# tsereda/fast-cwdm

Hardware: AMD Instinct MI355X
Metric: denoising-steps/sec on 8-ch 128^3 volumes (1000-step DDPM, i2i cWDM) (higher is better)
Workload: dtype bf16; 1 GPU; config2: BraTS 3->1 conditional synthesis, 1xMI355X per replica, 128^3 subbands, 1000-step DDPM (direct linear schedule); model=UNetModel run.sh (mc 64, mult 1,2,2,4,4, 2 res blocks, 81.5M params), global_batch=1, seq_len=2097152, parallelism=replicas1

## Files before the change

### fast-cwdm_amd/csrc/common.hpp

```cpp
#pragma once
#include <hip/hip_runtime.h>
#include <stdint.h>
#include <cstdlib>
#include <string>

#include "../../include/cwdm.h"

namespace cwdm {

void set_error(const std::string& msg);
int fail(int code, const std::string& msg);

#define CWDM_HIP(expr)                                                        \
  do {                                                                        \
    hipError_t e_ = (expr);                                                   \
    if (e_ != hipSuccess)                                                     \
      return ::cwdm::fail(CWDM_E_HIP, std::string(#expr) + ": " +            \
                                          hipGetErrorString(e_));             \
  } while (0)

#define CWDM_REQUIRE(cond, code, msg)                                         \
  do {                                                                        \
    if (!(cond)) return ::cwdm::fail(code, msg);                              \
  } while (0)
// ... 42 lines not shown
  static constexpr int kDtype = CWDM_BF16;
  __device__ __forceinline__ static float to_f(bf16_t v) { return bf2f(v); }
  __device__ __forceinline__ static bf16_t from_f(float v) { return f2bf(v); }
};
template <> struct Elem<f16_t> {
  static constexpr int kDtype = CWDM_F16;
  __device__ __forceinline__ static float to_f(f16_t v) { return (float)v; }
  __device__ __forceinline__ static f16_t from_f(float v) { return (f16_t)v; }
};

template <typename T> __device__ __forceinline__ float lo2f(unsigned u);
template <typename T> __device__ __forceinline__ float hi2f(unsigned u);
template <> __device__ __forceinline__ float lo2f<bf16_t>(unsigned u) { return __uint_as_float(u << 16); }
template <> __device__ __forceinline__ float hi2f<bf16_t>(unsigned u) { return __uint_as_float(u & 0xffff0000u); }
template <> __device__ __forceinline__ float lo2f<f16_t>(unsigned u) {
  return (float)__builtin_bit_cast(f16_t, (unsigned short)(u & 0xffffu));
}
template <> __device__ __forceinline__ float hi2f<f16_t>(unsigned u) {
  return (float)__builtin_bit_cast(f16_t, (unsigned short)(u >> 16));
}
template <typename T> __device__ __forceinline__ unsigned pack2(float a, float b);
template <> __device__ __forceinline__ unsigned pack2<bf16_t>(float a, float b) {
  typedef __bf16 bf16x2_t __attribute__((ext_vector_type(2)));
  const f32x2_t v = {a, b};
  return __builtin_bit_cast(unsigned, __builtin_convertvector(v, bf16x2_t));
}
template <> __device__ __forceinline__ unsigned pack2<f16_t>(float a, float b) {
  const f32x2_t v = {a, b};
  return __builtin_bit_cast(unsigned, __builtin_convertvector(v, f16x2_t));
}

inline int dtype_size(int dtype) { return dtype == CWDM_F32 ? 4 : 2; }
inline bool dtype_half(int dtype) { return dtype == CWDM_BF16 || dtype == CWDM_F16; }
inline bool dtype_compute(int dtype) { return dtype == CWDM_F32 || dtype == CWDM_BF16 || dtype == CWDM_F16; }

template <typename F>
inline int dispatch_dtype(int dtype, F&& f) {
  if (dtype == CWDM_BF16) return f(bf16_t{});
  if (dtype == CWDM_F16) return f(f16_t{});
  return f(float{});
}

inline int ck_of(int dtype) { return 32 / dtype_size(dtype); }

inline int64_t ceil_div(int64_t a, int64_t b) { return (a + b - 1) / b; }

inline int env_int(const char* name, int dflt) {
  const char* e = std::getenv(name);
  return e ? std::atoi(e) : dflt;
}
inline long long env_ll(const char* name, long long dflt) {
  const char* e = std::getenv(name);
  return e ? std::atoll(e) : dflt;
}
inline double env_double(const char* name, double dflt) {
  const char* e = std::getenv(name);
  return e ? std::atof(e) : dflt;
}
inline bool env_not0(const char* name) {
  const char* e = std::getenv(name);
  return !(e && e[0] == '0');
}
inline bool env_is1(const char* name) {
  const char* e = std::getenv(name);
  return e && e[0] == '1';
}
inline bool env_set(const char* name) { return std::getenv(name) != nullptr; }

struct FastDiv {
  unsigned d, m, s;
};
inline FastDiv make_fastdiv(unsigned d) {
  unsigned s = 0;
  while ((1ull << s) < d) ++s;
  return {d, (unsigned)(((1ull << 32) * ((1ull << s) - d)) / d + 1), s};
}
__device__ __forceinline__ unsigned fdiv(unsigned n, const FastDiv& f) { return (__umulhi(n, f.m) + n) >> f.s; }


struct PackJob {
  const float* w;
  void* out;
  long long total;
  int cout, cin, ntaps, NT, transpose, cin_real, s2_ci0, pad;
  long long blk0;
};
static_assert(sizeof(PackJob) == 64, "PackJob layout");

struct GbwdFuse {
  const void* x0; const void* x1; int c0;
  const float* ss; const float* mr; int groups;
  float* part; long long part_bytes;
  bool used; int nblk;
};
extern thread_local GbwdFuse* g_gbwd;

struct GapplyFuse {
  const void* x0; const void* x1;
  const void* du;
  const float* ss;
  const float* coef;
  bool used;
};
extern thread_local GapplyFuse* g_gapply;

struct GnFinFuse {
  const float* s0; long long p0; int c0;
  const float* s1; long long p1; int c1;
  const float* gamma; const float* beta;
  int groups; long long voxels; float eps;
  float* ss;
  float* mr;
  long long B;
  bool used;
};
extern thread_local GnFinFuse* g_gnfin;
}
```

### fast-cwdm_amd/csrc/conv3d.hip

```cpp
#include <algorithm>
#include <cstdlib>
#include <cstring>
#include <vector>

#include "conv3d_kernels.hpp"
#include "internal.hpp"

namespace cwdm {
CWDM_WIDE_INSTANCES(extern template, bf16_t)
CWDM_SMALL_INSTANCES(extern template, bf16_t)
CWDM_WIDE_INSTANCES(extern template, f16_t)
CWDM_SMALL_INSTANCES(extern template, f16_t)
CWDM_WIDE_INSTANCES(extern template, float)
CWDM_SMALL_INSTANCES(extern template, float)

__device__ __forceinline__ int s2_k(int t, int p) { return t == 1 ? 1 + p : ((t == 0 && p == 1) ? 0 : -1); }
__device__ __forceinline__ float s2_weight(const float* w, int ci0, int co, int ci_e, int t) {
  const int ph = ci_e / ci0, ci = ci_e % ci0;
  const int kz = s2_k(t / 9, ph >> 2), ky = s2_k((t / 3) % 3, (ph >> 1) & 1), kx = s2_k(t % 3, ph & 1);
  if (kz < 0 || ky < 0 || kx < 0) return 0.f;
  return w[((long long)co * ci0 + ci) * 27 + (kz * 3 + ky) * 3 + kx];
}

template <typename T>
__device__ __forceinline__ void pack_elem(const float* __restrict__ w, int cout, int cin, int ntaps, int NT,
                                          T* __restrict__ out, int transpose, int cin_real, int s2_ci0, long long i) {
  constexpr int CK = ConvTr<T>::CK, EPQ = ConvTr<T>::EPQ;
  const int nch = cin / CK;
  const int e = i % EPQ;
  long long r = i / EPQ;
  const int qp = r % 2;
  r /= 2;
  const int n = r % NT;
  r /= NT;
  const int tap = r % ntaps;
  r /= ntaps;
  const int chunk = r % nch;
  const int ct = r / nch;
  const int q = qp ^ ((n >> 3) & 1);
  const int co = ct * NT + n, ci = chunk * CK + q * EPQ + e;
  float v = 0.f;
  if (co < cout && ci < cin_real) {
    if (s2_ci0) v = transpose ? s2_weight(w, s2_ci0, ci, co, ntaps - 1 - tap) : s2_weight(w, s2_ci0, co, ci, tap);
    else if (transpose) v = w[((long long)ci * cout + co) * ntaps + (ntaps - 1 - tap)];
    else v = w[((long long)co * cin + ci) * ntaps + tap];
  }
  out[i] = Elem<T>::from_f(v);
}

template <typename T>
__global__ void __launch_bounds__(256) pack_kernel(const float* __restrict__ w, int cout, int cin, int ntaps, int NT,
                                                   int nct, T* __restrict__ out, int transpose, int cin_real,
                                                   int s2_ci0) {
  constexpr int CK = ConvTr<T>::CK;
  const long long total = (long long)nct * (cin / CK) * ntaps * NT * CK;
  const long long i = (long long)blockIdx.x * blockDim.x + threadIdx.x;
  if (i < total) pack_elem<T>(w, cout, cin, ntaps, NT, out, transpose, cin_real, s2_ci0, i);
}

template <typename T>
__global__ void __launch_bounds__(256) pack_batch_kernel(const PackJob* __restrict__ jobs, int njobs) {
  const long long bid = blockIdx.x;
  int lo = 0, hi = njobs - 1;
  while (lo < hi) {
    const int mid = (lo + hi + 1) >> 1;
    if (jobs[mid].blk0 <= bid) lo = mid;
    else hi = mid - 1;
  }
  const PackJob j = jobs[lo];
  const long long base = (bid - j.blk0) * 1024;
#pragma unroll
  for (int k = 0; k < 4; ++k) {
    const long long i = base + k * 256 + threadIdx.x;
    if (i < j.total)
      pack_elem<T>(j.w, j.cout, j.cin, j.ntaps, j.NT, reinterpret_cast<T*>(j.out), j.transpose, j.cin_real,
                   j.s2_ci0, i);
  }
}

template <typename T>
__global__ void __launch_bounds__(256) pack_tile_kernel(const PackJob* __restrict__ jobs, int njobs) {
  constexpr int CK = ConvTr<T>::CK, EPQ = ConvTr<T>::EPQ;
  __shared__ __attribute__((aligned(16))) float sm[32 * CK * 27];
  const long long bid = blockIdx.x;
  int lo = 0, hi = njobs - 1;
  while (lo < hi) {
    const int mid = (lo + hi + 1) >> 1;
    if (jobs[mid].blk0 <= bid) lo = mid;
    else hi = mid - 1;
  }
  const PackJob j = jobs[lo];
  const int nch = j.cin / CK, nsubs = j.NT / 32, nt = j.ntaps;
  long long r = bid - j.blk0;
  const int chunk = (int)(r % nch);
  r /= nch;
  const int nsub = (int)(r % nsubs);
  const int ct = (int)(r / nsubs);
  const int co0 = ct * j.NT + nsub * 32, ci0 = chunk * CK;
  const int tid = threadIdx.x;
  const int rows = j.transpose ? CK : 32, L = j.transpose ? 32 * nt : CK * nt;
  const int nk = j.transpose ? min(32, j.cout - co0) * nt : L;
  auto src_of = [&](int row) -> const float* {
    return j.transpose ? j.w + ((long long)(ci0 + row) * j.cout + co0) * nt
                       : j.w + ((long long)(co0 + row) * j.cin + ci0) * nt;
  };
  auto row_ok = [&](int row) { return j.transpose ? ci0 + row < j.cin_real : co0 + row < j.cout; };
  const bool v4 = ((size_t)j.w & 15) == 0 && L % 4 == 0 && nk % 4 == 0 &&
                  (j.transpose ? (long long)j.cout * nt % 4 == 0 : (long long)j.cin * nt % 4 == 0);
  if (v4) {
    const int L4 = L / 4, n4 = rows * L4;
    for (int i0 = tid; i0 < n4; i0 += 4 * 256) {
      float4 v[4];
#pragma unroll
      for (int u = 0; u < 4; ++u) {
        const int i = i0 + u * 256;
        v[u] = make_float4(0.f, 0.f, 0.f, 0.f);
        if (i < n4) {
          const int row = i / L4, k4 = i - row * L4;
          if (row_ok(row) && 4 * k4 < nk) v[u] = reinterpret_cast<const float4*>(src_of(row))[k4];
        }
      }
#pragma unroll
      for (int u = 0; u < 4; ++u) {
        const int i = i0 + u * 256;
        if (i < n4) reinterpret_cast<float4*>(sm)[i] = v[u];
      }
    }
  } else {
    for (int row = 0; row < rows; ++row) {
      const float* src = src_of(row);
      const bool ok = row_ok(row);
      for (int k = tid; k < L; k += 256) sm[row * L + k] = (ok && k < nk) ? src[k] : 0.f;
    }
  }
  __syncthreads();
  T* out = reinterpret_cast<T*>(j.out);
  for (int v = tid; v < nt * 64; v += 256) {
    const int qp = v & 1, nl = (v >> 1) & 31, tap = v >> 6;
    const int q = qp ^ ((nl >> 3) & 1);
    T tmp[EPQ] __attribute__((aligned(16)));
#pragma unroll
    for (int e = 0; e < EPQ; ++e) {
      const int cil = q * EPQ + e;
      const float x = j.transpose ? sm[(cil * 32 + nl) * nt + (nt - 1 - tap)] : sm[(nl * CK + cil) * nt + tap];
      tmp[e] = Elem<T>::from_f(x);
    }
    const long long off = (((((long long)ct * nch + chunk) * nt + tap) * j.NT + nsub * 32 + nl) * 2 + qp) * EPQ;
    *reinterpret_cast<uint4*>(out + off) = *reinterpret_cast<const uint4*>(tmp);
  }
}

__global__ void __launch_bounds__(256) pack_split_kernel(const float* __restrict__ w, int cout, int cin, int NT,
                                                         bf16_t* __restrict__ out, long long total) {
  const long long i = (long long)blockIdx.x * blockDim.x + threadIdx.x;
  if (i >= total) return;
  const int nvc = 3 * (cin / 16);
  const int e = (int)(i % 8);
  long long r = i / 8;
  const int qp = (int)(r % 2);
// ... 19 lines not shown
template <typename T, int NF>
int dispatch_brick(const ConvParams& p, const Brick& br, hipStream_t s) {
  if (br.bx == 32 && br.bz == 4) return launch_wide<T, NF>(p, s);
  if (br.bx == 32) return launch_conv<T, 32, 4, 2, NF>(p, s);
  if (br.bx == 16) return launch_conv<T, 16, 4, 4, NF>(p, s);
  return launch_conv<T, 8, 8, 4, NF>(p, s);
}

inline int pick_ksplit(long long nblk, int total_chunks) {
  static const long long target = env_ll("CWDM_KSPLIT_TARGET", 768);
  if (nblk >= 512 || nblk >= target || total_chunks <= 1) return 1;
  int S = (int)((target + nblk - 1) / nblk);
  if (S > total_chunks) S = total_chunks;
  const int per = (total_chunks + S - 1) / S;
  return (total_chunks + per - 1) / per;
}

}

using namespace cwdm;

extern "C" int64_t cwdm_conv3d_packed_bytes(int cout, int cin, int ksize, int dtype) {
  if (cout <= 0 || cin <= 0 || (ksize != 1 && ksize != 3)) return -1;
  const int ck = ck_of(dtype);
  if (cin % ck) return -1;
  const int NT = 32 * pick_nf(cout);
  const int nct = (int)ceil_div(cout, NT);
  const int ntaps = ksize * ksize * ksize;
  if (!dtype_compute(dtype)) return -1;
  const int esz = dtype_size(dtype);
  return (int64_t)nct * (cin / ck) * ntaps * NT * ck * esz;
}

static int pack_impl(const float* w, int cout, int cin, int ksize, int dtype, void* packed, int transpose,
                     cwdm_stream_t stream, int s2_ci0 = 0) {
  CWDM_REQUIRE(w && packed, CWDM_E_INVALID, "cwdm_conv3d_pack: null pointer");
  CWDM_REQUIRE(ksize == 1 || ksize == 3, CWDM_E_UNSUPPORTED, "cwdm_conv3d_pack: kernel size must be 1 or 3");
  CWDM_REQUIRE(dtype_compute(dtype), CWDM_E_INVALID, "cwdm_conv3d_pack: bad dtype");
  const int ck = ck_of(dtype);
  const int cin_real = cin;
  if (transpose) cin = (int)ceil_div(cin, ck) * ck;
  CWDM_REQUIRE(cin % ck == 0, CWDM_E_UNSUPPORTED,
               "cwdm_conv3d_pack: input channels must be a multiple of " + std::to_string(ck));
  const int NT = 32 * pick_nf(cout);
  const int nct = (int)ceil_div(cout, NT);
  const int ntaps = ksize * ksize * ksize;
  const long long total = (long long)nct * (cin / ck) * ntaps * NT * ck;
  if (g_pack_batch) {
    g_pack_batch->push_back(PackJob{w, packed, total, cout, cin, ntaps, NT, transpose, cin_real, s2_ci0, 0, 0});
    return CWDM_OK;
  }
  dim3 grid((unsigned)ceil_div(total, 256));
  return dispatch_dtype(dtype, [&](auto tag) -> int {
    using T = decltype(tag);
    hipLaunchKernelGGL(pack_kernel<T>, grid, dim3(256), 0, (hipStream_t)stream, w, cout, cin, ntaps, NT, nct,
                       reinterpret_cast<T*>(packed), transpose, cin_real, s2_ci0);
    CWDM_LAUNCHED();
    return CWDM_OK;
  });
}

extern "C" int cwdm_conv3d_pack(const float* w, int cout, int cin, int ksize, int dtype, void* packed,
                                cwdm_stream_t stream) {
  return pack_impl(w, cout, cin, ksize, dtype, packed, 0, stream);
}

extern "C" int64_t cwdm_conv3d_packed_split_bytes(int cout, int cin) {
  if (cout <= 0 || cout % 64 || cin <= 0 || cin % 16) return -1;
  return cwdm_conv3d_packed_bytes(cout, 3 * cin, 3, CWDM_BF16);
}

extern "C" int cwdm_conv3d_pack_split(const float* w, int cout, int cin, void* packed, cwdm_stream_t stream) {
  CWDM_REQUIRE(w && packed, CWDM_E_INVALID, "cwdm_conv3d_pack_split: null pointer");
  CWDM_REQUIRE(cout > 0 && cout % 64 == 0 && cin > 0 && cin % 16 == 0, CWDM_E_UNSUPPORTED,
               "cwdm_conv3d_pack_split: cout % 64 == 0, cin % 16 == 0");
  const int NT = 64;
  const long long total = (long long)(cout / NT) * (3 * cin / 16) * 27 * NT * 16;
  hipLaunchKernelGGL(pack_split_kernel, dim3((unsigned)ceil_div(total, 256)), dim3(256), 0, (hipStream_t)stream, w,
                     cout, cin, NT, reinterpret_cast<bf16_t*>(packed), total);
  CWDM_LAUNCHED();
  return CWDM_OK;
}

extern "C" int cwdm_conv3d_pack_s2(const float* w, int cout, int cin, int dtype, void* packed, int transpose,
                                   cwdm_stream_t stream) {
  return transpose ? pack_impl(w, 8 * cin, cout, 3, dtype, packed, 1, stream, cin)
                   : pack_impl(w, cout, 8 * cin, 3, dtype, packed, 0, stream, cin);
}

extern "C" int cwdm_conv3d_pack_dgrad(const float* w, int cout, int cin, int ksize, int dtype, void* packed,
                                      cwdm_stream_t stream) {
  return pack_impl(w, cin, cout, ksize, dtype, packed, 1, stream);
}

namespace cwdm {
thread_local std::vector<PackJob>* g_pack_batch = nullptr;

int pack_batch_run(std::vector<PackJob>& jobs, int dtype, PackJob* table, std::vector<PackJob>& cache,
                   hipStream_t s) {
  if (jobs.empty()) return CWDM_OK;
  static const bool tiled_on = env_not0("CWDM_PACK_TILED");
  auto tiled = [&](const PackJob& j) { return tiled_on && j.s2_ci0 == 0 && j.ntaps <= 27 && j.NT % 32 == 0; };
  std::stable_partition(jobs.begin(), jobs.end(), tiled);
  size_t nt = 0;
  while (nt < jobs.size() && tiled(jobs[nt])) ++nt;
  const int ck = ck_of(dtype);
  long long tb = 0, blk = 0;
  for (size_t i = 0; i < jobs.size(); ++i) {
    auto& j = jobs[i];
    if (i < nt) {
      j.blk0 = tb;
      tb += ceil_div(j.cout, j.NT) * (j.NT / 32) * (long long)(j.cin / ck);
    } else {
      j.blk0 = blk;
      blk += ceil_div(j.total, 1024);
    }
  }
  CWDM_REQUIRE(blk < (1LL << 31) && tb < (1LL << 31), CWDM_E_UNSUPPORTED, "pack batch: too many blocks");
  if (cache.size() != jobs.size() || std::memcmp(cache.data(), jobs.data(), jobs.size() * sizeof(PackJob))) {
    CWDM_HIP(hipMemcpyAsync(table, jobs.data(), jobs.size() * sizeof(PackJob), hipMemcpyHostToDevice, s));
    CWDM_HIP(hipStreamSynchronize(s));
    cache = jobs;
  }
  return dispatch_dtype(dtype, [&](auto tag) -> int {
    using T = decltype(tag);
    if (nt > 0) {
      hipLaunchKernelGGL(pack_tile_kernel<T>, dim3((unsigned)tb), dim3(256), 0, s, table, (int)nt);
      CWDM_LAUNCHED();
    }
    if (nt < jobs.size()) {
      hipLaunchKernelGGL(pack_batch_kernel<T>, dim3((unsigned)blk), dim3(256), 0, s, table + nt,
                         (int)(jobs.size() - nt));
      CWDM_LAUNCHED();
    }
    return CWDM_OK;
  });
}
}

namespace {
struct Plan1 { Brick br; int nf, nct, S; long long nblk; int64_t ws; };
Plan1 plan_conv(const cwdm_conv3d_desc* d) {
  Plan1 q;
  q.br = pick_brick(d->D, d->H, d->W);
  q.nf = pick_nf(d->cout);
  q.nct = (int)ceil_div(d->cout, 32 * q.nf);
  q.nblk = (long long)d->B * ceil_div(d->W, q.br.bx) * ceil_div(d->H, q.br.by) * ceil_div(d->D, q.br.bz) * q.nct;
  const int ck = ck_of(d->dtype);
  const int total = (d->a_c0 + d->a_c1) / ck + (d->b_w ? (d->b_c0 + d->b_c1) / ck : 0);
  q.S = pick_ksplit(q.nblk, total);
  q.ws = q.S > 1 ? (int64_t)q.S * d->B * d->D * d->H * d->W * d->cout * 4 : 0;
  return q;
}
}

extern "C" int64_t cwdm_conv3d_workspace_bytes(const cwdm_conv3d_desc* d) {
  if (!d || d->B <= 0 || d->D <= 0 || d->H <= 0 || d->W <= 0 || d->cout <= 0) return -1;
  const int64_t legacy = plan_conv(d).ws;
  return (v4_eligible(d) || (d->a_w_split && v5_eligible(d, false))) ? std::max(legacy, v4_workspace_bytes(d)) : legacy;
}

extern "C" int64_t cwdm_conv3d_parts(int dtype, int64_t D, int64_t H, int64_t W, int cout) {
  (void)dtype; (void)cout;
  Brick br = pick_brick(D, H, W);
  return ceil_div(D, br.bz) * ceil_div(H, br.by) * ceil_div(W, br.bx);
}

extern "C" int cwdm_conv3d_forward(const cwdm_conv3d_desc* d, cwdm_stream_t stream) {
  CWDM_REQUIRE(d && d->out && (d->a_w || d->b_w), CWDM_E_INVALID, "cwdm_conv3d_forward: null pointer");
  CWDM_REQUIRE(!d->a_w || (d->a0 && d->a_c0 > 0), CWDM_E_INVALID, "cwdm_conv3d_forward: segment A input missing");
  CWDM_REQUIRE(dtype_compute(d->dtype), CWDM_E_INVALID, "cwdm_conv3d_forward: bad dtype");
  CWDM_REQUIRE(d->B > 0 && d->D > 0 && d->H > 0 && d->W > 0 && d->cout > 0, CWDM_E_SHAPE,
               "cwdm_conv3d_forward: empty shape");
  const int ck = ck_of(d->dtype);
  CWDM_REQUIRE(!d->a_w || (d->a_c0 % ck == 0 && d->a_c1 % ck == 0 && (d->a_c1 == 0 || d->a1)), CWDM_E_UNSUPPORTED,
               "cwdm_conv3d_forward: segment A channels must be multiples of " + std::to_string(ck));
  if (d->b_w)
    CWDM_REQUIRE(d->b0 && d->b_c0 > 0 && d->b_c0 % ck == 0 && d->b_c1 % ck == 0 && (d->b_c1 == 0 || d->b1),
                 CWDM_E_UNSUPPORTED, "cwdm_conv3d_forward: segment B channels must be multiples of " + std::to_string(ck));
  CWDM_REQUIRE(d->a_mode >= 0 && d->a_mode <= 2 && d->res_mode >= -1 && d->res_mode <= 2, CWDM_E_INVALID,
               "cwdm_conv3d_forward: bad resample mode");
  if (d->a_mode == 1 || d->res_mode == 1)
    CWDM_REQUIRE(d->D % 2 == 0 && d->H % 2 == 0 && d->W % 2 == 0, CWDM_E_SHAPE,
                 "cwdm_conv3d_forward: upsample needs an even output grid");
  CWDM_REQUIRE(d->res_mode < 0 || d->res, CWDM_E_INVALID, "cwdm_conv3d_forward: residual pointer missing");
// ... 56 lines not shown
```

### fast-cwdm_amd/csrc/conv3d_v4.hip

```cpp
#include <algorithm>
#include <atomic>
#include <cstdlib>

#include "conv3d_v4.hpp"

namespace cwdm {

template __global__ void conv3d_v4_kernel<bf16_t, 0, true>(V4Params);
template __global__ void conv3d_v4_kernel<bf16_t, 0, true, true>(V4Params);
template __global__ void conv3d_v4_kernel<bf16_t, 0, true, false, true>(V4Params);
template __global__ void conv3d_v4_kernel<bf16_t, 0, true, true, true>(V4Params);
template __global__ void conv3d_v4_kernel<bf16_t, 1, true, true>(V4Params);
template __global__ void conv3d_v4_kernel<bf16_t, 1, true>(V4Params);
template __global__ void conv3d_v4_kernel<bf16_t, 0, false>(V4Params);
template __global__ void conv3d_v4_kernel<bf16_t, 1, false>(V4Params);
template __global__ void conv3d_v4_kernel<f16_t, 0, true>(V4Params);
template __global__ void conv3d_v4_kernel<f16_t, 0, true, true>(V4Params);
template __global__ void conv3d_v4_kernel<f16_t, 0, true, false, true>(V4Params);
template __global__ void conv3d_v4_kernel<f16_t, 0, true, true, true>(V4Params);
template __global__ void conv3d_v4_kernel<f16_t, 1, true, true>(V4Params);
template __global__ void conv3d_v4_kernel<f16_t, 1, true>(V4Params);
template __global__ void conv3d_v4_kernel<f16_t, 0, false>(V4Params);
template __global__ void conv3d_v4_kernel<f16_t, 1, false>(V4Params);
template __global__ void conv3d_v4_kernel<float, 0, false>(V4Params);
// ... 225 lines not shown
namespace {
bool gn_fin_fusable(const GnFinFuse& f, int dtype, int c0, int c1) {
  const int C = c0 + c1;
  if (!dtype_half(dtype) || C % 16 || c0 % 16 || f.c0 != c0 || f.c1 != c1 || f.groups <= 0 || C % f.groups) return false;
  const int cpg = C / f.groups;
  static const long long maxv = env_ll("CWDM_GNFIN_MAXV", 32768);
  return cpg <= 16 && 16 % cpg == 0 && f.p0 <= 256 && (c1 == 0 || f.p1 <= 256) && f.voxels <= maxv;
}

int gn_fin_apply(const GnFinFuse& f, const void* x0, int c0, const void* x1, int c1, int64_t B, int64_t V, int dtype,
                 void* out, hipStream_t s) {
  GnFinApplyArgs a{};
  a.x0 = x0; a.c0 = c0; a.x1 = x1; a.c1 = c1;
  a.s0 = f.s0; a.p0 = f.p0; a.s1 = f.s1; a.p1 = f.p1;
  a.gamma = f.gamma; a.beta = f.beta; a.groups = f.groups;
  a.n = (double)((c0 + c1) / f.groups) * (double)f.voxels; a.eps = f.eps;
  a.ss = f.ss; a.mr = f.mr; a.out = out;
  CWDM_REQUIRE(V < (1LL << 31) && V * (c0 + c1) < (1LL << 31), CWDM_E_UNSUPPORTED, "gn_fin_apply: grid too large");
  a.V = (int)V;
  const int nchunk = (c0 + c1) / 16;
  long long nvb = std::max<long long>(1, 512 / (nchunk * B));
  a.vblk = (int)std::max<long long>(128, ceil_div(V, nvb));
  nvb = ceil_div(V, (long long)a.vblk);
  CWDM_REQUIRE(B < 65536 && nvb < 65536, CWDM_E_UNSUPPORTED, "gn_fin_apply: grid too large");
  const dim3 grid((unsigned)nchunk, (unsigned)nvb, (unsigned)B);
  if (dtype == CWDM_F16) hipLaunchKernelGGL(gn_fin_apply_kernel<f16_t>, grid, dim3(256), 0, s, a);
  else hipLaunchKernelGGL(gn_fin_apply_kernel<bf16_t>, grid, dim3(256), 0, s, a);
  CWDM_LAUNCHED();
  return CWDM_OK;
}
}

bool gbwd_grid_ok(const cwdm_conv3d_desc* d) {
  static const int gb_maxw = env_int("CWDM_GBWD_MAXW", 32);
  return g_gbwd && !g_gbwd->used && dtype_half(d->dtype) && d->W <= gb_maxw && d->a_mode == 0 && d->res_mode < 0 &&
         !d->stats;
}

int gn_apply(const void* x0, int c0, const void* x1, int c1, const float* gn, int64_t B, int64_t vpb, int dtype,
             void* out, hipStream_t s, int cm = 0) {
  constexpr int VPT = 4;
  const int G8 = (c0 + c1) / 8;
  CWDM_REQUIRE(B * vpb * G8 < (1LL << 31) - 256 * VPT, CWDM_E_UNSUPPORTED,
               "gn_apply: more than 2^31 channel groups in one launch");
  const int64_t nvox = B * vpb, nq = ceil_div(nvox, VPT);
  const dim3 grid((unsigned)ceil_div(nq * G8, 256));
  const FastDiv dvpb = make_fastdiv((unsigned)vpb), dg8 = make_fastdiv((unsigned)G8);
  return dispatch_dtype(dtype, [&](auto tag) -> int {
    using T = decltype(tag);
    hipLaunchKernelGGL((gn_apply_kernel<T, VPT>), grid, dim3(256), 0, s, reinterpret_cast<const T*>(x0), c0,
                       reinterpret_cast<const T*>(x1), c1, gn, dvpb, dg8, (unsigned)nvox, (unsigned)nq,
                       reinterpret_cast<T*>(out), cm);
    CWDM_LAUNCHED();
    return CWDM_OK;
  });
}

int v4_launch(const cwdm_conv3d_desc* d, const void* a0, int c0, const void* a1, int c1, int a0_cm,
              const void* res, int rmode, void* partial, hipStream_t s) {
  const int esz = dtype_size(d->dtype);
  const int ck = 32 / esz;
  const int64_t SV = src_voxels(d);
  V4Params p{};
  p.B = (int)d->B; p.D = (int)d->D; p.H = (int)d->H; p.W = (int)d->W;
  p.tx = (p.W + 31) / 32; p.ty = p.H / 4; p.tz = p.D / 4;
  p.cout = d->cout; p.nct = d->cout / 64;
  p.nch0 = c0 / ck; p.nch = (c0 + c1) / ck;
  p.a0 = a0; p.ac0 = c0; p.a1 = a1; p.ac1 = c1;
  p.a0_bstride = SV * c0 * esz; p.a1_bstride = SV * c1 * esz;
  p.a0_bytes = (unsigned)(SV * c0 * esz); p.a1_bytes = (unsigned)(SV * c1 * esz);
  p.amode = d->a_mode;
  p.a0_cm = a0_cm;
  p.a0_cvox = (int)SV;
  p.aw = reinterpret_cast<const unsigned char*>(d->a_w);
  p.bias = d->bias; p.bias_bs = d->bias_bstride;
  p.res = res; p.rmode = rmode;
  p.out = d->out;
  p.out_f32 = (d->out_dtype == CWDM_F32 && d->dtype != CWDM_F32) ? 1 : 0;
  p.stats = d->stats;
  p.out1 = d->out1; p.out_c0 = d->out_c0;
  p.accumulate = d->accumulate;
  p.stamps = g_stamps.load(std::memory_order_relaxed);
  if (sg_eligible(d)) return sg_launch(p, d, partial, s);
  if (v5_eligible(d, false))
    return v5_launch(d, a0, c0, a1, c1, a0_cm, nullptr, res, rmode, s);
  const int S = v4_ksplit(d);
  p.ksplit = S;
  p.kper = (p.nch + S - 1) / S;
  if (S > 1) {
    CWDM_REQUIRE(partial, CWDM_E_INVALID, "conv3d: K-split scratch missing");
    p.ks_stride = (long long)p.B * p.D * p.H * p.W * p.cout;
    p.bias = nullptr; p.res = nullptr; p.rmode = -1; p.stats = nullptr;
    p.out = partial; p.out_f32 = 1; p.out1 = nullptr; p.out_c0 = 0; p.accumulate = 0;
  }
  static const bool ct32_on = env_not0("CWDM_V4_CT32");
  const bool ct32 = ct32_on && dtype_half(d->dtype) && S == 1 && !p.out_f32 && !p.accumulate && !p.out1 &&
                    (long long)p.B * p.tx * p.ty * p.tz * p.nct < 256 &&
                    (long long)p.D * p.H * p.W * p.cout * 2 < 0xFFFFE000LL;
  if (ct32) p.nct = d->cout / 32;
  const long long nblk = (long long)p.B * p.tx * p.ty * p.tz * p.nct * S;
  p.nblk = (int)nblk;
  static const int ncu = [] {
    int dev = 0, n = 0;
    if (hipGetDevice(&dev) != hipSuccess || hipDeviceGetAttribute(&n, hipDeviceAttributeMultiprocessorCount, dev) != hipSuccess)
      return 256;
    return n > 0 ? n : 256;
  }();
  static const long long gmul = env_ll("CWDM_V4_GRID_MULT", 4);
  const dim3 grid((unsigned)std::min<long long>(nblk, gmul * ncu));
  static const int stagger_env = env_int("CWDM_CONV_STAGGER", 0);
  p.stagger_cycles = nblk > 2LL * ncu ? (stagger_env >= 0 ? stagger_env : (p.nch * 17000 + 12000) / 2) : 0;
  const bool fast = !p.out_f32 && !p.accumulate && !p.out1 &&
                    (long long)p.D * p.H * p.W * p.cout * 2 < 0xFFFFE000LL;
  prof_begin(s);
  auto launch16 = [&](auto tag) {
    using T = decltype(tag);
    if (p.gx0) {
      if (ct32) hipLaunchKernelGGL((conv3d_v4_kernel<T, 0, true, true, true>), grid, dim3(256), 0, s, p);
      else hipLaunchKernelGGL((conv3d_v4_kernel<T, 0, true, false, true>), grid, dim3(256), 0, s, p);
    } else if (ct32) {
      if (p.amode == 1) hipLaunchKernelGGL((conv3d_v4_kernel<T, 1, true, true>), grid, dim3(256), 0, s, p);
      else hipLaunchKernelGGL((conv3d_v4_kernel<T, 0, true, true>), grid, dim3(256), 0, s, p);
    } else if (fast) {
      if (p.amode == 1) hipLaunchKernelGGL((conv3d_v4_kernel<T, 1, true>), grid, dim3(256), 0, s, p);
      else hipLaunchKernelGGL((conv3d_v4_kernel<T, 0, true>), grid, dim3(256), 0, s, p);
    } else {
      if (p.amode == 1) hipLaunchKernelGGL((conv3d_v4_kernel<T, 1, false>), grid, dim3(256), 0, s, p);
      else hipLaunchKernelGGL((conv3d_v4_kernel<T, 0, false>), grid, dim3(256), 0, s, p);
    }
  };
  if (gbwd_grid_ok(d) && (ct32 || fast) && S == 1 && rmode < 0 && !p.stats && p.amode == 0) {
    GbwdFuse& g = *g_gbwd;
    const int nc = ct32 ? 32 : 64;
    const int C = d->cout;
    const long long need = (long long)p.B * p.tx * p.ty * p.tz * C * 8;
    if (g.groups > 0 && C % g.groups == 0 && C / g.groups >= 2 && g.c0 % nc == 0 && g.c0 <= C &&
        (g.c0 == C || g.x1) && need <= g.part_bytes) {
      p.gx0 = g.x0; p.gx1 = g.x1; p.gc0 = g.c0;
      p.gss = g.ss; p.gmr = g.mr; p.ggroups = g.groups;
      p.gdiv = make_fastdiv((unsigned)(C / g.groups));
      p.stats = g.part;
      g.used = true;
      g.nblk = p.tx * p.ty * p.tz;
    }
  }
  if (d->dtype == CWDM_BF16) {
    launch16(bf16_t{});
  } else if (d->dtype == CWDM_F16) {
    launch16(f16_t{});
  } else {
    if (p.amode == 1) hipLaunchKernelGGL((conv3d_v4_kernel<float, 1, false>), grid, dim3(256), 0, s, p);
    else hipLaunchKernelGGL((conv3d_v4_kernel<float, 0, false>), grid, dim3(256), 0, s, p);
  }
  prof_end(s, 2.0 * p.B * p.D * p.H * p.W * (double)p.cout * 27.0 * (c0 + c1));
  CWDM_LAUNCHED();
  if (S > 1) {
    const long long n4 = p.ks_stride / 4;
    float* part = reinterpret_cast<float*>(partial);
    hipLaunchKernelGGL(splitk_sum_kernel<0>, dim3((unsigned)ceil_div(n4, 256)), dim3(256), 0, s, part, S, n4);
    CWDM_LAUNCHED();
    ConvParams q{};
    q.B = p.B; q.D = p.D; q.H = p.H; q.W = p.W;
    q.tx = p.tx; q.ty = p.ty; q.tz = p.tz;
    q.cout = p.cout; q.nct = p.nct;
    q.bias = d->bias; q.bias_bs = d->bias_bstride;
    q.res = res; q.rmode = rmode;
// ... 278 lines not shown
```

### fast-cwdm_amd/csrc/conv3d_v4.hpp

```cpp
#pragma once
#include <type_traits>

#include "conv3d_kernels.hpp"
#include "internal.hpp"

namespace cwdm {

struct V4Params {
  int B, D, H, W;
  int tx, ty, tz;
  int nct, cout;
  int nch, nch0;
  const void* a0; int ac0; const void* a1; int ac1;
  unsigned a0_bytes, a1_bytes;
  long long a0_bstride, a1_bstride;
  int amode;
  int a0_cm;
  int a0_cvox;
  const unsigned char* aw;
  const float* bias; long long bias_bs;
  const void* res; int rmode;
  void* out; int out_f32;
  float* stats;
  void* out1; int out_c0;
  int accumulate;
  int stagger_cycles;
  int nblk;
  int ksplit, kper;
  long long ks_stride;
  unsigned long long* stamps;
  const void* gx0; const void* gx1; int gc0;
  const float* gss; const float* gmr; int ggroups;
  FastDiv gdiv;
  const float* agn;
  int diag;
  const void* ax0; const void* ax1; int axc0, axc1; int aa_lead;
  int aa_units;
  int aa_prio;
  unsigned* aa_cnt;
  int aa_spin;
  int aa_extra;
  int stats_wg;
};


__device__ unsigned g_v4_cu_arrivals[8 * 256];

constexpr int kV5AaWords = 4096;
struct V5Aa { const void* x0; int c0; const void* x1; int c1; const float* gn; int lead, units; unsigned* cnt; };

int sg_launch(const V4Params& v, const cwdm_conv3d_desc* d, void* partial, hipStream_t s);
int v5_launch(const cwdm_conv3d_desc* d, const void* a0, int c0, const void* a1, int c1, int a0_cm,
              const float* agn, const void* res, int rmode, hipStream_t s, const V5Aa* aa = nullptr);

struct V4Cfg {
  static constexpr int HX = 34, HY = 6, HZ = 6, HV = HX * HY * HZ;
  static constexpr int HVP = 1280;
  static constexpr int PIECES = 2 * HVP / 64;
  static constexpr int HALO_B = 2 * HVP * 16;
  static constexpr int SMEM = 2 * HALO_B;
  static constexpr int pad(int k) { return (k >> 1) * HALO_B + (k & 1) * HVP * 16 + HV * 16; }
  static constexpr int gss_off(int s) { return pad(1 + 2 * s) + 256; }
  static constexpr int gmr_off(int s) { return pad(2) + 256 + 256 * s; }
};

template <typename T>
__device__ __forceinline__ void v4_mfma(f32x16& acc, const u32x4& a, const u32x4& b) {
  mfma_acc(acc, a, b, (T*)nullptr);
}

__device__ __forceinline__ void v4_gload(u32x4& dst, const unsigned char* src) {
  asm volatile("global_load_dwordx4 %0, %1, off" : "=v"(dst) : "v"(src) : "memory");
}
#ifdef CWDM_CONV_STAMPS
#define V4_STAMP(k)                                                                                   \
  do {                                                                                                \
    if (p.stamps && tid == 0) p.stamps[(long long)blockIdx.x * 24 + (k)] = __builtin_amdgcn_s_memtime(); \
  } while (0)
#else
#define V4_STAMP(k) do { } while (0)
#endif
#ifndef V4_HALO_GI
#define V4_HALO_GI 1
#endif
#define V4_WAIT_W(n, w) \
  asm volatile("s_waitcnt vmcnt(" #n ")" : "+v"((w)[0]), "+v"((w)[1]), "+v"((w)[2]) :: "memory")

__device__ __forceinline__ unsigned pack_bf16x2(float a, float b) {
  typedef __bf16 bf16x2_t __attribute__((ext_vector_type(2)));
  typedef float f32x2_t __attribute__((ext_vector_type(2)));
  const f32x2_t v = {a, b};
  return __builtin_bit_cast(unsigned, __builtin_convertvector(v, bf16x2_t));
}

__device__ __forceinline__ float row16_sum(float v) {
  v += __builtin_bit_cast(float, __builtin_amdgcn_mov_dpp(__builtin_bit_cast(int, v), 0xB1, 0xF, 0xF, true));
  v += __builtin_bit_cast(float, __builtin_amdgcn_mov_dpp(__builtin_bit_cast(int, v), 0x4E, 0xF, 0xF, true));
  v += __builtin_bit_cast(float, __builtin_amdgcn_mov_dpp(__builtin_bit_cast(int, v), 0x141, 0xF, 0xF, true));
  v += __builtin_bit_cast(float, __builtin_amdgcn_mov_dpp(__builtin_bit_cast(int, v), 0x140, 0xF, 0xF, true));
  return v;
}

template <int K>
__device__ __forceinline__ void v4_read_step(u32x4 (&av)[6], const unsigned char* hb) {
  constexpr int G = K / 2, PL = K % 2, DZ = G / 3 - 1, DX = G % 3 - 1;
#pragma unroll
  for (int L = 0; L < 6; ++L)
    av[L] = *reinterpret_cast<const u32x4*>(hb + (((PL + 1 + DZ) * V4Cfg::HY + L) * V4Cfg::HX + (DX + 1)) * 16);
}

template <typename T, bool FAST, bool CT32 = false, bool GB = false>
__device__ __forceinline__ void v4_epilogue(const V4Params& p, f32x16 (&acc)[2][4], int b, int sl, int ct, int x0,
                                            int y0, int z0, int ks, int tid, int wv, unsigned char* smem,
                                            int gslot = 0) {
  constexpr int NPL = CT32 ? 1 : 2;
  using T16 = std::conditional_t<sizeof(T) == 2, T, bf16_t>;
  const int lane = tid & 63, lr = lane & 31, hh = lane >> 5;
  const int zb = CT32 ? wv : 2 * (wv >> 1);
  const int c0w = CT32 ? ct * 32 : ct * 64 + (wv & 1) * 32;
  const int cbase = c0w + 4 * hh;
  float ssum[16], ssq[16];
#pragma unroll
  for (int i = 0; i < 16; ++i) { ssum[i] = 0.f; ssq[i] = 0.f; }
  const int ox = x0 + lr;
  const bool xin = ox < p.W;
  const float xm = xin ? 1.f : 0.f;
  const long long HW = (long long)p.H * p.W;
  const long long vox0 = (((long long)b * p.D + z0 + zb) * p.H + y0) * p.W + ox;
  if constexpr (FAST) {
    const int cl = c0w + 8 * hh;
    const long long V = (long long)p.D * HW;
    const __amdgpu_buffer_rsrc_t ro = __builtin_amdgcn_make_buffer_rsrc(
        reinterpret_cast<T16*>(p.out) + (long long)b * V * p.cout, (short)0, (int)(V * p.cout * 2), 0x00020000);
    const unsigned vb0 = (unsigned)((((z0 + zb) * p.H) + y0) * p.W + ox);
    const unsigned rowb = (unsigned)p.W * (unsigned)p.cout * 2u, planeb = (unsigned)HW * (unsigned)p.cout * 2u;
    const unsigned obase = vb0 * (unsigned)p.cout * 2u + (unsigned)cl * 2u;
// ... 155 lines not shown
          if (p.out1) {
            if (co >= p.out_c0) { obase = p.out1; ostride = p.cout - p.out_c0; oc = co - p.out_c0; }
            else ostride = p.out_c0;
          }
          if (p.out_f32 || sizeof(T) == 4) {
            float* o = reinterpret_cast<float*>(obase) + ks * p.ks_stride + vox * ostride + oc;
            if (p.accumulate) {
              const float4 oq = *reinterpret_cast<const float4*>(o);
              v[0] += oq.x; v[1] += oq.y; v[2] += oq.z; v[3] += oq.w;
            }
            *reinterpret_cast<float4*>(o) = make_float4(v[0], v[1], v[2], v[3]);
          } else {
            T16* o = reinterpret_cast<T16*>(obase) + vox * ostride + oc;
            if (p.accumulate) {
              const uint2 oq = *reinterpret_cast<const uint2*>(o);
              v[0] += lo2f<T16>(oq.x); v[1] += hi2f<T16>(oq.x);
              v[2] += lo2f<T16>(oq.y); v[3] += hi2f<T16>(oq.y);
            }
            uint2 sq;
            sq.x = pack2<T16>(v[0], v[1]);
            sq.y = pack2<T16>(v[2], v[3]);
            *reinterpret_cast<uint2*>(o) = sq;
          }
#pragma unroll
          for (int k = 0; k < 4; ++k) {
            ssum[4 * j + k] += v[k];
            ssq[4 * j + k] += v[k] * v[k];
          }
        }
      }
    }
  }
  if (p.stats) {
#pragma unroll
    for (int i = 0; i < 16; ++i) {
      ssum[i] = row16_sum(ssum[i]);
      ssq[i] = row16_sum(ssq[i]);
      ssum[i] += __builtin_bit_cast(float, __builtin_amdgcn_ds_swizzle(__builtin_bit_cast(int, ssum[i]), 0x401F));
      ssq[i] += __builtin_bit_cast(float, __builtin_amdgcn_ds_swizzle(__builtin_bit_cast(int, ssq[i]), 0x401F));
    }
    float* R = reinterpret_cast<float*>(smem + V4Cfg::pad(wv));
    if (lr == 0) {
#pragma unroll
      for (int i = 0; i < 16; ++i) {
        R[hh * 32 + i] = ssum[i];
        R[hh * 32 + 16 + i] = ssq[i];
      }
    }
    asm volatile("s_waitcnt lgkmcnt(0)" ::: "memory");
    __builtin_amdgcn_s_barrier();
    if (CT32 ? tid < 32 : tid < 64) {
      const int ff = tid >> 5, c32 = tid & 31;
      const int h2 = GB ? (c32 >> 3) & 1 : (c32 >> 2) & 1;
      const int i = GB ? 8 * (c32 >> 4) + (c32 & 7) : 4 * (c32 >> 3) + (c32 & 3);
      const int tiles = p.tx * p.ty * p.tz;
      float su, sq;
      if constexpr (CT32) {
        su = 0.f; sq = 0.f;
#pragma unroll
        for (int w = 0; w < 4; ++w) {
          const float* Rw = reinterpret_cast<const float*>(smem + V4Cfg::pad(w)) + h2 * 32;
          su += Rw[i];
          sq += Rw[16 + i];
        }
      } else {
        const float* R0 = reinterpret_cast<const float*>(smem + V4Cfg::pad(ff)) + h2 * 32;
        const float* R1 = reinterpret_cast<const float*>(smem + V4Cfg::pad(ff + 2)) + h2 * 32;
        su = R0[i] + R1[i];
        sq = R0[16 + i] + R1[16 + i];
      }
      const int c = (CT32 ? ct * 32 : ct * 64) + tid;
      if constexpr (GB) {
        const float* gm = reinterpret_cast<const float*>(smem + V4Cfg::gmr_off(gslot));
        const unsigned gi = fdiv((unsigned)c, p.gdiv) - fdiv((unsigned)(c - tid), p.gdiv);
        sq = gm[2 * gi + 1] * (sq - gm[2 * gi] * su);
      }
      const long long pidx = ((long long)b * tiles + sl) * p.cout + c;
      p.stats[pidx * 2 + 0] = su;
      p.stats[pidx * 2 + 1] = sq;
    }
  }
}

struct V4Tile { int b, sl, ct, x0, y0, z0, ks, c0, c1; };
__device__ __forceinline__ V4Tile v4_tile_of(const V4Params& p, int it) {
  const int tiles = p.tx * p.ty * p.tz;
  const int nbase = p.nblk / p.ksplit;
  const int t = blockIdx.x + it * gridDim.x;
  const int xcd = t & 7, q8 = p.nblk >> 3, r8 = p.nblk & 7;
  int wg = (xcd < r8 ? xcd * (q8 + 1) : r8 * (q8 + 1) + (xcd - r8) * q8) + (t >> 3);
  V4Tile r;
  r.ks = wg / nbase;
  wg -= r.ks * nbase;
  r.c0 = r.ks * p.kper;
  r.c1 = min(p.nch, r.c0 + p.kper);
  r.ct = wg % p.nct;
  const int st = wg / p.nct;
  r.b = st / tiles;
  r.sl = st - r.b * tiles;
  r.x0 = (r.sl % p.tx) * 32; r.y0 = ((r.sl / p.tx) % p.ty) * 4; r.z0 = (r.sl / (p.tx * p.ty)) * 4;
  r.ct = __builtin_amdgcn_readfirstlane(r.ct); r.b = __builtin_amdgcn_readfirstlane(r.b);
  r.sl = __builtin_amdgcn_readfirstlane(r.sl); r.x0 = __builtin_amdgcn_readfirstlane(r.x0);
  r.y0 = __builtin_amdgcn_readfirstlane(r.y0); r.z0 = __builtin_amdgcn_readfirstlane(r.z0);
  r.ks = __builtin_amdgcn_readfirstlane(r.ks); r.c0 = __builtin_amdgcn_readfirstlane(r.c0);
  r.c1 = __builtin_amdgcn_readfirstlane(r.c1);
  return r;
}

template <typename T, int MODE, int PB = V4Cfg::HVP * 16, bool ALL = false>
__device__ __forceinline__ void v4_issue_halo(const V4Params& p, const V4Tile& tt, int c, unsigned char* hb, int wv,
                                              int lane) {
  using C = V4Cfg;
  constexpr int CK = ConvTr<T>::CK;
  constexpr int ESZ = sizeof(T);
  const int SH = MODE == 1 ? p.H >> 1 : p.H, SW = MODE == 1 ? p.W >> 1 : p.W;
  int svox[5];
#pragma unroll
  for (int j = 0; j < 5; ++j) {
    const int hv = (wv + 4 * j) * 64 + lane;
    int sv = -2;
    if (hv < C::HV) {
      sv = -1;
      const int hx = hv % C::HX, hy = (hv / C::HX) % C::HY, hz = hv / (C::HX * C::HY);
      int ox = tt.x0 + hx - 1, oy = tt.y0 + hy - 1, oz = tt.z0 + hz - 1;
      if (ox >= 0 && oy >= 0 && oz >= 0 && ox < p.W && oy < p.H && oz < p.D) {
        if (MODE == 1) { ox >>= 1; oy >>= 1; oz >>= 1; }
        sv = (oz * SH + oy) * SW + ox;
      }
    }
    svox[j] = sv;
  }
  const bool s0 = c < p.nch0;
  const unsigned char* base = s0 ? reinterpret_cast<const unsigned char*>(p.a0) + (long long)tt.b * p.a0_bstride
                                 : reinterpret_cast<const unsigned char*>(p.a1) + (long long)tt.b * p.a1_bstride;
  const __amdgpu_buffer_rsrc_t rs =
      __builtin_amdgcn_make_buffer_rsrc((void*)base, (short)0, (int)(s0 ? p.a0_bytes : p.a1_bytes), 0x00020000);
  const int cs = s0 ? p.ac0 : p.ac1;
  const int cb = (s0 ? c : c - p.nch0) * CK;
  const bool cm = s0 && p.a0_cm;
  const unsigned rowb = cm ? 32u : (unsigned)cs * ESZ;
  const unsigned cofs = cm ? (unsigned)c * (unsigned)p.a0_cvox * 32u : (unsigned)(cb * ESZ);
#pragma unroll
  for (int j = 0; j < 10; ++j) {
    const int pc = wv + 4 * j;
    const int sv = svox[j % 5];
    const unsigned voff = sv >= 0 ? (unsigned)sv * rowb + cofs + (unsigned)((j / 5) * 16) : 0xFFFFFFF0u;
    if (ALL || sv != -2)
      __builtin_amdgcn_raw_ptr_buffer_load_lds(
          rs, (__attribute__((address_space(3))) void*)(hb + (PB == 20 * 1024 ? pc * 1024 : (pc / 20) * PB + (pc % 20) * 1024)),
          16, voff, 0, 0, 0);
  }
}

template <typename T, int MODE, bool FAST, bool CT32 = false, bool GB = false>
__global__ void __launch_bounds__(256, 2) conv3d_v4_kernel(V4Params p) {
  static_assert(!FAST || sizeof(T) == 2, "the fast epilogue is 16-bit (bf16 / fp16) only");
  using C = V4Cfg;
  __shared__ __attribute__((aligned(1024))) unsigned char smem[C::SMEM];

  const int tid = threadIdx.x, lane = tid & 63, lr = lane & 31, hh = lane >> 5;
  const int wv = __builtin_amdgcn_readfirstlane(tid >> 6);
  const int f = wv & 1, vg = wv >> 1;
  constexpr int NPL = CT32 ? 1 : 2;
  const int zb = CT32 ? wv : 2 * vg;
  V4_STAMP(0);
#ifdef CWDM_CONV_STAMPS
  if (p.stamps && tid == 0) p.stamps[(long long)blockIdx.x * 24 + 20] = __builtin_amdgcn_s_memrealtime();
  if (p.stamps && tid == 0) {
    p.stamps[(long long)blockIdx.x * 24 + 22] = __builtin_amdgcn_s_getreg((4 << 0) | (0 << 6) | (31 << 11));
    p.stamps[(long long)blockIdx.x * 24 + 23] = __builtin_amdgcn_s_getreg((20 << 0) | (0 << 6) | (31 << 11));
  }
#endif

  if (p.stagger_cycles > 0) {
// ... 159 lines not shown
```

### fast-cwdm_amd/csrc/conv3d_v5.hip

```cpp
#include <atomic>
#include <cstdlib>

#include "conv3d_v4.hpp"

namespace cwdm {

struct V5Cfg {
  static constexpr int HALO_B = V4Cfg::HALO_B;
  static constexpr int STG1 = 3 * HALO_B;
  static constexpr int BIAS = STG1 + 32768;
  static constexpr int SCR = BIAS + 512;
  static constexpr int GSS = SCR + 2048;
  static constexpr int CNT = GSS + 1536;
  static constexpr int RUN = CNT + 256;
  static constexpr int SMEM = RUN + 1024;
};
static_assert(V5Cfg::SMEM <= 163840, "v5 LDS");

#ifdef CWDM_V5_DIAG
#define V5_DIAG(bit) ((p.diag & (bit)) != 0)
#else
#define V5_DIAG(bit) false
#endif
#define V5_PHYS(t, c) (V5_DIAG(64) ? (t).c0 + ((c) - (t).c0 + (t).sl) % ((t).c1 - (t).c0) : (c))

#ifdef CWDM_CONV_STAMPS
#define V5_STAMP(k, cond)                                                                        \
  do {                                                                                           \
    if (p.stamps && (cond)) p.stamps[(long long)blockIdx.x * 64 + (k)] = __builtin_amdgcn_s_memtime(); \
  } while (0)
#else
#define V5_STAMP(k, cond) do { } while (0)
#endif

constexpr int kV5AaCnt = kV5AaWords;
__device__ unsigned g_cwdm_dev_err;

__device__ __forceinline__ bool v5aa_wait(unsigned* c, unsigned need, int spin, int sleep2) {
  for (int n = 0; __hip_atomic_load(c, __ATOMIC_RELAXED, __HIP_MEMORY_SCOPE_AGENT) < need; ++n) {
    if (n >= spin) {
      __hip_atomic_fetch_or(&g_cwdm_dev_err, 1u, __ATOMIC_RELAXED, __HIP_MEMORY_SCOPE_AGENT);
      return false;
    }
    if (sleep2) __builtin_amdgcn_s_sleep(2);
    else __builtin_amdgcn_s_sleep(1);
  }
  asm volatile("" ::: "memory");
  return true;
}

__device__ __forceinline__ int v5aa_pos() {
  const int G = gridDim.x;
  const int b = blockIdx.x;
  return (G & 7) ? b : (b & 7) * (G >> 3) + (b >> 3);
}
__device__ __forceinline__ V4Tile v5aa_tile_of(const V4Params& p, int it) {
  const int wg = it * (int)gridDim.x + v5aa_pos();
  V4Tile r;
  r.ks = 0; r.c0 = 0; r.c1 = p.nch; r.b = 0;
  r.ct = wg % p.nct;
  r.sl = wg / p.nct;
  r.x0 = (r.sl % p.tx) * 32; r.y0 = ((r.sl / p.tx) % p.ty) * 4; r.z0 = (r.sl / (p.tx * p.ty)) * 4;
  r.ct = __builtin_amdgcn_readfirstlane(r.ct); r.sl = __builtin_amdgcn_readfirstlane(r.sl);
  r.x0 = __builtin_amdgcn_readfirstlane(r.x0); r.y0 = __builtin_amdgcn_readfirstlane(r.y0);
  r.z0 = __builtin_amdgcn_readfirstlane(r.z0);
  return r;
}
__host__ __device__ __forceinline__ unsigned v5aa_need(int j, int G, int nblk, int nct, int tx, int ty, int D, int H,
                                                       int W) {
  if (j < 0) return 0u;
  long long w = (long long)(j + 1) * G;
  if (w > nblk) w = nblk;
  const int st = (int)(w - 1) / nct;
  const int z1 = (st / (tx * ty)) * 4 + 5;
  return (unsigned)(z1 < D ? z1 : D) * (unsigned)H * (unsigned)W;
}

template <typename T, int MODE, bool GN, int AA = 0>
__global__ void __launch_bounds__(512) conv3d_v5_kernel(V4Params p) {
  using C = V4Cfg;
  using T16 = T;
  constexpr int NI = 10 + (GN ? 1 : 0);
  __shared__ __attribute__((aligned(1024))) unsigned char smem[V5Cfg::SMEM];

  const int tid = threadIdx.x, lane = tid & 63, lr = lane & 31, hh = lane >> 5;
  const int wv = __builtin_amdgcn_readfirstlane(tid >> 6);
  const int nblk = p.nblk;
  const int ntile = (nblk - (AA ? v5aa_pos() : (int)blockIdx.x) + (int)gridDim.x - 1) / (int)gridDim.x;
  if (ntile <= 0) return;
  auto tile_of = [&](int it) { return AA ? v5aa_tile_of(p, it) : v4_tile_of(p, it); };
  const int tiles = p.tx * p.ty * p.tz;

  const int G = (int)gridDim.x;
  const unsigned V = (unsigned)p.D * (unsigned)p.H * (unsigned)p.W;
  struct AaLane { const unsigned char* src; unsigned rowb, oq; int vo, vps; bool on; float a[8], b[8]; };
  auto aa_lane = [&](int slot, int nslot) {
    AaLane l{};
    if constexpr (AA > 0) {
      const int Q = (p.axc0 + p.axc1) >> 3, q0 = p.axc0 >> 3;
      l.vps = nslot / Q;
      l.on = slot < l.vps * Q;
      const int q = l.on ? slot % Q : 0;
      l.vo = l.on ? slot / Q : 0;
      l.src = q < q0 ? reinterpret_cast<const unsigned char*>(p.ax0) + q * 16
                     : reinterpret_cast<const unsigned char*>(p.ax1) + (q - q0) * 16;
      l.rowb = (unsigned)(q < q0 ? p.axc0 : p.axc1) * 2u;
      l.oq = (unsigned)(q >> 1) * V * 32u + (unsigned)(q & 1) * 16u;
#pragma unroll
      for (int e = 0; e < 8; ++e) silu_aff_coef(p.agn[(q * 8 + e) * 2], p.agn[(q * 8 + e) * 2 + 1], l.a[e], l.b[e]);
    } else {
      (void)slot; (void)nslot;
    }
    return l;
  };
  const __amdgpu_buffer_rsrc_t ract = __builtin_amdgcn_make_buffer_rsrc(
      const_cast<void*>(p.a0), (short)0, (int)(AA ? V * (unsigned)(p.axc0 + p.axc1) * 2u : 0u), 0x00020000);
  auto aa_load = [&](const AaLane& l, unsigned v, bool ok) -> u32x4 {
    return *reinterpret_cast<const __attribute__((address_space(1))) u32x4*>(
        (const __attribute__((address_space(1))) unsigned char*)(l.src) + (size_t)(ok ? v : 0u) * l.rowb);
  };
  auto aa_store = [&](const AaLane& l, const u32x4& x, unsigned v, bool ok) {
    float xv[8], y[8];
    unpack<T>(x, xv);
#pragma unroll
    for (int e = 0; e < 8; ++e) y[e] = silu_aff(xv[e], l.a[e], l.b[e]);
    __builtin_amdgcn_raw_buffer_store_b128(pack<T>(y), ract, ok ? l.oq + v * 32u : 0xFFFFFFF0u, 0, 16);
  };
  auto aa_piece = [&](unsigned r0, unsigned r1, unsigned& lo, unsigned& hi) {
    const int pos = v5aa_pos();
    lo = r0 + (unsigned)((unsigned long long)(r1 - r0) * (unsigned)pos / (unsigned)G);
    hi = r0 + (unsigned)((unsigned long long)(r1 - r0) * (unsigned)(pos + 1) / (unsigned)G);
  };
  auto aa_need = [&](int j) { return v5aa_need(j, G, nblk, p.nct, p.tx, p.ty, p.D, p.H, p.W); };
  const int aa_nit = (nblk + G - 1) / G;
  if constexpr (AA > 0) {
    V5_STAMP(55, tid == 0);
    const AaLane l = aa_lane(tid, 512);
    unsigned lo, hi;
    aa_piece(0u, aa_need(p.aa_lead - 1), lo, hi);
    const int nst = l.vps > 0 ? (int)((hi - lo + (unsigned)l.vps - 1) / (unsigned)l.vps) : 0;
    for (int s0 = 0; s0 < nst; s0 += 4) {
      u32x4 x[4];
#pragma unroll
      for (int k = 0; k < 4; ++k) {
        const unsigned v = lo + (unsigned)((s0 + k) * l.vps + l.vo);
        x[k] = aa_load(l, v, l.on && v < hi);
      }
#pragma unroll
      for (int k = 0; k < 4; ++k) {
        const unsigned v = lo + (unsigned)((s0 + k) * l.vps + l.vo);
        aa_store(l, x[k], v, l.on && v < hi);
      }
    }
    asm volatile("s_waitcnt vmcnt(0)" ::: "memory");
    __syncthreads();
    if (tid == 0) {
      __hip_atomic_fetch_add(&p.aa_cnt[0], 1u, __ATOMIC_RELAXED, __HIP_MEMORY_SCOPE_AGENT);
      v5aa_wait(&p.aa_cnt[0], (unsigned)(G + p.aa_extra), p.aa_spin, 1);
    }
    __syncthreads();
  }

  V5_STAMP(0, tid == 0);
#ifdef CWDM_CONV_STAMPS
  if (p.stamps && tid == 0) {
    p.stamps[(long long)blockIdx.x * 64 + 50] = __builtin_amdgcn_s_memrealtime();
    p.stamps[(long long)blockIdx.x * 64 + 53] = __builtin_amdgcn_s_getreg((4 << 0) | (0 << 6) | (31 << 11));
    p.stamps[(long long)blockIdx.x * 64 + 54] = __builtin_amdgcn_s_getreg((20 << 0) | (0 << 6) | (31 << 11));
  }
#endif
  if (wv < 4) {
    __builtin_amdgcn_s_setprio(2);
    const int f = wv & 1, vg = wv >> 1, zb = 2 * vg;
    const unsigned char* wlane = p.aw + f * 1024 + lr * 32 + ((hh ^ ((lr >> 3) & 1)) << 4);
    auto load_w = [&](u32x4 (&w)[3], int ct, int c, int g) {
      if (V5_DIAG(4)) return;
      const unsigned char* src = wlane + ((long long)ct * p.nch + c) * 27 * 2048 + ((g / 3) * 9 + (g % 3)) * 2048;
      v4_gload(w[0], src);
      v4_gload(w[1], src + 3 * 2048);
      v4_gload(w[2], src + 6 * 2048);
    };
    const int hlane = hh * (C::HVP * 16) + (zb * (C::HX * C::HY) + lr) * 16;
    f32x16 acc[2][4];
    u32x4 wr[3][3];
    V4Tile cur = tile_of(0);
    load_w(wr[0], cur.ct, V5_PHYS(cur, cur.c0), 0);
    load_w(wr[1], cur.ct, V5_PHYS(cur, cur.c0), 1);
    __builtin_amdgcn_s_barrier();
    V5_STAMP(1, tid == 0);
    int gch = 0;
    for (int it = 0; it < ntile; ++it) {
      const bool more = it + 1 < ntile;
      const V4Tile nxt = more ? tile_of(it + 1) : cur;
      {
        float bia[16];
        const float* bl = reinterpret_cast<const float*>(smem + V5Cfg::BIAS + (it & 1) * 256) + f * 32 + 4 * hh;
#pragma unroll
        for (int i = 0; i < 16; ++i) bia[i] = p.bias ? bl[8 * (i >> 2) + (i & 3)] : 0.f;
#pragma unroll
        for (int a = 0; a < 2; ++a)
#pragma unroll
          for (int m = 0; m < 4; ++m)
#pragma unroll
            for (int i = 0; i < 16; ++i) acc[a][m][i] = bia[i];
      }
      auto chunk = [&](auto lastc, int c) {
        constexpr bool LAST = decltype(lastc)::value;
        const unsigned char* hb = smem + (gch % 3) * C::HALO_B + hlane;
        u32x4 av[2][6];
        if (!V5_DIAG(2)) v4_read_step<0>(av[0], hb);
#define V5_STEP(K)                                                                                           \
        {                                                                                                    \
          constexpr int GI = (K) / 2, PL = (K) % 2, KN = (K) + 1, BC = (K) & 1;                              \
           \
           \
           \
             \
          if (PL == 0) {                                                                                     \
            if (GI + 2 < 9) load_w(wr[(GI + 2) % 3], cur.ct, V5_PHYS(cur, c), GI + 2);                       \
            else if (!LAST) load_w(wr[(GI + 2) % 3], cur.ct, V5_PHYS(cur, c + 1), GI - 7);                   \
            else load_w(wr[(GI + 2) % 3], nxt.ct, V5_PHYS(nxt, nxt.c0), GI - 7);                             \
          }                                                                                                  \
          if (KN < 18 && !V5_DIAG(2)) v4_read_step<KN % 18>(av[BC ^ 1], hb);                                 \
          if (PL == 0) V4_WAIT_W(6, wr[GI % 3]);                                                             \
          __builtin_amdgcn_sched_barrier(0);                                                                 \
          _Pragma("unroll") for (int dy = 0; dy < 3; ++dy)                                                   \
          _Pragma("unroll") for (int m = 0; m < 4; ++m)                                                      \
            v4_mfma<T>(acc[PL][m], wr[GI % 3][dy], av[BC][m + dy]);                                          \
          __builtin_amdgcn_sched_barrier(0);                                                                 \
        }
        V5_STEP(0) V5_STEP(1) V5_STEP(2) V5_STEP(3) V5_STEP(4) V5_STEP(5)
        V5_STEP(6) V5_STEP(7) V5_STEP(8) V5_STEP(9) V5_STEP(10) V5_STEP(11)
        V5_STEP(12) V5_STEP(13) V5_STEP(14) V5_STEP(15) V5_STEP(16) V5_STEP(17)
#undef V5_STEP
        V5_STAMP(2 + gch, tid == 0 && gch < 16);
        __builtin_amdgcn_s_barrier();
        V5_STAMP(18 + gch, tid == 0 && gch < 16);
        ++gch;
      };
      for (int c = cur.c0; c + 1 < cur.c1; ++c) chunk(std::false_type{}, c);
      chunk(std::true_type{}, cur.c1 - 1);
      unsigned char* st = smem + (vg == 0 ? ((gch + 2) % 3) * C::HALO_B : V5Cfg::STG1);
#pragma unroll
      for (int pl = 0; pl < 2; ++pl)
#pragma unroll
        for (int m = 0; m < 4; ++m)
#pragma unroll
          for (int jj = 0; jj < 2; ++jj) {
            float v[8];
#pragma unroll
            for (int k = 0; k < 8; ++k) v[k] = acc[pl][m][8 * jj + k];
            const unsigned p0 = pack2<T16>(v[0], v[1]), p1 = pack2<T16>(v[2], v[3]);
            const unsigned p2 = pack2<T16>(v[4], v[5]), p3 = pack2<T16>(v[6], v[7]);
            const auto t0 = __builtin_amdgcn_permlane32_swap(p0, p2, false, false);
            const auto t1 = __builtin_amdgcn_permlane32_swap(p1, p3, false, false);
            u32x4 w;
            w[0] = t0[0]; w[1] = t1[0]; w[2] = t0[1]; w[3] = t1[1];
            const int row = pl * 128 + m * 32 + lr;
            const int q = 4 * f + 2 * jj + hh;
            *reinterpret_cast<u32x4*>(st + row * 128 + ((q ^ (lr & 7)) << 4)) = w;
          }
      asm volatile("s_waitcnt lgkmcnt(0)" ::: "memory");
      __builtin_amdgcn_s_barrier();
      cur = nxt;
    }
    asm volatile("s_waitcnt vmcnt(0)" : "+v"(wr[0][0]), "+v"(wr[0][1]), "+v"(wr[0][2]), "+v"(wr[1][0]), "+v"(wr[1][1]),
                 "+v"(wr[1][2])::"memory");
#ifdef CWDM_CONV_STAMPS
    if (p.stamps && tid == 0) p.stamps[(long long)blockIdx.x * 64 + 51] = __builtin_amdgcn_s_memrealtime();
#endif
    return;
  }

  const int h = wv - 4;
  const int r8 = lane >> 3, q = lane & 7;
  unsigned* cnt = reinterpret_cast<unsigned*>(smem + V5Cfg::CNT);
  int pit = 0;
  V4Tile pt = tile_of(0);
  int pc = pt.c0;
  auto issue_next = [&](int buf) -> bool {
    if (pit >= ntile) return false;
    if (!V5_DIAG(1)) v4_issue_halo<T, MODE>(p, pt, V5_PHYS(pt, pc), smem + buf * C::HALO_B, h, lane);
    if constexpr (GN) {
      if (lane < 32)
        __builtin_amdgcn_global_load_lds(
            (const __attribute__((address_space(1))) void*)(p.agn + ((long long)pt.b * (p.ac0 + p.ac1) +
                                                                      V5_PHYS(pt, pc) * 16) * 2 + lane),
            (__attribute__((address_space(3))) void*)(smem + V5Cfg::GSS + (buf * 4 + h) * 128), 4, 0, 0);
    }
    if (pc + 1 < pt.c1) ++pc;
    else if (++pit < ntile) { pt = tile_of(pit); pc = pt.c0; }
    return true;
  };
  auto transform = [&](int x0, int y0, int z0, int buf) {
    if constexpr (GN) {
      if (V5_DIAG(16)) return;
      unsigned char* hb = smem + buf * C::HALO_B;
      const float* gs = reinterpret_cast<const float*>(smem + V5Cfg::GSS + (buf * 4 + h) * 128);
      u32x4 x[2][5];
#pragma unroll
      for (int j = 0; j < 5; ++j)
#pragma unroll
        for (int qd = 0; qd < 2; ++qd)
          x[qd][j] = *reinterpret_cast<const u32x4*>(hb + qd * (C::HVP * 16) + ((h + 4 * j) * 64 + lane) * 16);
      float mk[5];
#pragma unroll
      for (int j = 0; j < 5; ++j) {
        const int hv = (h + 4 * j) * 64 + lane;
        const int hx = hv % C::HX, hy = (hv / C::HX) % C::HY, hz = hv / (C::HX * C::HY);
        const int ox = x0 + hx - 1, oy = y0 + hy - 1, oz = z0 + hz - 1;
        mk[j] = (hv < C::HV && ox >= 0 && oy >= 0 && oz >= 0 && ox < p.W && oy < p.H && oz < p.D) ? 1.f : 0.f;
      }
      const bool inner = x0 >= 1 && y0 >= 1 && z0 >= 1 && x0 + C::HX - 1 <= p.W && y0 + C::HY - 1 <= p.H &&
                         z0 + C::HZ - 1 <= p.D;
#pragma unroll
      for (int qd = 0; qd < 2; ++qd) {
        float sa[8], sb[8];
#pragma unroll
        for (int e = 0; e < 8; ++e) silu_aff_coef(gs[2 * (8 * qd + e)], gs[2 * (8 * qd + e) + 1], sa[e], sb[e]);
#pragma unroll
        for (int j = 0; j < 5; ++j) {
          float xv[8], y[8];
          unpack<T>(x[qd][j], xv);
#pragma unroll
          for (int e = 0; e < 8; ++e) y[e] = V5_DIAG(8) ? xv[e] : silu_aff(xv[e], sa[e], sb[e]);
          if (!inner) {
#pragma unroll
            for (int e = 0; e < 8; ++e) y[e] *= mk[j];
          }
          *reinterpret_cast<u32x4*>(hb + qd * (C::HVP * 16) + ((h + 4 * j) * 64 + lane) * 16) = pack<T>(y);
        }
      }
    } else {
      (void)x0; (void)y0; (void)z0; (void)buf;
    }
  };
  const long long HW = (long long)p.H * p.W, VV = (long long)p.D * HW;
  const unsigned rowb = (unsigned)p.W * (unsigned)p.cout * 2u, planeb = (unsigned)HW * (unsigned)p.cout * 2u;
  float s1[8], s2[8];
  bool wg_final = false;
  u32x4 dq[8];
  unsigned doff[8];
  u32x4 rq[8];
  auto drain_load = [&](const V4Tile& tt, int part) {
    if (p.rmode < 0) return;
    const int ox = tt.x0 + 8 * h + r8;
    const bool xin = ox < p.W;
    const long long rV = p.rmode == 1 ? VV / 8 : VV;
    const __amdgpu_buffer_rsrc_t rr = __builtin_amdgcn_make_buffer_rsrc(
        (void*)(reinterpret_cast<const T16*>(p.res) + (long long)tt.b * rV * p.cout), (short)0,
        (int)(rV * p.cout * 2), 0x00020000);
#pragma unroll
    for (int k = 0; k < 8; ++k) {
      const int i = 8 * part + k;
      const int oy = tt.y0 + (i & 3), oz = tt.z0 + (i >> 2);
      unsigned rv = p.rmode == 1 ? (unsigned)(((oz >> 1) * (p.H >> 1) + (oy >> 1)) * (p.W >> 1) + (ox >> 1))
                                 : (unsigned)((oz * p.H + oy) * p.W + ox);
      rq[k] = __builtin_amdgcn_raw_buffer_load_b128(
          rr, xin ? rv * (unsigned)p.cout * 2u + (unsigned)(tt.ct * 64 + 8 * q) * 2u : 0xFFFFFFF0u, 0, 0);
    }
  };
  auto drain = [&](const V4Tile& tt, int part, int sb, int k0, int k1) {
    if (V5_DIAG(32)) return;
    const int ox = tt.x0 + 8 * h + r8;
    const bool xin = ox < p.W;
    const float xm = xin ? 1.f : 0.f;
    u32x4 sv[8];
    const unsigned char* base = smem + (part ? V5Cfg::STG1 : sb * C::HALO_B);
#pragma unroll
    for (int k = 0; k < 8; ++k) {
      if (k < k0 || k >= k1) continue;
      const int row = 8 * (h + 4 * k) + r8;
      sv[k] = *reinterpret_cast<const u32x4*>(base + row * 128 + ((q ^ r8) << 4));
    }
    if (part == 0) {
#pragma unroll
      for (int e = 0; e < 8; ++e) { s1[e] = 0.f; s2[e] = 0.f; }
    }
    const unsigned obase =
        ((unsigned)((tt.z0 * p.H + tt.y0) * p.W) + (unsigned)ox) * (unsigned)p.cout * 2u + (unsigned)(tt.ct * 64 + 8 * q) * 2u;
#pragma unroll
    for (int k = 0; k < 8; ++k) {
      if (k < k0 || k >= k1) continue;
      const int i = 8 * part + k;
      float v[8];
      unpack<T>(sv[k], v);
      if (p.rmode >= 0) {
        float r[8];
        unpack<T>(rq[k], r);
#pragma unroll
        for (int e = 0; e < 8; ++e) v[e] += r[e];
      }
#pragma unroll
      for (int e = 0; e < 8; ++e) {
        const float vv = v[e] * xm;
        s1[e] += vv;
        s2[e] += vv * vv;
      }
      const unsigned oo = obase + (unsigned)(i >> 2) * planeb + (unsigned)(i & 3) * rowb;
      dq[k] = pack<T>(v);
      doff[k] = xin ? oo : 0xFFFFFFF0u;
    }
    if (part == 1 && k1 == 8 && p.stats) {
#pragma unroll
      for (int e = 0; e < 16; ++e) {
        float& sx = e < 8 ? s1[e] : s2[e - 8];
        sx += __builtin_bit_cast(float, __builtin_amdgcn_mov_dpp(__builtin_bit_cast(int, sx), 0x128, 0xF, 0xF, true));
        sx += __builtin_bit_cast(float, __builtin_amdgcn_ds_swizzle(__builtin_bit_cast(int, sx), 0x401F));
        const unsigned u = __builtin_bit_cast(unsigned, sx);
        const auto sw = __builtin_amdgcn_permlane32_swap(u, u, false, false);
        sx += __builtin_bit_cast(float, lane < 32 ? (unsigned)sw[1] : (unsigned)sw[0]);
      }
      float* sc = reinterpret_cast<float*>(smem + V5Cfg::SCR) + (h * 64 + 8 * q) * 2;
      if (lane < 8) {
#pragma unroll
        for (int e = 0; e < 8; e += 2)
          *reinterpret_cast<float4*>(sc + 2 * e) = make_float4(s1[e], s2[e], s1[e + 1], s2[e + 1]);
      }
      asm volatile("s_waitcnt lgkmcnt(0)" ::: "memory");
      unsigned old = 0;
      if (lane == 0) old = __hip_atomic_fetch_add(cnt, 1u, __ATOMIC_ACQ_REL, __HIP_MEMORY_SCOPE_WORKGROUP);
      old = __builtin_amdgcn_readfirstlane(old);
      if ((old & 3u) == 3u) {
        const float* s0 = reinterpret_cast<const float*>(smem + V5Cfg::SCR) + lane * 2;
        float su = 0.f, sq = 0.f;
#pragma unroll
        for (int k = 0; k < 4; ++k) { su += s0[k * 128]; sq += s0[k * 128 + 1]; }
        if (p.stats_wg) {
          float2* run = reinterpret_cast<float2*>(smem + V5Cfg::RUN);
          float2 r = run[tt.ct * 64 + lane];
          r.x += su; r.y += sq;
          run[tt.ct * 64 + lane] = r;
          if (wg_final) {
            for (int ct = 0; ct < p.nct; ++ct)
              *reinterpret_cast<float2*>(p.stats + ((long long)blockIdx.x * p.cout + ct * 64 + lane) * 2) =
                  run[ct * 64 + lane];
          }
        } else {
          const long long pidx = ((long long)tt.b * tiles + tt.sl) * p.cout + tt.ct * 64 + lane;
          *reinterpret_cast<float2*>(p.stats + pidx * 2) = make_float2(su, sq);
        }
      }
    }
  };
  auto drain_put = [&](const V4Tile& tt, int k0, int k1) {
    if (V5_DIAG(32)) return;
    const __amdgpu_buffer_rsrc_t ro = __builtin_amdgcn_make_buffer_rsrc(
        reinterpret_cast<T16*>(p.out) + (long long)tt.b * VV * p.cout, (short)0, (int)(VV * p.cout * 2), 0x00020000);
#pragma unroll
    for (int k = 0; k < 8; ++k) {
      if (k < k0 || k >= k1) continue;
      __builtin_amdgcn_raw_buffer_store_b128(dq[k], ro, doff[k], 0, 0);
    }
  };
  auto issue_bias = [&](const V4Tile& tt, int slot) {
    if (p.bias && h == 0)
      __builtin_amdgcn_global_load_lds(
          (const __attribute__((address_space(1))) void*)(p.bias + (long long)tt.b * p.bias_bs + tt.ct * 64 + lane),
          (__attribute__((address_space(3))) void*)(smem + V5Cfg::BIAS + slot * 256), 4, 0, 0);
  };

  if constexpr (AA > 0) {
    constexpr int NA = 10;
    const AaLane al = aa_lane(h * 64 + lane, 256);
    const int L = p.aa_lead;
    int pit = 0;
    V4Tile pt = tile_of(0);
    int pc = pt.c0;
    bool chk = false;
    auto issue_aa = [&](int buf) {
      v4_issue_halo<T, MODE, C::HVP * 16, true>(p, pt, pc, smem + buf * C::HALO_B, h, lane);
      if (pc + 1 < pt.c1) {
        ++pc;
      } else if (pit + 1 < ntile) {
        ++pit; pt = tile_of(pit); pc = pt.c0;
        chk = pit >= L && pit < aa_nit;
      }
    };
    V4Tile cur = tile_of(0);
    if (h == 0 && lane == 0) *cnt = 0u;
    if (p.stats_wg && h == 0) {
      reinterpret_cast<float4*>(smem + V5Cfg::RUN)[lane] = make_float4(0.f, 0.f, 0.f, 0.f);
    }
    issue_aa(0);
    issue_bias(cur, 0);
    issue_aa(1);
    asm volatile("s_waitcnt vmcnt(%0)" ::"n"(NA) : "memory");
    asm volatile("s_waitcnt lgkmcnt(0)" ::: "memory");
    __builtin_amdgcn_s_barrier();
    int gch = 0;
    int pend = 0, pr = 0;
    const int nch = cur.c1 - cur.c0;
    const int nslice = (nch - 1) < 3 ? (nch - 1) : 3;
    const int srows = (8 + nslice - 1) / nslice;
    const int cs = nch >= 3 ? 1 : 0;
    V4Tile dt = cur;
    for (int it = 0; it < ntile; ++it) {
      const bool more = it + 1 < ntile;
      const V4Tile nxt = more ? tile_of(it + 1) : cur;
      unsigned plo = 0u, phi = 0u;
      if (it + L < aa_nit) aa_piece(aa_need(it + L - 1), aa_need(it + L), plo, phi);
      for (int c = cur.c0; c < cur.c1; ++c) {
        const bool first = c == cur.c0, lastc = c + 1 == cur.c1;
        const int cc = c - cur.c0;
        if (chk && pc == pt.c0) {
#ifdef CWDM_CONV_STAMPS
          const unsigned long long t0 = __builtin_amdgcn_s_memtime();
#endif
          v5aa_wait(&p.aa_cnt[pit], (unsigned)(G + p.aa_extra), p.aa_spin, 0);
          chk = false;
#ifdef CWDM_CONV_STAMPS
          if (p.stamps && tid == 256) p.stamps[(long long)blockIdx.x * 64 + 56] += __builtin_amdgcn_s_memtime() - t0;
#endif
        }
        if (cc == 1 && it > 0 && it - 1 + L < aa_nit && tid == 256)
          __hip_atomic_fetch_add(&p.aa_cnt[it - 1 + L], 1u, __ATOMIC_RELAXED, __HIP_MEMORY_SCOPE_AGENT);
        int d0 = 0, k0 = 0, k1 = 0;
        if (pend == 2) {
          drain(dt, 0, (gch + 2) % 3, 0, 8);
          d0 = 1; k0 = 0; k1 = 8;
          pend = 1; pr = 0;
        } else if (pend == 1) {
          k0 = pr; k1 = pr + srows < 8 ? pr + srows : 8;
          drain(dt, 1, 0, k0, k1);
          pr = k1;
          if (pr == 8) pend = 0;
        }
        if (k1 > k0) asm volatile("s_waitcnt lgkmcnt(0)" ::: "memory");
        const int n0 = cc >= cs ? (cc - cs) * p.aa_units : -1;
        u32x4 ax[AA];
        unsigned av[AA];
        bool aok[AA];
#pragma unroll
        for (int a = 0; a < AA; ++a) {
          av[a] = plo + (unsigned)((n0 + a) * al.vps + al.vo);
          aok[a] = n0 >= 0 && a < p.aa_units && al.on && av[a] < phi;
          v4_gload(ax[a], al.src + (size_t)(aok[a] ? av[a] : 0u) * al.rowb);
        }
        issue_aa((gch + 2) % 3);
        if constexpr (AA == 1) {
          asm volatile("s_waitcnt vmcnt(%1)" : "+v"(ax[0]) : "n"(NA) : "memory");
        } else if constexpr (AA == 2) {
          asm volatile("s_waitcnt vmcnt(%2)" : "+v"(ax[0]), "+v"(ax[1]) : "n"(NA) : "memory");
        } else if constexpr (AA == 4) {
          asm volatile("s_waitcnt vmcnt(%4)" : "+v"(ax[0]), "+v"(ax[1]), "+v"(ax[2]), "+v"(ax[3]) : "n"(NA) : "memory");
        } else {
          asm volatile("s_waitcnt vmcnt(%8)"
                       : "+v"(ax[0]), "+v"(ax[1]), "+v"(ax[2]), "+v"(ax[3]), "+v"(ax[4]), "+v"(ax[5]), "+v"(ax[6]),
                         "+v"(ax[7])
                       : "n"(NA)
                       : "memory");
        }
        if (p.aa_prio) __builtin_amdgcn_s_setprio(1);
#pragma unroll
// ... 361 lines not shown
      const float* gs = reinterpret_cast<const float*>(smem + S::GSS + (bi * 4 + h) * 128);
#pragma unroll
      for (int e = 0; e < 8; ++e) silu_aff_coef(gs[2 * e], gs[2 * e + 1], sc[e], sh[e]);
#pragma unroll
      for (int j = 0; j < 5; ++j) {
        const int hv = (h + 4 * j) * 64 + lane;
        const int hx = hv % C::HX, hy = (hv / C::HX) % C::HY, hz = hv / (C::HX * C::HY);
        const int ox = x0 + hx - 1, oy = y0 + hy - 1, oz = z0 + hz - 1;
        mk[j] = (hv < C::HV && ox >= 0 && oy >= 0 && oz >= 0 && ox < p.W && oy < p.H && oz < p.D) ? 1.f : 0.f;
      }
    } else {
      (void)x0; (void)y0; (void)z0;
    }
#pragma unroll
    for (int j = 0; j < 5; ++j) {
      const int hv = (h + 4 * j) * 64 + lane;
      if (j == 4 && hv >= C::HV) continue;
      float v[8];
#pragma unroll
      for (int e = 0; e < 4; ++e) { v[e] = __uint_as_float(x[0][j][e]); v[4 + e] = __uint_as_float(x[1][j][e]); }
      if constexpr (GN) {
#pragma unroll
        for (int e = 0; e < 8; ++e) v[e] = silu_aff(v[e], sc[e], sh[e]) * mk[j];
      }
      u32x4 hi, lo;
#pragma unroll
      for (int e = 0; e < 4; ++e) {
        hi[e] = pack2<bf16_t>(v[2 * e], v[2 * e + 1]);
        lo[e] = pack2<bf16_t>(v[2 * e] - lo2f<bf16_t>(hi[e]), v[2 * e + 1] - hi2f<bf16_t>(hi[e]));
      }
      *reinterpret_cast<u32x4*>(hb + hv * 16) = hi;
      *reinterpret_cast<u32x4*>(hb + S::PLANE + hv * 16) = lo;
    }
  };
  auto issue_bias = [&](const V4Tile& tt, int slot) {
    if (p.bias && h == 0)
      __builtin_amdgcn_global_load_lds(
          (const __attribute__((address_space(1))) void*)(p.bias + (long long)tt.b * p.bias_bs + tt.ct * 64 + lane),
          (__attribute__((address_space(3))) void*)(smem + S::BIAS + slot * 256), 4, 0, 0);
  };
  V4Tile cur = tile_of(0);
  if (h == 0 && lane < 2) cnt[lane] = 0u;
  if (p.stats_wg && h == 0) reinterpret_cast<float4*>(smem + S::RUN)[lane] = make_float4(0.f, 0.f, 0.f, 0.f);
  issue_pair(0);
  issue_bias(cur, 0);
  asm volatile("s_waitcnt vmcnt(0)" ::: "memory");
  split(cur.x0, cur.y0, cur.z0, 0);
  split(cur.x0, cur.y0, cur.z0, 1);
  asm volatile("s_waitcnt lgkmcnt(0)" ::: "memory");
  __builtin_amdgcn_s_barrier();
  int gp = 0;
  for (int it = 0; it < ntile; ++it) {
    const bool more = it + 1 < ntile;
    const V4Tile nxt = more ? tile_of(it + 1) : cur;
    for (int pp = cur.c0 / 2; pp < cur.c1 / 2; ++pp) {
      const bool first = pp == cur.c0 / 2, lastp = pp + 1 == cur.c1 / 2;
      const int st = (gp + 1) & 1;
      const bool iss = issue_pair(st);
      if (first && more) issue_bias(nxt, (it + 1) & 1);
      if (iss) {
        asm volatile("s_waitcnt vmcnt(0)" ::: "memory");
        const V4Tile& t1 = lastp ? nxt : cur;
        split(t1.x0, t1.y0, t1.z0, 2 * st);
        split(t1.x0, t1.y0, t1.z0, 2 * st + 1);
      }
      asm volatile("s_waitcnt vmcnt(0) lgkmcnt(0)" ::: "memory");
      __builtin_amdgcn_s_barrier();
      ++gp;
    }
    cur = nxt;
  }
}

namespace {
int v5_mode() {
  static const int m = env_int("CWDM_V5", 3);
  return m;
}
}

std::atomic<int> g_v5_grid{0};
std::atomic<int> g_v5_aa{env_int("CWDM_V5_AA", 1)};
std::atomic<int> g_v5_aa_launches{0};
std::atomic<int> g_v5_aa_extra{0};
std::atomic<int> g_v5_aa_spin{0};
thread_local int g_stats_wg = 0;
thread_local int64_t g_stats_rows = 0;

namespace {
int v5_ncu() {
  static const int ncu = [] {
    int dev = 0, n = 0;
    if (hipGetDevice(&dev) != hipSuccess || hipDeviceGetAttribute(&n, hipDeviceAttributeMultiprocessorCount, dev) != hipSuccess)
      return 256;
    return n > 0 ? n : 256;
  }();
  return ncu;
}
int v5_aa_grid(int64_t nblk) {
  static const int occ = [] {
    int n = 0;
    if (hipOccupancyMaxActiveBlocksPerMultiprocessor(&n, conv3d_v5_kernel<bf16_t, 0, false, 8>, 512, 0) != hipSuccess)
      return 1;
    return n > 0 ? n : 1;
  }();
  const int cap = g_v5_grid.load(std::memory_order_relaxed);
  const int64_t lim = (int64_t)v5_ncu() * occ;
  return (int)std::min<int64_t>(nblk, cap > 0 ? std::min<int64_t>(cap, lim) : v5_ncu());
}
}

bool v5_eligible(const cwdm_conv3d_desc* d, bool gn) {
  const int mode = v5_mode();
  const int path = g_conv_path.load(std::memory_order_relaxed);
  if (d->dtype == CWDM_F32) {
    if (!d->a_w_split || path == 1 || path == 3) return false;
    if (d->out_dtype != CWDM_F32 || d->accumulate || d->out1) return false;
    if (d->a_mode != 0 && d->a_mode != 1) return false;
    if (d->a_c0 % 16 || d->a_c1 % 16) return false;
    if (d->res_mode < -1 || d->res_mode > 1) return false;
    if (d->b_w && d->res_mode >= 0) return false;
    if (d->W < kWideMinW || d->H % 4 || d->D % 4 || d->cout % 64) return false;
    const int64_t lim = 0xFFFFE000LL;
    if (d->D * d->H * d->W * d->cout * 4 >= lim) return false;
    const int64_t sv = d->a_mode == 1 ? d->D * d->H * d->W / 8 : d->D * d->H * d->W;
    if (d->a_gn ? sv * (d->a_c0 + d->a_c1) * 4 >= lim : (sv * d->a_c0 * 4 >= lim || sv * d->a_c1 * 4 >= lim))
      return false;
    return !(gn && d->a_mode == 1);
  }
  if (mode <= 0 || (mode == 1 && !gn) || path == 1 || path == 3) return false;
  if (gn && (d->a_mode == 1 || mode == 3)) return false;
  if (!dtype_half(d->dtype) || sg_eligible(d)) return false;
  if (path != 2 && v4_ksplit(d) != 1) return false;
  if (d->out_dtype != d->dtype || d->accumulate || d->out1) return false;
  if (d->a_mode != 0 && d->a_mode != 1) return false;
  if (d->res_mode < -1 || d->res_mode > 1) return false;
  if (d->W < kWideMinW || d->H % 4 || d->D % 4 || d->cout % 64) return false;
  if (d->D * d->H * d->W * d->cout * 2 >= 0xFFFFE000LL) return false;
  if (d->a_c0 + d->a_c1 < 32) return false;
  if (gbwd_grid_ok(d)) return false;
  static const int ncu = [] {
    int dev = 0, n = 0;
    if (hipGetDevice(&dev) != hipSuccess || hipDeviceGetAttribute(&n, hipDeviceAttributeMultiprocessorCount, dev) != hipSuccess)
      return 256;
    return n > 0 ? n : 256;
  }();
  static const double min_tpc = env_double("CWDM_V5_MIN_TPC", 1.0);
  return path == 2 || (double)v4_items(d) >= min_tpc * ncu;
}

int v5_aa_units(const cwdm_conv3d_desc* d, int* lead) {
  const int mode = g_v5_aa.load(std::memory_order_relaxed);
  if (!mode || !d->a_gn || d->B != 1 || d->a_mode != 0 || !dtype_half(d->dtype)) return 0;
  const int C = d->a_c0 + d->a_c1;
  if (d->a_c0 % 8 || d->a_c1 % 8 || C % 16 || C > 2048) return 0;
  if (!v5_eligible(d, false)) return 0;
  static const int minch = env_int("CWDM_V5_AA_MINCH", 8);
  if (mode == 1 && (d->a_c0 + d->a_c1) / 16 < minch) return 0;
  const int64_t V = d->D * d->H * d->W;
  if (V * C * 2 >= 0x7FFFF000LL) return 0;
  const int tx = (int)((d->W + 31) / 32), ty = (int)(d->H / 4), tz = (int)(d->D / 4), nct = d->cout / 64;
  const int64_t nblk = (int64_t)tx * ty * tz * nct;
  const int G = v5_aa_grid(nblk);
  const int nit = (int)((nblk + G - 1) / G);
  if (nit > kV5AaCnt - 2) return 0;
  const int nch = C / 16;
  const int L = nch >= 8 ? 2 : 3;
  if (mode == 1 && nit < 16) return 0;
  const int Q = C / 8, vps = 256 / Q;
  if (vps < 1) return 0;
  const int cs = nch >= 3 ? 1 : 0;
  int64_t steps = 0;
  for (int r = L; r < nit; ++r) {
    const int64_t len = (int64_t)v5aa_need(r, G, (int)nblk, nct, tx, ty, (int)d->D, (int)d->H, (int)d->W) -
                        v5aa_need(r - 1, G, (int)nblk, nct, tx, ty, (int)d->D, (int)d->H, (int)d->W);
    steps = std::max<int64_t>(steps, ((len + G - 1) / G + vps - 1) / vps);
  }
  const int64_t per = std::max<int64_t>(1, (steps + (nch - cs) - 1) / (nch - cs));
  if (per > 8) return 0;
  if (lead) *lead = L;
  return (int)per;
}

int v5_launch(const cwdm_conv3d_desc* d, const void* a0, int c0, const void* a1, int c1, int a0_cm,
              const float* agn, const void* res, int rmode, hipStream_t s, const V5Aa* aa) {
  const int esz = dtype_size(d->dtype);
  const int ck = 32 / esz;
  const int64_t SV = d->a_mode == 1 ? d->D * d->H * d->W / 8 : d->D * d->H * d->W;
  CWDM_REQUIRE(!agn || !a0_cm, CWDM_E_INVALID, "conv3d_v5: GroupNorm applies to raw channels-last sources only");
  V4Params p{};
  p.B = (int)d->B; p.D = (int)d->D; p.H = (int)d->H; p.W = (int)d->W;
  p.tx = (p.W + 31) / 32; p.ty = p.H / 4; p.tz = p.D / 4;
  p.cout = d->cout; p.nct = d->cout / 64;
  p.nch0 = c0 / ck; p.nch = (c0 + c1) / ck;
  p.a0 = a0; p.ac0 = c0; p.a1 = a1; p.ac1 = c1;
  p.a0_bstride = SV * c0 * esz; p.a1_bstride = SV * c1 * esz;
  p.a0_bytes = (unsigned)(SV * c0 * esz); p.a1_bytes = (unsigned)(SV * c1 * esz);
  p.amode = d->a_mode;
  p.a0_cm = a0_cm;
  p.a0_cvox = (int)SV;
  p.aw = reinterpret_cast<const unsigned char*>(d->a_w);
  p.bias = d->bias; p.bias_bs = d->bias_bstride;
  p.res = res; p.rmode = rmode;
  p.out = d->out;
  p.stats = d->stats;
  p.ksplit = 1; p.kper = p.nch;
  p.agn = agn;
  if (aa) {
    CWDM_REQUIRE(a0_cm && !agn && d->B == 1 && d->a_mode == 0, CWDM_E_INVALID, "conv3d_v5: apply-ahead arguments");
    p.ax0 = aa->x0; p.axc0 = aa->c0; p.ax1 = aa->x1; p.axc1 = aa->c1;
    p.agn = aa->gn;
    p.aa_lead = aa->lead;
    p.aa_units = aa->units;
    static const int prio = env_int("CWDM_V5_AA_PRIO", 0);
    p.aa_prio = prio;
    CWDM_REQUIRE(aa->cnt, CWDM_E_INVALID, "conv3d_v5: apply-ahead counters missing");
    p.aa_cnt = aa->cnt;
    const int spin = g_v5_aa_spin.load(std::memory_order_relaxed);
    p.aa_spin = spin > 0 ? spin : (1 << 24);
    p.aa_extra = g_v5_aa_extra.load(std::memory_order_relaxed);
  }
#ifdef CWDM_V5_DIAG
  static const int diag = env_int("CWDM_V5_DIAGMASK", 0);
  p.diag = diag;
#endif
  p.stamps = g_stamps.load(std::memory_order_relaxed);
  const long long nblk = (long long)p.B * p.tx * p.ty * p.tz * p.nct;
  p.nblk = (int)nblk;
  static const int ncu = [] {
    int dev = 0, n = 0;
    if (hipGetDevice(&dev) != hipSuccess || hipDeviceGetAttribute(&n, hipDeviceAttributeMultiprocessorCount, dev) != hipSuccess)
      return 256;
    return n > 0 ? n : 256;
  }();
  const int cap = g_v5_grid.load(std::memory_order_relaxed);
  const dim3 grid(aa ? (unsigned)v5_aa_grid(nblk) : (unsigned)std::min<long long>(nblk, cap > 0 ? cap : ncu));
  if (g_stats_wg && d->stats && p.B == 1 && p.nct <= 2 &&
      (long long)grid.x <= (long long)p.tx * p.ty * p.tz) {
    p.stats_wg = 1;
    g_stats_rows = grid.x;
  }
  prof_begin(s);
  auto go = [&](auto tag) {
    using T = decltype(tag);
    if (agn) {
      if (p.amode == 1) hipLaunchKernelGGL((conv3d_v5_kernel<T, 1, true>), grid, dim3(512), 0, s, p);
      else hipLaunchKernelGGL((conv3d_v5_kernel<T, 0, true>), grid, dim3(512), 0, s, p);
    } else {
      if (p.amode == 1) hipLaunchKernelGGL((conv3d_v5_kernel<T, 1, false>), grid, dim3(512), 0, s, p);
      else hipLaunchKernelGGL((conv3d_v5_kernel<T, 0, false>), grid, dim3(512), 0, s, p);
    }
  };
  if (d->dtype == CWDM_F32) {
    p.aw = reinterpret_cast<const unsigned char*>(d->a_w_split);
    if (agn) {
      if (p.amode == 1) hipLaunchKernelGGL((conv3d_v5s_kernel<1, true>), grid, dim3(512), 0, s, p);
      else hipLaunchKernelGGL((conv3d_v5s_kernel<0, true>), grid, dim3(512), 0, s, p);
    } else {
      if (p.amode == 1) hipLaunchKernelGGL((conv3d_v5s_kernel<1, false>), grid, dim3(512), 0, s, p);
      else hipLaunchKernelGGL((conv3d_v5s_kernel<0, false>), grid, dim3(512), 0, s, p);
    }
  } else if (aa) {
    g_v5_aa_launches.fetch_add(1, std::memory_order_relaxed);
    auto go_aa = [&](auto tag) {
      using T = decltype(tag);
      if (aa->units <= 4) hipLaunchKernelGGL((conv3d_v5_kernel<T, 0, false, 4>), grid, dim3(512), 0, s, p);
      else hipLaunchKernelGGL((conv3d_v5_kernel<T, 0, false, 8>), grid, dim3(512), 0, s, p);
    };
    if (d->dtype == CWDM_BF16) go_aa(bf16_t{});
    else go_aa(f16_t{});
  } else if (d->dtype == CWDM_BF16) {
    go(bf16_t{});
  } else {
    go(f16_t{});
  }
  prof_end(s, 2.0 * p.B * p.D * p.H * p.W * (double)p.cout * 27.0 * (c0 + c1));
  CWDM_LAUNCHED();
  return CWDM_OK;
}

template __global__ void conv3d_v5_kernel<bf16_t, 0, true>(V4Params);
template __global__ void conv3d_v5_kernel<bf16_t, 1, true>(V4Params);
template __global__ void conv3d_v5_kernel<bf16_t, 0, false>(V4Params);
template __global__ void conv3d_v5_kernel<bf16_t, 1, false>(V4Params);
template __global__ void conv3d_v5_kernel<f16_t, 0, true>(V4Params);
template __global__ void conv3d_v5_kernel<f16_t, 1, true>(V4Params);
template __global__ void conv3d_v5_kernel<f16_t, 0, false>(V4Params);
template __global__ void conv3d_v5_kernel<f16_t, 1, false>(V4Params);
template __global__ void conv3d_v5_kernel<bf16_t, 0, false, 4>(V4Params);
template __global__ void conv3d_v5_kernel<bf16_t, 0, false, 8>(V4Params);
template __global__ void conv3d_v5_kernel<f16_t, 0, false, 4>(V4Params);
template __global__ void conv3d_v5_kernel<f16_t, 0, false, 8>(V4Params);
template __global__ void conv3d_v5s_kernel<0, true>(V4Params);
template __global__ void conv3d_v5s_kernel<1, true>(V4Params);
template __global__ void conv3d_v5s_kernel<0, false>(V4Params);
template __global__ void conv3d_v5s_kernel<1, false>(V4Params);

}

extern "C" int cwdm_debug_v5_aa(int on) {
  if (on < 0) return cwdm::g_v5_aa_launches.load(std::memory_order_relaxed);
  return cwdm::g_v5_aa.exchange(on > 2 ? 2 : on);
}

extern "C" int cwdm_debug_v5_aa_timeout(int extra, int spin) {
  CWDM_REQUIRE(extra >= 0 && spin >= 0, CWDM_E_INVALID, "cwdm_debug_v5_aa_timeout: extra, spin >= 0");
  cwdm::g_v5_aa_extra.store(extra);
  cwdm::g_v5_aa_spin.store(spin);
  return CWDM_OK;
}

extern "C" int cwdm_device_status(int clear) {
  unsigned v = 0;
  CWDM_HIP(hipDeviceSynchronize());
  CWDM_HIP(hipMemcpyFromSymbol(&v, HIP_SYMBOL(cwdm::g_cwdm_dev_err), sizeof(v), 0, hipMemcpyDeviceToHost));
  if (clear && v) {
    const unsigned z = 0;
    CWDM_HIP(hipMemcpyToSymbol(HIP_SYMBOL(cwdm::g_cwdm_dev_err), &z, sizeof(z), 0, hipMemcpyHostToDevice));
  }
  return (int)v;
}

extern "C" int cwdm_debug_v5_grid(int n) {
  CWDM_REQUIRE(n >= 0, CWDM_E_INVALID, "cwdm_debug_v5_grid: n >= 0");
  return cwdm::g_v5_grid.exchange(n);
}
```

### fast-cwdm_amd/csrc/internal.hpp

```cpp
#pragma once
#include <atomic>
#include <vector>

#include "common.hpp"

namespace cwdm {

extern std::atomic<int> g_conv_path;
extern std::atomic<unsigned long long*> g_stamps;

int legacy_conv3d_forward(const cwdm_conv3d_desc* d, cwdm_stream_t stream);
extern thread_local std::vector<PackJob>* g_pack_batch;
int pack_batch_run(std::vector<PackJob>& jobs, int dtype, PackJob* table, std::vector<PackJob>& cache, hipStream_t s);

bool head_eligible(const cwdm_conv3d_desc* d);
int head_conv_forward(const cwdm_conv3d_desc* d, hipStream_t s);
bool head_sampler_eligible(const cwdm_conv3d_desc* d, const cwdm_sampler_args* a);
int head_sampler_forward(const cwdm_conv3d_desc* d, const cwdm_sampler_args* a, hipStream_t s);
int head_split3_prep(const float* x, const float* gn, int64_t B, int64_t V, int C, void* x3, hipStream_t s);
int head_split3_pack(const float* w, int cout, int cin, float* tmp, void* out, hipStream_t s, int k);
int split3_prep(const float* x0, int c0, const float* x1, int c1, const float* gn, int64_t B, int64_t V, int cm,
                void* x3, hipStream_t s);

bool pw_eligible(const cwdm_conv3d_desc* d);
int pw_forward(const cwdm_conv3d_desc* d, hipStream_t s);
bool pw_gapply_ok(const cwdm_conv3d_desc* d);
bool pw_split_eligible(const cwdm_conv3d_desc* d);
int pw_split_forward(const cwdm_conv3d_desc* d, hipStream_t s);

bool v4_eligible(const cwdm_conv3d_desc* d);
int64_t v4_items(const cwdm_conv3d_desc* d);
int v4_ksplit(const cwdm_conv3d_desc* d);
int64_t v4_workspace_bytes(const cwdm_conv3d_desc* d);
int conv3d_v4_forward(const cwdm_conv3d_desc* d, hipStream_t s);
int v4_launch(const cwdm_conv3d_desc* d, const void* a0, int c0, const void* a1, int c1, int a0_cm,
              const void* res, int rmode, void* partial, hipStream_t s);
bool gbwd_grid_ok(const cwdm_conv3d_desc* d);
bool apply_skip_ok(int dtype, int C, int cout, int64_t B, int64_t vpb);
int gn_apply_skip(const void* x0, int c0, const void* x1, int c1, const float* gn, int64_t B, int64_t vpb, int dtype,
                  const void* wskip, int cout, void* act, void* skip, hipStream_t s);
int gnfin_flush(const cwdm_conv3d_desc* d, hipStream_t s);
extern thread_local void* g_act_keep;
extern thread_local int g_act_kept;
struct ActKeepScope {
  void* ptr;
  explicit ActKeepScope(void* p) : ptr(p) { g_act_keep = p; g_act_kept = 0; }
  ~ActKeepScope() { g_act_keep = nullptr; }
  bool used() const { return g_act_kept != 0; }
};

bool v5_eligible(const cwdm_conv3d_desc* d, bool gn);
int v5_aa_units(const cwdm_conv3d_desc* d, int* lead);
extern thread_local int g_stats_wg;
extern thread_local int64_t g_stats_rows;

bool sg_eligible(const cwdm_conv3d_desc* d);
int sg_ksplit(const cwdm_conv3d_desc* d);
bool sg_skip_eligible(const cwdm_conv3d_desc* d);
int sg_skip_ksplit(const cwdm_conv3d_desc* d);
int sg_skip_launch(const cwdm_conv3d_desc* d, void* out, void* partial, hipStream_t s);
int64_t ksplit_slice_voxels(const cwdm_conv3d_desc* d);
int64_t sg_sync_bytes(int ksplit);
int64_t plan_sync_bytes();
unsigned* plan_aa_counters();
extern thread_local unsigned* g_sg_sync;
struct SgSyncScope {
  SgSyncScope(void* block) { g_sg_sync = reinterpret_cast<unsigned*>(block); }
  ~SgSyncScope() { g_sg_sync = nullptr; }
};
extern thread_local bool g_sg_fp32x;
struct SgFp32xScope {
  SgFp32xScope() { g_sg_fp32x = true; }
  ~SgFp32xScope() { g_sg_fp32x = false; }
};

int launch_time_embed(const float* t, int B, int mc, const float* w1, const float* b1, const float* w2,
                      const float* b2, float* temb, hipStream_t s);
int launch_emb_proj(const float* temb, int B, int E, const float* W, const float* bias, int R, float* out,
                    hipStream_t s);
int launch_emb_bwd(const float* dEb, int R, int n, int B, const float* temb, int E, const float* W, float* dw,
                   float* db, float* dcb, float* dsil, hipStream_t s, int acc);
int launch_temb_bwd(const float* t, int B, int mc, const float* w1, const float* b1, const float* w2,
                    const float* temb, const float* dsil, float* dw1, float* db1, float* dw2, float* db2,
                    hipStream_t s);
int gn_silu_bwd_impl(const void* x0, int c0, const void* x1, int c1, const void* du, int du_mode, const float* ss,
                     const float* mr, const float* gamma, int groups, int64_t B, int64_t d, int64_t h, int64_t w,
                     int dtype, void* dx0, int acc0, void* dx1, int acc1, float* dgamma, float* dbeta, void* ws,
                     int64_t ws_bytes, float* chs, int64_t chs_stride, cwdm_stream_t stream, int acc_affine,
                     const float* pre_part = nullptr, int pre_nblk = 0, const float** coef_out = nullptr);
int gb_part_reduce(const float* part, int nblk, int C, int64_t B, int slices, float* out, hipStream_t s);
int haar_nd_synth_add(int dtype, int64_t B, int64_t d, int64_t h, int64_t w, int C, const void* L, int64_t l_vs,
                      float lll, const void* H, int64_t h_vs, float high, void* fine, int acc, hipStream_t s);
int haar_nd_anal_add(int dtype, int64_t B, int64_t d, int64_t h, int64_t w, int C, const void* fine, void* L,
                     int64_t l_vs, float lll, int accL, void* H, int64_t h_vs, float high, int accH, hipStream_t s);
int sampler2_launch(const cwdm_sampler_args* a, hipStream_t s);

}
```

### fast-cwdm_amd/csrc/unet_plan.cpp

```cpp
#include <hip/hip_runtime.h>

#include <algorithm>
#include <cstring>
#include <mutex>
#include <string>
#include <cstdlib>
#include <vector>

#include "internal.hpp"

using namespace cwdm;

namespace {

constexpr int64_t kAlign = 256;
inline int64_t align_up(int64_t v) { return (v + kAlign - 1) / kAlign * kAlign; }

struct Param { std::string name; std::vector<int64_t> shape; int64_t numel() const { int64_t n = 1; for (auto s : shape) n *= s; return n; } };

struct Tensor {
  int level, channels;
  int stats_kind = 0;
};

struct GnStep {
  int src0, src1;
  int gamma_p, beta_p;
  int64_t gamma_off, beta_off;
  int channels;
  int level;
  int ss_id;
};

struct ConvStep {
  int a0, a1, amode, gn;
  int w_p, b_p;
  int64_t w_off;
  int cin_a;
  int sb0, sb1;
  int ws_p, wsb_p;
  int64_t wsk_off;
  int cin_b;
  int bias_kind;
  int64_t bias_off;
  int emb_w_p, emb_b_p;
  int res, rmode;
  int out;
  int cout;
  int level;
  bool stats;
  int skip_conv = -1;
  int64_t wsplit_off = -1;
  int64_t hsplit_off = -1;
  int64_t xsplit_off = -1;
  int64_t xsplit_sk_off = -1;
  int s2 = 0;
};

struct S2dStep {
  int src, out, level_out, channels;
};

struct PoolStep {
  int src, ss_id, out_h, out_x, level_out, channels;
};

struct HaarStep {
  int src, high_in, out, high_out;
  int inverse, all8;
  float lll_scale, high_scale;
  int emb_row;
  bool stats;
  int level;
};

struct Step { int kind; int idx; };

struct Block {
  int g1, pool, c1, g2, c2;
  int x0, x1;
  int updown;
  int p_begin, p_end;
  int emb_k;
  int hh = -1, hx = -1;
};

}

struct CopyJob {
  float* dst;
  const float* a;
  const float* b;
  long long n, blk0;
};

struct cwdm_unet {
  cwdm_unet_config cfg;
  cwdm::PackJob* pack_tab = nullptr;
  cwdm::PackJob* bwd_tab = nullptr;
  CopyJob* copy_tab = nullptr;
  size_t pack_cap = 0, bwd_cap = 0, copy_cap = 0;
  std::vector<cwdm::PackJob> pack_cache, bwd_cache;
  std::vector<CopyJob> copy_cache;
  int E = 0;
  std::vector<Param> params;
  std::vector<Tensor> tensors;
  std::vector<GnStep> gns;
  std::vector<ConvStep> convs;
  std::vector<PoolStep> pools;
  std::vector<S2dStep> s2ds;
  std::vector<HaarStep> haars;
  std::vector<Step> steps;
  struct Alias { std::string name; int owner, before; };
  std::vector<Alias> aliases;
  std::vector<int> trace;
  std::vector<int> trace_level;
  int input_tensor = -1;
  int R = 0;
  std::vector<int> emb_rows_w, emb_rows_b, emb_rows_cb;
  std::vector<int> emb_rows_off, emb_rows_n;
  int te_w1, te_b1, te_w2, te_b2;
  std::vector<Block> blocks;
  int head_g = -1, head_c = -1, head_p_begin = 0;
  std::vector<int64_t> goff;
  int64_t grad_numel = 0;
  std::vector<int64_t> dg_off, dgs_off;
  int64_t packed_bwd_bytes = 0;
  std::vector<char> ginit;
  int64_t off_te_w1, off_te_b1, off_te_w2, off_te_b2, off_emb_w, off_emb_b;
  int64_t packed_bytes = 0;
  int64_t split3_tmp = -1;
  bool profiling = false;
  std::vector<hipEvent_t> ev;
  std::vector<double> ev_flops;
  std::vector<cwdm::ProfHook> hooks;
  int ev_used = 0;
// ... 286 lines not shown
          h = resblock(p + ".0", h, -1, ch, 0);
          alias_from.clear();
          h = resblock(p + ".1", h, -1, ch, 6, sk);
          --level;
        }
        u->trace.push_back(h); u->trace_level.push_back(level);
        ++idx;
      }
    }
    for (int i = 0; i < c.num_res_blocks; ++i) {
      h = resblock("out_res." + std::to_string(i) + ".0", h, -1, ch, 0);
      u->trace.push_back(h); u->trace_level.push_back(level);
    }
  }
  for (int l = 0; l < nl && !c.use_freq; ++l) {
    const int mult = c.channel_mult[l];
    for (int r = 0; r < c.num_res_blocks; ++r) {
      h = resblock("input_blocks." + std::to_string(idx) + ".0", h, -1, mult * mc, 0);
      ch = mult * mc;
      stack.push_back(h);
      u->trace.push_back(h); u->trace_level.push_back(level);
      ++idx;
    }
    if (l != nl - 1) {
      const std::string p = "input_blocks." + std::to_string(idx) + ".0";
      h = c.resblock_updown ? resblock(p, h, -1, ch, 2) : resample_layer(p + ".op", h, 1);
      ++level;
      stack.push_back(h);
      u->trace.push_back(h); u->trace_level.push_back(level);
      ++idx;
    }
  }
  if (!c.use_freq) {
    h = resblock("middle_block.0", h, -1, ch, 0);
    u->trace.push_back(h); u->trace_level.push_back(level);
    h = resblock("middle_block.1", h, -1, ch, 0);
    u->trace.push_back(h); u->trace_level.push_back(level);
    idx = 0;
  }
  for (int l = nl - 1; l >= 0 && !c.use_freq; --l) {
    const int mult = c.channel_mult[l];
    for (int i = 0; i <= c.num_res_blocks; ++i) {
      int skip = stack.back();
      stack.pop_back();
      h = resblock("output_blocks." + std::to_string(idx) + ".0", h, skip, mc * mult, 0);
      ch = mc * mult;
      u->trace.push_back(h); u->trace_level.push_back(level);
      if (l && i == c.num_res_blocks) {
        const std::string p = "output_blocks." + std::to_string(idx) + ".1";
        h = c.resblock_updown ? resblock(p, h, -1, ch, 1) : resample_layer(p + ".conv", h, 0);
        --level;
        u->trace.push_back(h); u->trace_level.push_back(level);
      }
      ++idx;
    }
  }
  u->head_p_begin = (int)u->params.size();
  int g = gn_step("out.0", h, -1, 0);
  u->head_g = g;
  ConvStep co{};
  conv_params("out.2", c.out_channels, ch, 3, &co.w_p, &co.b_p);
  co.a0 = h; co.a1 = -1; co.amode = 0; co.gn = g; co.cin_a = ch;
  co.sb0 = co.sb1 = -1; co.ws_p = co.wsb_p = -1; co.cin_b = 0;
  co.bias_kind = 0; co.res = -1; co.rmode = -1; co.cout = c.out_channels; co.level = 0; co.stats = false;
  co.out = -1;
  u->convs.push_back(co);
  u->head_c = (int)u->convs.size() - 1;
  u->steps.push_back({1, (int)u->convs.size() - 1});
  u->trace.push_back(-1); u->trace_level.push_back(0);

  int64_t off = 0;
  auto take = [&](int64_t bytes) { int64_t o = off; off = align_up(off + bytes); return o; };
  u->off_te_w1 = take(u->params[u->te_w1].numel() * 4);
  u->off_te_b1 = take(u->params[u->te_b1].numel() * 4);
  u->off_te_w2 = take(u->params[u->te_w2].numel() * 4);
  u->off_te_b2 = take(u->params[u->te_b2].numel() * 4);
  u->off_emb_w = take((int64_t)u->R * E * 4);
  u->off_emb_b = take((int64_t)u->R * 4);
  int64_t split3_max = 0;
  for (auto& cs : u->convs) {
    cs.w_off = take(cwdm_conv3d_packed_bytes(cs.cout, cs.cin_a, 3, c.dtype));
    if (c.mfma_split && c.dtype == CWDM_F32 && !cs.s2 && cs.cout % 64 == 0 && cs.cin_a % 16 == 0)
      cs.wsplit_off = take(cwdm_conv3d_packed_split_bytes(cs.cout, cs.cin_a));
    if (c.mfma_split && c.dtype == CWDM_F32 && &cs == &u->convs[u->head_c] && cs.a1 < 0 && cs.amode == 0 &&
        cs.gn >= 0 && cs.cout <= 16 && cs.cin_a % 32 == 0 && 3 * cs.cin_a <= 256) {
      cs.hsplit_off = take(cwdm_conv3d_packed_bytes(cs.cout, 3 * cs.cin_a, 3, CWDM_BF16));
      split3_max = std::max(split3_max, (int64_t)3 * cs.cout * cs.cin_a * 27 * 4);
    }
    if (c.mfma_split && c.dtype == CWDM_F32 && !cs.s2 && cs.level >= 2 && cs.amode <= 1 &&
        cs.cout % 64 == 0 && cs.cin_a % 32 == 0) {
      cs.xsplit_off = take(cwdm_conv3d_packed_bytes(cs.cout, 3 * cs.cin_a, 3, CWDM_BF16));
      split3_max = std::max(split3_max, (int64_t)3 * cs.cout * cs.cin_a * 27 * 4);
      if (cs.ws_p >= 0 && cs.cin_b % 32 == 0) {
        cs.xsplit_sk_off = take(cwdm_conv3d_packed_bytes(cs.cout, 3 * cs.cin_b, 1, CWDM_BF16));
        split3_max = std::max(split3_max, (int64_t)3 * cs.cout * cs.cin_b * 4);
      }
    }
    if (cs.ws_p >= 0) cs.wsk_off = take(cwdm_conv3d_packed_bytes(cs.cout, cs.cin_b, 1, c.dtype));
    if (cs.bias_kind == 0) cs.bias_off = take((int64_t)cs.cout * 4);
  }
  for (auto& gs : u->gns) {
    gs.gamma_off = take((int64_t)gs.channels * 4);
    gs.beta_off = take((int64_t)gs.channels * 4);
  }
  if (split3_max > 0) u->split3_tmp = take(split3_max);
  u->packed_bytes = off;

  int64_t go = 0;
  for (const auto& pr : u->params) { u->goff.push_back(go); go += pr.numel(); }
  u->grad_numel = go;
  const int ck = ck_of(c.dtype);
  int64_t bo = 0;
  auto takeb = [&](int64_t bytes) { int64_t o = bo; bo = align_up(bo + bytes); return o; };
  for (size_t i = 0; i < u->convs.size(); ++i) {
    const auto& cs = u->convs[i];
    const int cpad = (int)((cs.cout + ck - 1) / ck * ck);
    u->dg_off.push_back(i == 0 ? -1 : takeb(cwdm_conv3d_packed_bytes(cs.cin_a, cpad, 3, c.dtype)));
    u->dgs_off.push_back(cs.ws_p >= 0 ? takeb(cwdm_conv3d_packed_bytes(cs.cin_b, cpad, 1, c.dtype)) : -1);
  }
  u->packed_bwd_bytes = bo;
}

struct Layout {
  int64_t temb, ebias, split, split_bytes, sync;
  int64_t skipbuf = 0;
  std::vector<char> skip_fused;
  std::vector<int64_t> t_off, s_off, s_parts;
  std::vector<int64_t> ss_off, mr_off;
  int64_t total;
  std::vector<int64_t> keep_off;
  int64_t train_total;
};

cwdm_conv3d_desc conv_shape(const cwdm_unet* u, const ConvStep& cs, int64_t B, int64_t D, int64_t H, int64_t W) {
  cwdm_conv3d_desc d{};
  d.dtype = u->cfg.dtype;
  d.B = B; d.D = D >> cs.level; d.H = H >> cs.level; d.W = W >> cs.level;
  d.cout = cs.cout;
  d.a_c0 = u->tensors[cs.a0].channels;
  d.a_c1 = cs.a1 >= 0 ? u->tensors[cs.a1].channels : 0;
  d.a_mode = cs.amode;
  d.a_w = reinterpret_cast<const void*>(1);
  if (cs.gn >= 0) d.a_gn = reinterpret_cast<const float*>(1);
  if (cs.ws_p >= 0) {
    d.b_c0 = u->tensors[cs.sb0].channels;
    d.b_c1 = cs.sb1 >= 0 ? u->tensors[cs.sb1].channels : 0;
    d.b_w = reinterpret_cast<const void*>(1);
  }
  d.res_mode = cs.rmode;
  d.out_dtype = cs.out < 0 ? CWDM_F32 : u->cfg.dtype;
  if (cs.wsplit_off >= 0) d.a_w_split = reinterpret_cast<const void*>(1);
  return d;
}

struct XsgPlan {
  bool ok = false;
  bool sk_sg = false;
  cwdm_conv3d_desc e{};
  cwdm_conv3d_desc ek{};
  int64_t x3_bytes = 0, skip_bytes = 0, total = 0;
};
XsgPlan xsg_plan(const cwdm_unet* u, const ConvStep& cs, const cwdm_conv3d_desc& d) {
  XsgPlan x;
  if (cs.xsplit_off < 0 || d.res_mode > 1 || (d.b_w && d.res_mode >= 0)) return x;
  const int64_t sv = cs.amode == 1 ? (d.D / 2) * (d.H / 2) * (d.W / 2) : d.D * d.H * d.W;
  const int C = d.a_c0 + d.a_c1;
// ... 194 lines not shown
}

extern "C" int cwdm_unet_num_aliases(const cwdm_unet* u) { return u ? (int)u->aliases.size() : -1; }

extern "C" int cwdm_unet_alias_info(const cwdm_unet* u, int i, char* name, int cap, int* owner, int* before) {
  CWDM_REQUIRE(u && i >= 0 && i < (int)u->aliases.size(), CWDM_E_INVALID, "cwdm_unet_alias_info: bad index");
  if (name && cap > 0) {
    std::strncpy(name, u->aliases[i].name.c_str(), cap - 1);
    name[cap - 1] = 0;
  }
  if (owner) *owner = u->aliases[i].owner;
  if (before) *before = u->aliases[i].before;
  return CWDM_OK;
}

extern "C" int64_t cwdm_unet_packed_bytes(const cwdm_unet* u) { return u ? u->packed_bytes : -1; }

template <typename J>
static int ensure_table(J*& tab, size_t& cap, size_t n) {
  if (n <= cap) return CWDM_OK;
  if (tab) CWDM_HIP(hipFree(tab));
  tab = nullptr;
  CWDM_HIP(hipMalloc(reinterpret_cast<void**>(&tab), n * sizeof(J)));
  cap = n;
  return CWDM_OK;
}

static int copy_batch_run(cwdm_unet* u, std::vector<CopyJob>& jobs, hipStream_t s) {
  if (jobs.empty()) return CWDM_OK;
  long long blk = 0;
  for (auto& j : jobs) {
    j.blk0 = blk;
    blk += (j.n + 1023) / 1024;
  }
  int rc;
  if ((rc = ensure_table(u->copy_tab, u->copy_cap, jobs.size()))) return rc;
  if (u->copy_cache.size() != jobs.size() ||
      std::memcmp(u->copy_cache.data(), jobs.data(), jobs.size() * sizeof(CopyJob))) {
    CWDM_HIP(hipMemcpyAsync(u->copy_tab, jobs.data(), jobs.size() * sizeof(CopyJob), hipMemcpyHostToDevice, s));
    CWDM_HIP(hipStreamSynchronize(s));
    u->copy_cache = jobs;
  }
  hipLaunchKernelGGL(cwdm::copy_batch_kernel, dim3((unsigned)blk), dim3(256), 0, s, u->copy_tab, (int)jobs.size());
  CWDM_LAUNCHED();
  return CWDM_OK;
}

struct PackBatchScope {
  explicit PackBatchScope(std::vector<cwdm::PackJob>* v) { cwdm::g_pack_batch = v; }
  ~PackBatchScope() { cwdm::g_pack_batch = nullptr; }
};

extern "C" int cwdm_unet_pack(const cwdm_unet* uc, const float* const* P, void* packed, cwdm_stream_t stream) {
  CWDM_REQUIRE(uc && P && packed, CWDM_E_INVALID, "cwdm_unet_pack: null pointer");
  cwdm_unet* u = const_cast<cwdm_unet*>(uc);
  hipStream_t s = (hipStream_t)stream;
  auto* base = reinterpret_cast<unsigned char*>(packed);
  std::vector<CopyJob> cj;
  auto cp = [&](int pi, int64_t off) {
    cj.push_back(CopyJob{reinterpret_cast<float*>(base + off), P[pi], nullptr, u->params[pi].numel(), 0});
  };
  cp(u->te_w1, u->off_te_w1);
  cp(u->te_b1, u->off_te_b1);
  cp(u->te_w2, u->off_te_w2);
  cp(u->te_b2, u->off_te_b2);
  float* ew = reinterpret_cast<float*>(base + u->off_emb_w);
  float* eb = reinterpret_cast<float*>(base + u->off_emb_b);
  for (size_t k = 0; k < u->emb_rows_w.size(); ++k) {
    const int64_t o = u->emb_rows_off[k], n = u->emb_rows_n[k];
    cj.push_back(CopyJob{ew + o * u->E, P[u->emb_rows_w[k]], nullptr, n * u->E, 0});
    cj.push_back(CopyJob{eb + o, P[u->emb_rows_b[k]], u->emb_rows_cb[k] < 0 ? nullptr : P[u->emb_rows_cb[k]], n, 0});
  }
  std::vector<cwdm::PackJob> jobs;
  int rc;
  {
    PackBatchScope scope(&jobs);
    for (const auto& cs : u->convs) {
      if (cs.s2) {
        if ((rc = cwdm_conv3d_pack_s2(P[cs.w_p], cs.cout, cs.cin_a / 8, u->cfg.dtype, base + cs.w_off, 0, stream)))
          return rc;
      } else if ((rc = cwdm_conv3d_pack(P[cs.w_p], cs.cout, cs.cin_a, 3, u->cfg.dtype, base + cs.w_off, stream))) {
        return rc;
      }
      if (cs.wsplit_off >= 0 &&
          (rc = cwdm_conv3d_pack_split(P[cs.w_p], cs.cout, cs.cin_a, base + cs.wsplit_off, stream)))
        return rc;
      if (cs.ws_p >= 0 &&
          (rc = cwdm_conv3d_pack(P[cs.ws_p], cs.cout, cs.cin_b, 1, u->cfg.dtype, base + cs.wsk_off, stream)))
        return rc;
      if (cs.bias_kind == 0)
        cj.push_back(CopyJob{reinterpret_cast<float*>(base + cs.bias_off), P[cs.b_p],
                             cs.wsb_p >= 0 ? P[cs.wsb_p] : nullptr, cs.cout, 0});
    }
  }
  for (const auto& cs : u->convs) {
    float* tmp = reinterpret_cast<float*>(base + u->split3_tmp);
    for (const int64_t o : {cs.hsplit_off, cs.xsplit_off})
      if (o >= 0 && (rc = cwdm::head_split3_pack(P[cs.w_p], cs.cout, cs.cin_a, tmp, base + o, s, 3))) return rc;
    if (cs.xsplit_sk_off >= 0 &&
        (rc = cwdm::head_split3_pack(P[cs.ws_p], cs.cout, cs.cin_b, tmp, base + cs.xsplit_sk_off, s, 1)))
      return rc;
  }
  for (const auto& g : u->gns) {
    cp(g.gamma_p, g.gamma_off);
    cp(g.beta_p, g.beta_off);
  }
  if ((rc = copy_batch_run(u, cj, s))) return rc;
  if ((rc = ensure_table(u->pack_tab, u->pack_cap, jobs.size()))) return rc;
  return cwdm::pack_batch_run(jobs, u->cfg.dtype, u->pack_tab, u->pack_cache, s);
}

extern "C" int64_t cwdm_unet_workspace_bytes(const cwdm_unet* u, int64_t B, int64_t D, int64_t H, int64_t W) {
  if (!u || B <= 0 || D <= 0 || H <= 0 || W <= 0) return -1;
  return layout(u, B, D, H, W).total;
}

extern "C" int64_t cwdm_unet_train_workspace_bytes(const cwdm_unet* u, int64_t B, int64_t D, int64_t H, int64_t W) {
  const int64_t n = cwdm_unet_workspace_bytes(u, B, D, H, W);
  if (n < 0) return n;
  return layout(u, B, D, H, W).train_total;
}

extern "C" double cwdm_unet_flops(const cwdm_unet* u, int64_t B, int64_t D, int64_t H, int64_t W) {
  if (!u) return -1;
  double f = 0;
  for (const auto& cs : u->convs) {
    const double v = (double)B * (D >> cs.level) * (H >> cs.level) * (W >> cs.level);
    f += 2.0 * v * cs.cout * (27.0 * (cs.s2 ? cs.cin_a / 8 : cs.cin_a) + cs.cin_b);
  }
  return f;
}

static int unet_forward_impl(cwdm_unet* u, const void* packed, const void* x, const float* t, float* out,
                             int64_t B, int64_t D, int64_t H, int64_t W, void* ws, int64_t ws_bytes,
                             cwdm_stream_t stream, const cwdm_sampler_args* samp, int* fused) {
  CWDM_REQUIRE(u && packed && x && t && out && ws, CWDM_E_INVALID, "cwdm_unet_forward: null pointer");
  CWDM_REQUIRE(B > 0 && D > 0 && H > 0 && W > 0, CWDM_E_SHAPE, "cwdm_unet_forward: empty grid");
  const int64_t div = int64_t(1) << (u->cfg.num_levels - (u->cfg.use_freq ? 0 : 1));
  CWDM_REQUIRE(D % div == 0 && H % div == 0 && W % div == 0, CWDM_E_SHAPE,
               "cwdm_unet_forward: every subband edge must be divisible by " + std::to_string(div));
  Layout L = layout(u, B, D, H, W);
  CWDM_REQUIRE(ws_bytes >= L.total, CWDM_E_WORKSPACE,
               "cwdm_unet_forward: workspace too small (need " + std::to_string(L.total) + " bytes)");
  const bool keep = L.train_total > L.total && ws_bytes >= L.train_total;
  hipStream_t s = (hipStream_t)stream;
  auto* pk = reinterpret_cast<const unsigned char*>(packed);
  auto* wb = reinterpret_cast<unsigned char*>(ws);
  CWDM_HIP(hipMemsetAsync(wb + L.sync, 0, cwdm::plan_sync_bytes(), s));
  SgSyncScope sync_scope(wb + L.sync);
  float* temb = reinterpret_cast<float*>(wb + L.temb);
  float* ebias = reinterpret_cast<float*>(wb + L.ebias);
  int rc;
  const float* f = nullptr;
  auto P = [&](int64_t off) { return reinterpret_cast<const float*>(pk + off); };
  if ((rc = launch_time_embed(t, (int)B, u->cfg.model_channels, P(u->off_te_w1), P(u->off_te_b1), P(u->off_te_w2),
                              P(u->off_te_b2), temb, s)))
    return rc;
  if ((rc = launch_emb_proj(temb, (int)B, u->E, P(u->off_emb_w), P(u->off_emb_b), u->R, ebias, s))) return rc;
  (void)f;
  auto tptr = [&](int id) -> const void* {
    if (id < 0) return nullptr;
    if (id == u->input_tensor) return x;
    return wb + L.t_off[id];
  };
  int conv_i = 0;
  struct ProfReset {
// ... 14 lines not shown
      for (int k = 0; k < 4; ++k) u->hooks[i].ev[k >> 1][k & 1] = u->ev[4 * i + k];
    u->ev_used = 0;
  }
  static const bool fin_on = env_not0("CWDM_GNFIN");
  static const int stats_wg = env_not0("CWDM_STATS_WG");
  std::vector<int64_t> srows(L.s_parts);
  struct StatsWgScope {
    StatsWgScope() { cwdm::g_stats_wg = stats_wg; cwdm::g_stats_rows = 0; }
    ~StatsWgScope() { cwdm::g_stats_wg = 0; cwdm::g_stats_rows = 0; }
  } stats_wg_scope;
  int fin_pend = -1;
  auto fin_args = [&](int gi, cwdm::GnFinFuse& f) {
    const auto& g = u->gns[gi];
    f.s0 = reinterpret_cast<const float*>(wb + L.s_off[g.src0]); f.p0 = srows[g.src0];
    f.c0 = u->tensors[g.src0].channels;
    f.s1 = g.src1 >= 0 ? reinterpret_cast<const float*>(wb + L.s_off[g.src1]) : nullptr;
    f.p1 = g.src1 >= 0 ? srows[g.src1] : 0; f.c1 = g.src1 >= 0 ? u->tensors[g.src1].channels : 0;
    f.gamma = P(g.gamma_off); f.beta = P(g.beta_off); f.groups = u->cfg.num_groups;
    f.voxels = (D >> g.level) * (H >> g.level) * (W >> g.level); f.eps = 1e-5f;
    f.ss = reinterpret_cast<float*>(wb + L.ss_off[g.ss_id]); f.mr = reinterpret_cast<float*>(wb + L.mr_off[g.ss_id]);
    f.B = B;
    f.used = false;
  };
  auto flush_fin = [&]() -> int {
    if (fin_pend < 0) return CWDM_OK;
    cwdm::GnFinFuse f{};
    fin_args(fin_pend, f);
    fin_pend = -1;
    return cwdm_gn_finalize(f.s0, f.p0, f.c0, f.s1, f.p1, f.c1, f.gamma, f.beta, f.groups, B, f.voxels, f.eps, f.ss,
                            f.mr, stream);
  };
  for (const auto& st : u->steps) {
    if (fin_pend >= 0 && !(st.kind == 1 && u->convs[st.idx].gn == u->gns[fin_pend].ss_id) && (rc = flush_fin()))
      return rc;
    if (st.kind == 2) {
      const auto& ps = u->pools[st.idx];
      const int lv = ps.level_out;
      if ((rc = cwdm_gn_silu_pool(tptr(ps.src), ps.channels, reinterpret_cast<const float*>(wb + L.ss_off[ps.ss_id]),
                                  B, D >> lv, H >> lv, W >> lv, u->cfg.dtype, wb + L.t_off[ps.out_h],
                                  wb + L.t_off[ps.out_x], stream)))
        return rc;
      continue;
    }
    if (st.kind == 3) {
      const auto& sd = u->s2ds[st.idx];
      const int lv = sd.level_out;
      if ((rc = cwdm_space_to_depth(tptr(sd.src), sd.channels, B, D >> lv, H >> lv, W >> lv, u->cfg.dtype,
                                    wb + L.t_off[sd.out], 1, 0, stream)))
        return rc;
      continue;
    }
    if (st.kind == 4) {
      const auto& hs = u->haars[st.idx];
      const int lv = hs.level;
      cwdm_haar_nd_desc a{};
      a.dtype = u->cfg.dtype;
      a.B = B; a.d = D >> lv; a.h = H >> lv; a.w = W >> lv;
      a.C = u->tensors[hs.src].channels;
      a.inverse = hs.inverse; a.all8 = hs.all8;
      a.src = tptr(hs.src); a.high_in = tptr(hs.high_in);
      a.lll_scale = hs.lll_scale; a.high_scale = hs.high_scale;
      a.out = wb + L.t_off[hs.out];
      a.high_out = hs.high_out >= 0 ? wb + L.t_off[hs.high_out] : nullptr;
      a.bias = hs.emb_row >= 0 ? ebias + hs.emb_row : nullptr;
      a.bias_bstride = u->R;
      a.stats = hs.stats ? reinterpret_cast<float*>(wb + L.s_off[hs.out]) : nullptr;
      if ((rc = cwdm_haar_nd(&a, stream))) return rc;
      continue;
    }
    if (st.kind == 0) {
      fin_pend = st.idx;
      if (!fin_on && (rc = flush_fin())) return rc;
      continue;
    }
    const auto& cs = u->convs[st.idx];
    cwdm_conv3d_desc d = conv_shape(u, cs, B, D, H, W);
    d.a0 = tptr(cs.a0);
    d.a1 = tptr(cs.a1);
    d.workspace = wb + L.split;
    d.ws_bytes = L.split_bytes;
    d.a_gn = cs.gn >= 0 ? reinterpret_cast<const float*>(wb + L.ss_off[cs.gn]) : nullptr;
    d.a_w = pk + cs.w_off;
    d.a_w_split = cs.wsplit_off >= 0 ? pk + cs.wsplit_off : nullptr;
    if (cs.ws_p >= 0) {
      d.b0 = tptr(cs.sb0); d.b_c0 = u->tensors[cs.sb0].channels;
      d.b1 = tptr(cs.sb1); d.b_c1 = cs.sb1 >= 0 ? u->tensors[cs.sb1].channels : 0;
      d.b_w = pk + cs.wsk_off;
    }
    if (cs.bias_kind == 0) { d.bias = P(cs.bias_off); d.bias_bstride = 0; }
    else { d.bias = ebias + cs.bias_off; d.bias_bstride = u->R; }
    d.res = tptr(cs.res); d.res_mode = cs.rmode;
    if (cs.out < 0) { d.out = out; d.out_dtype = CWDM_F32; }
    else { d.out = wb + L.t_off[cs.out]; d.out_dtype = u->cfg.dtype; }
    d.stats = (cs.stats && cs.out >= 0) ? reinterpret_cast<float*>(wb + L.s_off[cs.out]) : nullptr;
    if (u->profiling) cwdm::g_prof = &u->hooks[conv_i];
    auto skip_pass_at = [&](int ci) {
      if (!L.skip_fused[ci]) return false;
      if (keep) return true;
      const cwdm_conv3d_desc dc = conv_shape(u, u->convs[ci], B, D, H, W);
      return !cwdm::v5_eligible(&dc, true);
    };
    if (skip_pass_at(st.idx)) {
      const auto& c2 = u->convs[cs.skip_conv];
      const int64_t vpb = d.D * d.H * d.W;
      void* act = keep && L.keep_off[st.idx] >= 0 ? wb + L.keep_off[st.idx] : wb + L.split;
      if ((rc = flush_fin())) return rc;
      if ((rc = cwdm::gn_apply_skip(d.a0, d.a_c0, d.a1, d.a_c1, d.a_gn, B, vpb, u->cfg.dtype, pk + c2.wsk_off,
                                    c2.cout, act, wb + L.skipbuf, s)))
        return rc;
      void* part = wb + L.split + ((B * vpb * (d.a_c0 + d.a_c1) * es + 255) & ~(int64_t)255);
      if ((rc = cwdm::v4_launch(&d, act, d.a_c0 + d.a_c1, nullptr, 0, 1, d.res, d.res_mode, part, s))) return rc;
    } else {
      if (cs.ws_p >= 0 && st.idx > 0 && u->convs[st.idx - 1].skip_conv == st.idx && skip_pass_at(st.idx - 1)) {
        d.b0 = d.b1 = nullptr; d.b_c0 = d.b_c1 = 0; d.b_w = nullptr;
        d.res = wb + L.skipbuf; d.res_mode = 0;
      }
      const int64_t x3_bytes = B * d.D * d.H * d.W * 3 * d.a_c0 * 2;
      if (samp && cs.out < 0 && cwdm::head_sampler_eligible(&d, samp)) {
        if ((rc = flush_fin())) return rc;
        if ((rc = cwdm::head_sampler_forward(&d, samp, s))) return rc;
        if (fused) *fused = 1;
      } else if (cs.hsplit_off >= 0 && !keep && d.a_gn && x3_bytes <= L.split_bytes) {
        if ((rc = flush_fin())) return rc;
        void* x3 = wb + L.split;
        if ((rc = cwdm::head_split3_prep(reinterpret_cast<const float*>(d.a0), d.a_gn, B, d.D * d.H * d.W, d.a_c0, x3,
                                          s)))
          return rc;
        cwdm_conv3d_desc e = d;
        e.dtype = CWDM_BF16;
        e.a0 = x3; e.a_c0 = 3 * d.a_c0; e.a1 = nullptr; e.a_c1 = 0;
        e.a_gn = nullptr; e.a_w = pk + cs.hsplit_off; e.a_w_split = nullptr;
        e.workspace = nullptr; e.ws_bytes = 0;
        if ((rc = cwdm_conv3d_forward(&e, stream))) return rc;
      } else if (XsgPlan xp = keep ? XsgPlan{} : xsg_plan(u, cs, d); xp.ok && xp.total <= L.split_bytes) {
        if ((rc = flush_fin())) return rc;
        unsigned char* x3 = wb + L.split;
        const void* res = d.res;
        int rmode = d.res_mode;
        SgFp32xScope fx;
        void* part = x3 + xp.x3_bytes + xp.skip_bytes;
        if (d.b_w && xp.sk_sg) {
          if ((rc = cwdm::split3_prep(reinterpret_cast<const float*>(d.b0), d.b_c0, reinterpret_cast<const float*>(d.b1),
                                      d.b_c1, nullptr, B, d.D * d.H * d.W, 0, x3, s)))
            return rc;
          cwdm_conv3d_desc k = xp.ek;
          k.b0 = x3; k.b_w = pk + cs.xsplit_sk_off;
          if ((rc = cwdm::sg_skip_launch(&k, x3 + xp.x3_bytes, cwdm::sg_skip_ksplit(&k) > 1 ? part : nullptr, s)))
            return rc;
          res = x3 + xp.x3_bytes; rmode = 0;
        } else if (d.b_w) {
          cwdm_conv3d_desc k = d;
          k.a0 = k.a1 = nullptr; k.a_c0 = k.a_c1 = 0; k.a_gn = nullptr; k.a_w = nullptr; k.a_mode = 0;
          k.bias = nullptr; k.bias_bstride = 0; k.stats = nullptr; k.res = nullptr; k.res_mode = -1;
          k.out = x3 + xp.x3_bytes; k.out_dtype = CWDM_F32;
          k.workspace = nullptr; k.ws_bytes = 0;
          if ((rc = cwdm::pw_split_eligible(&k) ? cwdm::pw_split_forward(&k, s) : cwdm_conv3d_forward(&k, stream)))
            return rc;
          res = k.out; rmode = 0;
        }
        const int64_t sv = cs.amode == 1 ? (d.D / 2) * (d.H / 2) * (d.W / 2) : d.D * d.H * d.W;
        if ((rc = cwdm::split3_prep(reinterpret_cast<const float*>(d.a0), d.a_c0, reinterpret_cast<const float*>(d.a1),
                                    d.a_c1, d.a_gn, B, sv, 1, x3, s)))
          return rc;
        cwdm_conv3d_desc e = xp.e;
        e.a0 = x3; e.a1 = nullptr; e.a_w = pk + cs.xsplit_off;
        e.bias = d.bias; e.bias_bstride = d.bias_bstride;
// ... 634 lines not shown
```

### fast-cwdm_amd/cwdm_hip/_lib.py

```python
import ctypes
import os

_HERE = os.path.dirname(os.path.abspath(__file__))
LIB_PATH = os.environ.get("CWDM_LIB", os.path.join(_HERE, "..", "lib", "libcwdm.so"))

CWDM_F32 = 0
CWDM_BF16 = 1
CWDM_F64 = 2
CWDM_F16 = 3

E_INVALID, E_SHAPE, E_HIP, E_WORKSPACE, E_INDEX, E_UNSUPPORTED = -1, -2, -3, -4, -5, -6

i64 = ctypes.c_int64
vp = ctypes.c_void_p
I64x3 = i64 * 3
I64x4 = i64 * 4


class SamplerArgs(ctypes.Structure):
    _fields_ = [
        ("model_out", vp), ("mo_s", I64x3),
        ("x_t", vp), ("xt_s", I64x3),
        ("x_prev", vp), ("xp_s", I64x3),
        ("noise", vp), ("nz_s", I64x3),
        ("pred_xstart", vp), ("px_s", I64x3),
        ("mirror", vp), ("mirror_dtype", ctypes.c_int), ("mr_s", I64x3),
        ("coef", vp), ("t", vp),
        ("T", i64), ("B", i64), ("d", i64), ("h", i64), ("w", i64),
        ("clip_denoised", ctypes.c_int),
        ("mean_type", ctypes.c_int),
        ("update", ctypes.c_int),
        ("per_band", ctypes.c_int),
        ("levels", ctypes.c_int),
        ("noise_philox", ctypes.c_int),
        ("reserved0", ctypes.c_int),
        ("noise_seed", ctypes.c_uint64),
    ]


class ConvDesc(ctypes.Structure):
    _fields_ = [
        ("dtype", ctypes.c_int),
        ("B", i64), ("D", i64), ("H", i64), ("W", i64),
        ("cout", ctypes.c_int),
        ("a0", vp), ("a_c0", ctypes.c_int),
        ("a1", vp), ("a_c1", ctypes.c_int),
        ("a_mode", ctypes.c_int),
        ("a_gn", vp),
        ("a_w", vp),
        ("b0", vp), ("b_c0", ctypes.c_int),
        ("b1", vp), ("b_c1", ctypes.c_int),
        ("b_w", vp),
        ("bias", vp), ("bias_bstride", i64),
        ("res", vp), ("res_mode", ctypes.c_int),
        ("out", vp), ("out_dtype", ctypes.c_int),
        ("stats", vp),
        ("workspace", vp), ("ws_bytes", i64),
        ("out1", vp), ("out_c0", ctypes.c_int),
        ("accumulate", ctypes.c_int),
        ("a_w_split", vp),
    ]


class WgradDesc(ctypes.Structure):
    _fields_ = [
        ("dtype", ctypes.c_int),
        ("B", i64), ("D", i64), ("H", i64), ("W", i64),
        ("ksize", ctypes.c_int),
        ("u0", vp), ("u_c0", ctypes.c_int),
        ("u1", vp), ("u_c1", ctypes.c_int),
        ("u_mode", ctypes.c_int),
        ("u_gn", vp),
        ("dy", vp), ("dy_cs", ctypes.c_int), ("cout", ctypes.c_int),
        ("dw", vp),
        ("workspace", vp),
        ("u_cm", ctypes.c_int),
        ("ws_bytes", i64),
    ]


class UNetConfig(ctypes.Structure):
    _fields_ = [
        ("in_channels", ctypes.c_int), ("model_channels", ctypes.c_int),
        ("out_channels", ctypes.c_int), ("num_res_blocks", ctypes.c_int),
        ("num_levels", ctypes.c_int), ("channel_mult", ctypes.c_int * 8),
        ("num_groups", ctypes.c_int), ("dtype", ctypes.c_int),
        ("resblock_updown", ctypes.c_int), ("use_freq", ctypes.c_int),
        ("mfma_split", ctypes.c_int),
    ]


class HaarNdDesc(ctypes.Structure):
    _fields_ = [
        ("dtype", ctypes.c_int),
        ("B", i64), ("d", i64), ("h", i64), ("w", i64),
        ("C", ctypes.c_int),
        ("inverse", ctypes.c_int),
        ("src", vp), ("high_in", vp),
        ("lll_scale", ctypes.c_float), ("high_scale", ctypes.c_float),
        ("out", vp), ("all8", ctypes.c_int), ("high_out", vp),
        ("bias", vp), ("bias_bstride", i64),
        ("stats", vp),
    ]


_PROTOS = {
    "cwdm_version": (ctypes.c_int, []),
    "cwdm_last_error": (ctypes.c_char_p, []),
    "cwdm_build_id": (ctypes.c_char_p, []),
    "cwdm_haar_dwt3d": (ctypes.c_int, [vp, i64, i64, i64, i64, i64, vp, ctypes.c_int, ctypes.POINTER(i64),
                                       ctypes.c_int, vp]),
    "cwdm_haar_idwt3d": (ctypes.c_int, [vp, ctypes.c_int, ctypes.POINTER(i64), i64, i64, i64, i64, i64, vp,
                                        ctypes.c_int, ctypes.c_int, vp]),
    "cwdm_haar_idwt3d_planes": (ctypes.c_int, [ctypes.POINTER(vp), ctypes.c_int, ctypes.POINTER(i64), i64, i64, i64,
                                               i64, i64, vp, vp]),
    "cwdm_prepare_batch": (ctypes.c_int, [vp, vp, vp, vp, vp, i64, i64, i64, i64, vp, ctypes.c_int, vp, i64, vp, vp,
                                          vp]),
    "cwdm_prepare_batch2": (ctypes.c_int, [vp, vp, vp, vp, vp, i64, i64, i64, i64, vp, ctypes.c_int, vp, i64, vp, vp,
                                           vp]),
    "cwdm_sampler_step": (ctypes.c_int, [ctypes.POINTER(SamplerArgs), vp]),
    "cwdm_quantile_workspace_bytes": (i64, []),
    "cwdm_quantiles": (ctypes.c_int, [vp, ctypes.c_int, i64, ctypes.POINTER(i64), ctypes.c_int,
                                      ctypes.POINTER(ctypes.c_double), vp, vp, i64, vp]),
    "cwdm_volume_prepare": (ctypes.c_int, [vp, ctypes.c_int, i64, i64, i64, vp, i64, i64, vp, ctypes.c_int, vp]),
    "cwdm_sample_finish": (ctypes.c_int, [vp, i64, i64, i64, i64, vp, i64, vp, vp]),
    "cwdm_copy3": (ctypes.c_int, [vp, ctypes.c_int, ctypes.POINTER(i64), vp, ctypes.c_int, ctypes.POINTER(i64),
                                  i64, i64, i64, vp]),
    "cwdm_conv3d_packed_bytes": (i64, [ctypes.c_int, ctypes.c_int, ctypes.c_int, ctypes.c_int]),
    "cwdm_conv3d_pack": (ctypes.c_int, [vp, ctypes.c_int, ctypes.c_int, ctypes.c_int, ctypes.c_int, vp, vp]),
    "cwdm_conv3d_packed_split_bytes": (i64, [ctypes.c_int, ctypes.c_int]),
    "cwdm_conv3d_pack_split": (ctypes.c_int, [vp, ctypes.c_int, ctypes.c_int, vp, vp]),
    "cwdm_conv3d_pack_dgrad": (ctypes.c_int, [vp, ctypes.c_int, ctypes.c_int, ctypes.c_int, ctypes.c_int, vp, vp]),
    "cwdm_conv3d_parts": (i64, [ctypes.c_int, i64, i64, i64, ctypes.c_int]),
    "cwdm_space_to_depth": (ctypes.c_int, [vp, ctypes.c_int, i64, i64, i64, i64, ctypes.c_int, vp, ctypes.c_int,
                                           ctypes.c_int, vp]),
    "cwdm_conv3d_pack_s2": (ctypes.c_int, [vp, ctypes.c_int, ctypes.c_int, ctypes.c_int, vp, ctypes.c_int, vp]),
    "cwdm_conv3d_s2_fold_dw": (ctypes.c_int, [vp, ctypes.c_int, ctypes.c_int, vp, ctypes.c_int, vp]),
    "cwdm_conv3d_forward": (ctypes.c_int, [ctypes.POINTER(ConvDesc), vp]),
    "cwdm_conv3d_workspace_bytes": (i64, [ctypes.POINTER(ConvDesc)]),
    "cwdm_gn_finalize": (ctypes.c_int, [vp, i64, ctypes.c_int, vp, i64, ctypes.c_int, vp, vp, ctypes.c_int, i64, i64,
                                        ctypes.c_float, vp, vp, vp]),
    "cwdm_gn_silu_pool": (ctypes.c_int, [vp, ctypes.c_int, vp, i64, i64, i64, i64, ctypes.c_int, vp, vp, vp]),
    "cwdm_gn_apply": (ctypes.c_int, [vp, ctypes.c_int, vp, ctypes.c_int, vp, i64, i64, ctypes.c_int, vp, vp]),
    "cwdm_conv3d_set_path": (ctypes.c_int, [ctypes.c_int]),
    "cwdm_debug_v5_grid": (ctypes.c_int, [ctypes.c_int]),
    "cwdm_debug_v5_aa": (ctypes.c_int, [ctypes.c_int]),
    "cwdm_debug_v5_aa_timeout": (ctypes.c_int, [ctypes.c_int, ctypes.c_int]),
    "cwdm_device_status": (ctypes.c_int, [ctypes.c_int]),
    "cwdm_debug_gn_fin_apply": (ctypes.c_int, [vp, i64, ctypes.c_int, vp, i64, ctypes.c_int, vp, vp, ctypes.c_int,
                                               i64, i64, ctypes.c_float, vp, vp, ctypes.c_int, vp, vp, vp, vp]),
    "cwdm_debug_head2": (ctypes.c_int, [ctypes.c_int]),
    "cwdm_debug_pw_lt": (ctypes.c_int, [ctypes.c_int]),
    "cwdm_debug_conv_stamps": (ctypes.c_int, [vp]),
    "cwdm_conv3d_wgrad": (ctypes.c_int, [ctypes.POINTER(WgradDesc), vp]),
    "cwdm_conv3d_wgrad_workspace_bytes": (i64, [ctypes.c_int, ctypes.c_int, ctypes.c_int]),
    "cwdm_gn_silu_bwd_workspace_bytes": (i64, [ctypes.c_int, i64, i64, i64, i64]),
    "cwdm_gn_silu_bwd": (ctypes.c_int, [vp, ctypes.c_int, vp, ctypes.c_int, vp, ctypes.c_int, vp, vp, vp,
                                        ctypes.c_int, i64, i64, i64, i64, ctypes.c_int, vp, ctypes.c_int, vp,
                                        ctypes.c_int, vp, vp, vp, i64, vp]),
    "cwdm_resample_add": (ctypes.c_int, [vp, vp, ctypes.c_int, i64, i64, i64, i64, ctypes.c_int, ctypes.c_int,
                                         ctypes.c_int, vp]),
    "cwdm_channel_sum_workspace_bytes": (i64, [i64, i64, ctypes.c_int]),
    "cwdm_channel_sum": (ctypes.c_int, [vp, ctypes.c_int, i64, i64, ctypes.c_int, ctypes.c_int, vp, i64, vp, vp,
                                        vp, i64, vp]),
    "cwdm_adamw": (ctypes.c_int, [vp, vp, vp, vp, i64, ctypes.c_double, ctypes.c_double, ctypes.c_double,
                                  ctypes.c_double, ctypes.c_double, i64, vp]),
    "cwdm_adamw_device_step": (ctypes.c_int, [vp, vp, vp, vp, i64, ctypes.c_double, ctypes.c_double, ctypes.c_double,
                                               ctypes.c_double, ctypes.c_double, vp, vp, vp]),
    "cwdm_adamw_maxabs": (ctypes.c_int, [vp, vp, vp, vp, i64, ctypes.c_double, ctypes.c_double, ctypes.c_double,
                                         ctypes.c_double, ctypes.c_double, i64, vp, vp]),
    "cwdm_unet_create": (ctypes.c_int, [ctypes.POINTER(UNetConfig), ctypes.POINTER(vp)]),
    "cwdm_unet_destroy": (None, [vp]),
    "cwdm_unet_num_params": (ctypes.c_int, [vp]),
    "cwdm_unet_num_aliases": (ctypes.c_int, [vp]),
    "cwdm_unet_alias_info": (ctypes.c_int, [vp, ctypes.c_int, ctypes.c_char_p, ctypes.c_int,
                                            ctypes.POINTER(ctypes.c_int), ctypes.POINTER(ctypes.c_int)]),
    "cwdm_haar_nd_parts": (i64, [i64, i64, i64]),
    "cwdm_haar_nd": (ctypes.c_int, [ctypes.POINTER(HaarNdDesc), vp]),
    "cwdm_wavelet2_analysis": (ctypes.c_int, [vp, i64, i64, i64, i64, vp, ctypes.c_int, i64, i64, ctypes.c_int, vp]),
    "cwdm_wavelet2_synthesis": (ctypes.c_int, [vp, i64, i64, i64, i64, i64, i64, ctypes.c_int, vp, vp]),
    "cwdm_unet_param_info": (ctypes.c_int, [vp, ctypes.c_int, ctypes.c_char_p, ctypes.c_int, ctypes.POINTER(i64),
                                            ctypes.POINTER(ctypes.c_int)]),
    "cwdm_unet_packed_bytes": (i64, [vp]),
    "cwdm_unet_pack": (ctypes.c_int, [vp, ctypes.POINTER(vp), vp, vp]),
    "cwdm_unet_workspace_bytes": (i64, [vp, i64, i64, i64, i64]),
    "cwdm_unet_train_workspace_bytes": (i64, [vp, i64, i64, i64, i64]),
    "cwdm_unet_forward": (ctypes.c_int, [vp, vp, vp, vp, vp, i64, i64, i64, i64, vp, i64, vp]),
    "cwdm_unet_forward_step": (ctypes.c_int, [vp, vp, vp, vp, ctypes.POINTER(SamplerArgs), i64, i64, i64, i64,
                                              vp, i64, ctypes.POINTER(ctypes.c_int), vp]),
    "cwdm_unet_trace_count": (ctypes.c_int, [vp]),
    "cwdm_unet_trace_info": (ctypes.c_int, [vp, ctypes.c_int, i64, i64, i64, i64, ctypes.POINTER(i64),
                                            ctypes.POINTER(ctypes.c_int), ctypes.POINTER(ctypes.c_int)]),
    "cwdm_unet_flops": (ctypes.c_double, [vp, i64, i64, i64, i64]),
    "cwdm_unet_packed_bwd_bytes": (i64, [vp]),
    "cwdm_unet_pack_bwd": (ctypes.c_int, [vp, ctypes.POINTER(vp), vp, vp]),
    "cwdm_unet_grad_workspace_bytes": (i64, [vp, i64, i64, i64, i64]),
    "cwdm_unet_backward_segments": (ctypes.c_int, [vp]),
    "cwdm_unet_segment_range": (ctypes.c_int, [vp, ctypes.c_int, ctypes.POINTER(i64), ctypes.POINTER(i64)]),
    "cwdm_unet_backward": (ctypes.c_int, [vp, vp, vp, vp, vp, vp, vp, i64, i64, i64, i64, vp, i64, vp, i64,
                                          ctypes.c_int, ctypes.c_int, vp]),
    "cwdm_unet_backward_flops": (ctypes.c_double, [vp, i64, i64, i64, i64]),
    "cwdm_unet_set_profiling": (ctypes.c_int, [vp, ctypes.c_int]),
    "cwdm_unet_profile_read": (ctypes.c_int, [vp, ctypes.POINTER(ctypes.c_double), ctypes.POINTER(ctypes.c_double),
                                              ctypes.POINTER(ctypes.c_int)]),
}

EXPORTED = tuple(_PROTOS)

_lib = None


class CwdmError(RuntimeError):
    pass


def lib():
    global _lib
    if _lib is None:
        if not os.path.exists(LIB_PATH):
            raise OSError(f"libcwdm.so not found at {LIB_PATH}: run __graft_entry__.build() "
                          f"or `make -C fast-cwdm_amd/csrc` (no CPU fallback exists)")
        L = ctypes.CDLL(LIB_PATH)
        for name, (res, args) in _PROTOS.items():
            fn = getattr(L, name)
            fn.restype = res
            fn.argtypes = args
        check_build_id(L)
        _lib = L
    return _lib
# ... 41 lines not shown
```

### include/cwdm.h

```cpp
#ifndef CWDM_H_
#define CWDM_H_

#include <stddef.h>
#include <stdint.h>

#ifdef __cplusplus
extern "C" {
#endif

typedef struct ihipStream_t* cwdm_stream_t;

enum {
  CWDM_F32 = 0,
  CWDM_BF16 = 1,
  CWDM_F64 = 2,
  CWDM_F16 = 3
};

enum {
  CWDM_OK = 0,
  CWDM_E_INVALID = -1,
  CWDM_E_SHAPE = -2,
  CWDM_E_HIP = -3,
  CWDM_E_WORKSPACE = -4,
// ... 22 lines not shown
  int C;
  int inverse;
  const void* src;
  const void* high_in;
  float lll_scale, high_scale;
  void* out;
  int all8;
  void* high_out;
  const float* bias; int64_t bias_bstride;
  float* stats;
} cwdm_haar_nd_desc;
int64_t cwdm_haar_nd_parts(int64_t d, int64_t h, int64_t w);
int cwdm_haar_nd(const cwdm_haar_nd_desc* desc, cwdm_stream_t stream);

int cwdm_prepare_batch(const float* target, const float* c1, const float* c2, const float* c3,
                       const float* eps_img, int64_t B, int64_t D, int64_t H, int64_t W,
                       const float* coef, int per_band, const int64_t* t, int64_t T, float* x_in, float* x0,
                       cwdm_stream_t stream);

int cwdm_prepare_batch2(const float* target, const float* c1, const float* c2, const float* c3,
                        const float* eps_img, int64_t B, int64_t D, int64_t H, int64_t W,
                        const float* coef, int per_band, const int64_t* t, int64_t T, float* x_in, float* x0,
                        cwdm_stream_t stream);

typedef struct {
  const float* model_out; int64_t mo_s[3];
  const float* x_t;       int64_t xt_s[3];
  float* x_prev;          int64_t xp_s[3];
  const float* noise;     int64_t nz_s[3];
  float* pred_xstart;     int64_t px_s[3];
  void* mirror; int mirror_dtype; int64_t mr_s[3];
  const float* coef;
  const int64_t* t;
  int64_t T, B, d, h, w;
  int clip_denoised;
  int mean_type;
  int update;
  int per_band;
  int levels;
  int noise_philox;
  int reserved0;
  uint64_t noise_seed;
} cwdm_sampler_args;
int cwdm_sampler_step(const cwdm_sampler_args* args, cwdm_stream_t stream);

int cwdm_wavelet2_analysis(const float* x, int64_t B, int64_t D, int64_t H, int64_t W, void* out, int out_dtype,
                           int64_t out_bs, int64_t out_vs, int out_c0, cwdm_stream_t stream);
int cwdm_wavelet2_synthesis(const float* coef, int64_t B, int64_t d, int64_t h, int64_t w, int64_t c_bs,
                            int64_t c_vs, int c_c0, float* out, cwdm_stream_t stream);

int64_t cwdm_quantile_workspace_bytes(void);
int cwdm_quantiles(const void* x, int dtype, int64_t n, const int64_t* ranks , int nranks,
                   const double* gammas , double* out, void* workspace, int64_t ws_bytes,
                   cwdm_stream_t stream);
int cwdm_volume_prepare(const void* x, int dtype, int64_t X, int64_t Y, int64_t Z, const double* lohi,
                        int64_t crop, int64_t out_z, void* out, int out_dtype, cwdm_stream_t stream);
int cwdm_sample_finish(const float* sample, int64_t B, int64_t d, int64_t h, int64_t w, const float* mask,
                       int64_t keep_z, float* out, cwdm_stream_t stream);

int cwdm_copy3(const void* src, int src_dtype, const int64_t* src_s ,
               void* dst, int dst_dtype, const int64_t* dst_s ,
               int64_t B, int64_t C, int64_t V, cwdm_stream_t stream);

typedef struct {
  int dtype;
  int64_t B, D, H, W;
  int cout;
  const void* a0; int a_c0;
  const void* a1; int a_c1;
  int a_mode;
  const float* a_gn;
  const void* a_w;
  const void* b0; int b_c0;
  const void* b1; int b_c1;
  const void* b_w;
  const float* bias; int64_t bias_bstride;
  const void* res; int res_mode;
  void* out; int out_dtype;
  float* stats;
  void* workspace; int64_t ws_bytes;
  void* out1; int out_c0;
  int accumulate;
  const void* a_w_split;
} cwdm_conv3d_desc;
int64_t cwdm_conv3d_packed_bytes(int cout, int cin, int ksize, int dtype);
int64_t cwdm_conv3d_packed_split_bytes(int cout, int cin);
int cwdm_conv3d_pack_split(const float* w_oidhw, int cout, int cin, void* packed, cwdm_stream_t stream);
int cwdm_conv3d_pack(const float* w_oidhw, int cout, int cin, int ksize, int dtype,
                     void* packed, cwdm_stream_t stream);
int cwdm_conv3d_pack_dgrad(const float* w_oidhw, int cout, int cin, int ksize, int dtype,
                           void* packed, cwdm_stream_t stream);
int cwdm_space_to_depth(const void* x, int C, int64_t B, int64_t d, int64_t h, int64_t w, int dtype, void* out,
                        int to_depth, int accumulate, cwdm_stream_t stream);
int cwdm_conv3d_pack_s2(const float* w_oidhw, int cout, int cin, int dtype, void* packed, int transpose,
                        cwdm_stream_t stream);
int cwdm_conv3d_s2_fold_dw(const float* dwe, int cout, int cin, float* dw, int accumulate, cwdm_stream_t stream);
int64_t cwdm_conv3d_parts(int dtype, int64_t D, int64_t H, int64_t W, int cout);
int64_t cwdm_conv3d_workspace_bytes(const cwdm_conv3d_desc* desc);
int cwdm_conv3d_forward(const cwdm_conv3d_desc* desc, cwdm_stream_t stream);

int cwdm_gn_finalize(const float* stats0, int64_t parts0, int c0,
                     const float* stats1, int64_t parts1, int c1,
                     const float* gamma, const float* beta, int groups,
                     int64_t B, int64_t voxels, float eps,
                     float* scale_shift, float* mean_rstd ,
                     cwdm_stream_t stream);

int cwdm_gn_silu_pool(const void* x, int C, const float* gn, int64_t B, int64_t d, int64_t h, int64_t w,
                      int dtype, void* out_h, void* out_x, cwdm_stream_t stream);

int cwdm_conv3d_set_path(int path);

int cwdm_debug_v5_grid(int n);

int cwdm_debug_v5_aa(int on);

int cwdm_debug_v5_aa_timeout(int extra, int spin);

enum { CWDM_DEV_E_AA_TIMEOUT = 1 };
int cwdm_device_status(int clear);

int cwdm_debug_gn_fin_apply(const float* stats0, int64_t parts0, int c0, const float* stats1, int64_t parts1,
                            int c1, const float* gamma, const float* beta, int groups, int64_t B, int64_t voxels,
                            float eps, const void* x0, const void* x1, int dtype, float* scale_shift,
                            float* mean_rstd, void* out_cm, cwdm_stream_t stream);

int cwdm_debug_head2(int mode);

int cwdm_debug_pw_lt(int on);

int cwdm_debug_conv_stamps(void* buf);

int cwdm_gn_apply(const void* x0, int c0, const void* x1, int c1, const float* scale_shift, int64_t B,
                  int64_t voxels, int dtype, void* out, cwdm_stream_t stream);

typedef struct {
  int dtype;
  int64_t B, D, H, W;
  int ksize;
  const void* u0; int u_c0;
  const void* u1; int u_c1;
  int u_mode;
  const float* u_gn;
  const void* dy; int dy_cs; int cout;
  float* dw;
  void* workspace;
  int u_cm;
  int64_t ws_bytes;
} cwdm_wgrad_desc;
int64_t cwdm_conv3d_wgrad_workspace_bytes(int cout, int cin, int ksize);
int cwdm_conv3d_wgrad(const cwdm_wgrad_desc* desc, cwdm_stream_t stream);

int64_t cwdm_gn_silu_bwd_workspace_bytes(int C, int64_t B, int64_t d, int64_t h, int64_t w);
int cwdm_gn_silu_bwd(const void* x0, int c0, const void* x1, int c1, const void* du, int du_mode,
                     const float* scale_shift, const float* mean_rstd, const float* gamma, int groups,
                     int64_t B, int64_t d, int64_t h, int64_t w, int dtype,
                     void* dx0, int acc0, void* dx1, int acc1, float* dgamma, float* dbeta,
                     void* workspace, int64_t ws_bytes, cwdm_stream_t stream);

int cwdm_resample_add(void* dst, const void* src, int C, int64_t B, int64_t d, int64_t h, int64_t w,
                      int mode, int accumulate, int dtype, cwdm_stream_t stream);

int64_t cwdm_channel_sum_workspace_bytes(int64_t B, int64_t V, int C);
int cwdm_channel_sum(const void* src, int dtype, int64_t B, int64_t V, int C, int cs,
                     float* out_bc, int64_t bc_stride, float* out_c, float* out_c2,
                     void* workspace, int64_t ws_bytes, cwdm_stream_t stream);

int cwdm_adamw(float* p, const float* g, float* m, float* v, int64_t n, double lr, double beta1, double beta2,
               double eps, double weight_decay, int64_t step, cwdm_stream_t stream);

int cwdm_adamw_maxabs(float* p, const float* g, float* m, float* v, int64_t n, double lr, double beta1, double beta2,
                      double eps, double weight_decay, int64_t step, float* maxabs, cwdm_stream_t stream);

int cwdm_adamw_device_step(float* p, const float* g, float* m, float* v, int64_t n, double lr, double beta1,
                           double beta2, double eps, double weight_decay, double* step, const float* found_inf,
                           cwdm_stream_t stream);

typedef struct cwdm_unet cwdm_unet;
typedef struct {
  int in_channels, model_channels, out_channels, num_res_blocks;
  int num_levels;
  int channel_mult[8];
  int num_groups;
  int dtype;
  int resblock_updown;
  int use_freq;
  int mfma_split;
} cwdm_unet_config;

int cwdm_unet_create(const cwdm_unet_config* cfg, cwdm_unet** plan);
void cwdm_unet_destroy(cwdm_unet* plan);
int cwdm_unet_num_params(const cwdm_unet* plan);
int cwdm_unet_param_info(const cwdm_unet* plan, int i, char* name, int name_cap,
                         int64_t* shape , int* ndim);
int cwdm_unet_num_aliases(const cwdm_unet* plan);
int cwdm_unet_alias_info(const cwdm_unet* plan, int i, char* name, int name_cap, int* owner, int* before);
int64_t cwdm_unet_packed_bytes(const cwdm_unet* plan);
int cwdm_unet_pack(const cwdm_unet* plan, const float* const* params, void* packed,
// ... 32 lines not shown
```

Measured before the change: 65.75 denoising-steps/s.

## Fuse nearest upsample into conv via per-phase 2x2x2 folded weights

Adds a phase-decomposed path for 3x3x3 convolutions that read a nearest-upsampled (amode 1) input. The kernel reads the low-resolution halo directly and applies pre-summed 2x2x2 weights for each of the 8 output sub-voxel phases. This cuts MFMA work from 27 taps to 8 per output voxel and avoids reading an upsampled activation. It costs an extra packed phase-weight buffer per eligible conv, a new tile mapping and output addressing, and it drops the GN plus upsample kernel instance.

```diff
diff --git a/fast-cwdm_amd/csrc/common.hpp b/fast-cwdm_amd/csrc/common.hpp
--- a/fast-cwdm_amd/csrc/common.hpp
+++ b/fast-cwdm_amd/csrc/common.hpp
@@ -148,7 +148,8 @@
   const float* w;
   void* out;
   long long total;
-  int cout, cin, ntaps, NT, transpose, cin_real, s2_ci0, pad;
+  int cout, cin, ntaps, NT, transpose, cin_real, s2_ci0;
+  int phase;
   long long blk0;
 };
 static_assert(sizeof(PackJob) == 64, "PackJob layout");
diff --git a/fast-cwdm_amd/csrc/conv3d.hip b/fast-cwdm_amd/csrc/conv3d.hip
--- a/fast-cwdm_amd/csrc/conv3d.hip
+++ b/fast-cwdm_amd/csrc/conv3d.hip
@@ -49,6 +49,45 @@
 }
 
 template <typename T>
+__device__ __forceinline__ void pack_phase_elem(const float* __restrict__ w, int cout, int cin, T* __restrict__ out,
+                                                long long i) {
+  constexpr int CK = ConvTr<T>::CK, EPQ = ConvTr<T>::EPQ;
+  const int nch = cin / CK, nct = cout / 64;
+  const int e = i % EPQ;
+  long long r = i / EPQ;
+  const int qp = r % 2;
+  r /= 2;
+  const int n = r % 64;
+  r /= 64;
+  const int tap = r % 8;
+  r /= 8;
+  const int chunk = r % nch;
+  r /= nch;
+  const int ct = r % nct;
+  const int ph = (int)(r / nct);
+  const int q = qp ^ ((n >> 3) & 1);
+  const int co = ct * 64 + n, ci = chunk * CK + q * EPQ + e;
+  auto lo = [](int p, int t) { return t == 0 ? 0 : 1 + p; };
+  auto hi = [](int p, int t) { return t == 0 ? p : 2; };
+  const int pz = ph >> 2, py = (ph >> 1) & 1, px = ph & 1, tz = tap >> 2, ty = (tap >> 1) & 1, tx = tap & 1;
+  const float* wc = w + ((long long)co * cin + ci) * 27;
+  float v = 0.f;
+  for (int kz = lo(pz, tz); kz <= hi(pz, tz); ++kz)
+    for (int ky = lo(py, ty); ky <= hi(py, ty); ++ky)
+      for (int kx = lo(px, tx); kx <= hi(px, tx); ++kx) v += wc[(kz * 3 + ky) * 3 + kx];
+  out[i] = Elem<T>::from_f(v);
+}
+
+template <typename T>
+__global__ void __launch_bounds__(256) pack_phase_kernel(const float* __restrict__ w, int cout, int cin,
+                                                         T* __restrict__ out, long long total) {
+  const long long i = (long long)blockIdx.x * blockDim.x + threadIdx.x;
+  if constexpr (sizeof(T) == 2) {
+    if (i < total) pack_phase_elem<T>(w, cout, cin, out, i);
+  }
+}
+
+template <typename T>
 __global__ void __launch_bounds__(256) pack_kernel(const float* __restrict__ w, int cout, int cin, int ntaps, int NT,
                                                    int nct, T* __restrict__ out, int transpose, int cin_real,
                                                    int s2_ci0) {
@@ -72,9 +111,15 @@
 #pragma unroll
   for (int k = 0; k < 4; ++k) {
     const long long i = base + k * 256 + threadIdx.x;
-    if (i < j.total)
-      pack_elem<T>(j.w, j.cout, j.cin, j.ntaps, j.NT, reinterpret_cast<T*>(j.out), j.transpose, j.cin_real,
-                   j.s2_ci0, i);
+    if (i >= j.total) continue;
+    if constexpr (sizeof(T) == 2) {
+      if (j.phase) {
+        pack_phase_elem<T>(j.w, j.cout, j.cin, reinterpret_cast<T*>(j.out), i);
+        continue;
+      }
+    }
+    pack_elem<T>(j.w, j.cout, j.cin, j.ntaps, j.NT, reinterpret_cast<T*>(j.out), j.transpose, j.cin_real,
+                 j.s2_ci0, i);
   }
 }
 
@@ -260,6 +305,32 @@
   return CWDM_OK;
 }
 
+extern "C" int64_t cwdm_conv3d_packed_phase_bytes(int cout, int cin, int dtype) {
+  if (cout <= 0 || cout % 64 || cin <= 0 || cin % 16 || !dtype_half(dtype)) return -1;
+  return (int64_t)8 * (cout / 64) * (cin / 16) * 8 * 2048;
+}
+
+extern "C" int cwdm_conv3d_pack_phase(const float* w, int cout, int cin, int dtype, void* packed,
+                                      cwdm_stream_t stream) {
+  CWDM_REQUIRE(w && packed, CWDM_E_INVALID, "cwdm_conv3d_pack_phase: null pointer");
+  CWDM_REQUIRE(dtype_half(dtype) && cout > 0 && cout % 64 == 0 && cin > 0 && cin % 16 == 0, CWDM_E_UNSUPPORTED,
+               "cwdm_conv3d_pack_phase: bf16 / fp16, cout % 64 == 0, cin % 16 == 0");
+  const long long total = cwdm_conv3d_packed_phase_bytes(cout, cin, dtype) / 2;
+  if (g_pack_batch) {
+    g_pack_batch->push_back(PackJob{w, packed, total, cout, cin, 8, 64, 0, cin, 0, 1, 0});
+    return CWDM_OK;
+  }
+  const dim3 grid((unsigned)ceil_div(total, 256));
+  if (dtype == CWDM_BF16)
+    hipLaunchKernelGGL(pack_phase_kernel<bf16_t>, grid, dim3(256), 0, (hipStream_t)stream, w, cout, cin,
+                       reinterpret_cast<bf16_t*>(packed), total);
+  else
+    hipLaunchKernelGGL(pack_phase_kernel<f16_t>, grid, dim3(256), 0, (hipStream_t)stream, w, cout, cin,
+                       reinterpret_cast<f16_t*>(packed), total);
+  CWDM_LAUNCHED();
+  return CWDM_OK;
+}
+
 extern "C" int cwdm_conv3d_pack_s2(const float* w, int cout, int cin, int dtype, void* packed, int transpose,
                                    cwdm_stream_t stream) {
   return transpose ? pack_impl(w, 8 * cin, cout, 3, dtype, packed, 1, stream, cin)
@@ -278,7 +349,9 @@
                    hipStream_t s) {
   if (jobs.empty()) return CWDM_OK;
   static const bool tiled_on = env_not0("CWDM_PACK_TILED");
-  auto tiled = [&](const PackJob& j) { return tiled_on && j.s2_ci0 == 0 && j.ntaps <= 27 && j.NT % 32 == 0; };
+  auto tiled = [&](const PackJob& j) {
+    return tiled_on && j.s2_ci0 == 0 && !j.phase && j.ntaps <= 27 && j.NT % 32 == 0;
+  };
   std::stable_partition(jobs.begin(), jobs.end(), tiled);
   size_t nt = 0;
   while (nt < jobs.size() && tiled(jobs[nt])) ++nt;
diff --git a/fast-cwdm_amd/csrc/conv3d_v4.hip b/fast-cwdm_amd/csrc/conv3d_v4.hip
--- a/fast-cwdm_amd/csrc/conv3d_v4.hip
+++ b/fast-cwdm_amd/csrc/conv3d_v4.hip
@@ -331,6 +331,7 @@
   p.accumulate = d->accumulate;
   p.stamps = g_stamps.load(std::memory_order_relaxed);
   if (sg_eligible(d)) return sg_launch(p, d, partial, s);
+  if (v5_phase_ok(d, rmode)) return v5_launch(d, a0, c0, a1, c1, a0_cm, nullptr, nullptr, -1, s, nullptr, true);
   if (v5_eligible(d, false))
     return v5_launch(d, a0, c0, a1, c1, a0_cm, nullptr, res, rmode, s);
   const int S = v4_ksplit(d);
diff --git a/fast-cwdm_amd/csrc/conv3d_v4.hpp b/fast-cwdm_amd/csrc/conv3d_v4.hpp
--- a/fast-cwdm_amd/csrc/conv3d_v4.hpp
+++ b/fast-cwdm_amd/csrc/conv3d_v4.hpp
@@ -51,7 +51,8 @@
 
 int sg_launch(const V4Params& v, const cwdm_conv3d_desc* d, void* partial, hipStream_t s);
 int v5_launch(const cwdm_conv3d_desc* d, const void* a0, int c0, const void* a1, int c1, int a0_cm,
-              const float* agn, const void* res, int rmode, hipStream_t s, const V5Aa* aa = nullptr);
+              const float* agn, const void* res, int rmode, hipStream_t s, const V5Aa* aa = nullptr,
+              bool phase = false);
 
 struct V4Cfg {
   static constexpr int HX = 34, HY = 6, HZ = 6, HV = HX * HY * HZ;
@@ -373,7 +374,7 @@
   }
 }
 
-struct V4Tile { int b, sl, ct, x0, y0, z0, ks, c0, c1; };
+struct V4Tile { int b, sl, ct, x0, y0, z0, ks, c0, c1, ph; };
 __device__ __forceinline__ V4Tile v4_tile_of(const V4Params& p, int it) {
   const int tiles = p.tx * p.ty * p.tz;
   const int nbase = p.nblk / p.ksplit;
@@ -381,6 +382,7 @@
   const int xcd = t & 7, q8 = p.nblk >> 3, r8 = p.nblk & 7;
   int wg = (xcd < r8 ? xcd * (q8 + 1) : r8 * (q8 + 1) + (xcd - r8) * q8) + (t >> 3);
   V4Tile r;
+  r.ph = 0;
   r.ks = wg / nbase;
   wg -= r.ks * nbase;
   r.c0 = r.ks * p.kper;
diff --git a/fast-cwdm_amd/csrc/conv3d_v5.hip b/fast-cwdm_amd/csrc/conv3d_v5.hip
--- a/fast-cwdm_amd/csrc/conv3d_v5.hip
+++ b/fast-cwdm_amd/csrc/conv3d_v5.hip
@@ -57,7 +57,7 @@
 __device__ __forceinline__ V4Tile v5aa_tile_of(const V4Params& p, int it) {
   const int wg = it * (int)gridDim.x + v5aa_pos();
   V4Tile r;
-  r.ks = 0; r.c0 = 0; r.c1 = p.nch; r.b = 0;
+  r.ks = 0; r.c0 = 0; r.c1 = p.nch; r.b = 0; r.ph = 0;
   r.ct = wg % p.nct;
   r.sl = wg / p.nct;
   r.x0 = (r.sl % p.tx) * 32; r.y0 = ((r.sl / p.tx) % p.ty) * 4; r.z0 = (r.sl / (p.tx * p.ty)) * 4;
@@ -76,10 +76,42 @@
   return (unsigned)(z1 < D ? z1 : D) * (unsigned)H * (unsigned)W;
 }
 
+__device__ __forceinline__ V4Tile v5p_tile_of(const V4Params& p, int it) {
+  const int tiles = p.tx * p.ty * p.tz;
+  const int t = blockIdx.x + it * gridDim.x;
+  const int xcd = t & 7, q8 = p.nblk >> 3, r8 = p.nblk & 7;
+  const int wg = (xcd < r8 ? xcd * (q8 + 1) : r8 * (q8 + 1) + (xcd - r8) * q8) + (t >> 3);
+  V4Tile r;
+  r.ks = 0; r.c0 = 0; r.c1 = p.nch;
+  const int per = 8 * p.nct;
+  const int st = wg / per, in = wg - st * per;
+  r.ph = in / p.nct;
+  r.ct = in - r.ph * p.nct;
+  r.b = st / tiles;
+  r.sl = st - r.b * tiles;
+  r.x0 = (r.sl % p.tx) * 32; r.y0 = ((r.sl / p.tx) % p.ty) * 4; r.z0 = (r.sl / (p.tx * p.ty)) * 4;
+  r.ct = __builtin_amdgcn_readfirstlane(r.ct); r.b = __builtin_amdgcn_readfirstlane(r.b);
+  r.sl = __builtin_amdgcn_readfirstlane(r.sl); r.x0 = __builtin_amdgcn_readfirstlane(r.x0);
+  r.y0 = __builtin_amdgcn_readfirstlane(r.y0); r.z0 = __builtin_amdgcn_readfirstlane(r.z0);
+  r.ph = __builtin_amdgcn_readfirstlane(r.ph);
+  return r;
+}
+template <int K>
+__device__ __forceinline__ void v5p_read_step(u32x4 (&av)[6], const unsigned char* hb) {
+  constexpr int G = K / 2, PL = K % 2, TZ = G / 2, TX = G % 2;
+#pragma unroll
+  for (int L = 0; L < 5; ++L)
+    av[L] = *reinterpret_cast<const u32x4*>(hb + (((PL + TZ) * V4Cfg::HY + L) * V4Cfg::HX + TX) * 16);
+}
+#define V5P_WAIT_W(n, w) asm volatile("s_waitcnt vmcnt(" #n ")" : "+v"((w)[0]), "+v"((w)[1]) :: "memory")
+
 template <typename T, int MODE, bool GN, int AA = 0>
 __global__ void __launch_bounds__(512) conv3d_v5_kernel(V4Params p) {
   using C = V4Cfg;
   using T16 = T;
+  constexpr bool PH = MODE == 2;
+  constexpr int HM = MODE == 1 ? 1 : 0;
+  static_assert(!PH || (!GN && AA == 0), "the phase instance reads an activated or raw source");
   constexpr int NI = 10 + (GN ? 1 : 0);
   __shared__ __attribute__((aligned(1024))) unsigned char smem[V5Cfg::SMEM];
 
@@ -88,7 +120,10 @@
   const int nblk = p.nblk;
   const int ntile = (nblk - (AA ? v5aa_pos() : (int)blockIdx.x) + (int)gridDim.x - 1) / (int)gridDim.x;
   if (ntile <= 0) return;
-  auto tile_of = [&](int it) { return AA ? v5aa_tile_of(p, it) : v4_tile_of(p, it); };
+  auto tile_of = [&](int it) {
+    if constexpr (PH) return v5p_tile_of(p, it);
+    else return AA ? v5aa_tile_of(p, it) : v4_tile_of(p, it);
+  };
   const int tiles = p.tx * p.ty * p.tz;
 
   const int G = (int)gridDim.x;
@@ -180,12 +215,24 @@
       v4_gload(w[1], src + 3 * 2048);
       v4_gload(w[2], src + 6 * 2048);
     };
+    auto load_wp = [&](u32x4 (&w)[3], const V4Tile& t, int c, int g) {
+      if (V5_DIAG(4)) return;
+      const unsigned char* src = wlane + (((long long)t.ph * p.nct + t.ct) * p.nch + V5_PHYS(t, c)) * 8 * 2048 +
+                                 ((g >> 1) * 4 + (g & 1)) * 2048;
+      v4_gload(w[0], src);
+      v4_gload(w[1], src + 2 * 2048);
+    };
     const int hlane = hh * (C::HVP * 16) + (zb * (C::HX * C::HY) + lr) * 16;
     f32x16 acc[2][4];
-    u32x4 wr[3][3];
+    u32x4 wr[4][3];
     V4Tile cur = tile_of(0);
-    load_w(wr[0], cur.ct, V5_PHYS(cur, cur.c0), 0);
-    load_w(wr[1], cur.ct, V5_PHYS(cur, cur.c0), 1);
+    if constexpr (PH) {
+      load_wp(wr[0], cur, cur.c0, 0);
+      load_wp(wr[1], cur, cur.c0, 1);
+    } else {
+      load_w(wr[0], cur.ct, V5_PHYS(cur, cur.c0), 0);
+      load_w(wr[1], cur.ct, V5_PHYS(cur, cur.c0), 1);
+    }
     __builtin_amdgcn_s_barrier();
     V5_STAMP(1, tid == 0);
     int gch = 0;
@@ -206,8 +253,31 @@
       }
       auto chunk = [&](auto lastc, int c) {
         constexpr bool LAST = decltype(lastc)::value;
+        u32x4 av[2][6];
+        if constexpr (PH) {
+          const unsigned char* hb = smem + (gch % 3) * C::HALO_B + hlane +
+                                    ((((cur.ph >> 2) * C::HY + ((cur.ph >> 1) & 1)) * C::HX + (cur.ph & 1)) << 4);
+          if (!V5_DIAG(2)) v5p_read_step<0>(av[0], hb);
+#define V5P_STEP(K)                                                                                          \
+          {                                                                                                  \
+            constexpr int GI = (K) / 2, PL = (K) % 2, KN = (K) + 1, BC = (K) & 1;                            \
+            if (PL == 0) {                                                                                   \
+              if (GI + 2 < 4) load_wp(wr[(GI + 2) % 4], cur, c, GI + 2);                                     \
+              else if (!LAST) load_wp(wr[(GI + 2) % 4], cur, c + 1, GI - 2);                                 \
+              else load_wp(wr[(GI + 2) % 4], nxt, nxt.c0, GI - 2);                                           \
+            }                                                                                                \
+            if (KN < 8 && !V5_DIAG(2)) v5p_read_step<KN % 8>(av[BC ^ 1], hb);                                \
+            if (PL == 0) V5P_WAIT_W(4, wr[GI]);                                                              \
+            __builtin_amdgcn_sched_barrier(0);                                                               \
+            _Pragma("unroll") for (int ty = 0; ty < 2; ++ty)                                                 \
+            _Pragma("unroll") for (int m = 0; m < 4; ++m)                                                    \
+              v4_mfma<T>(acc[PL][m], wr[GI][ty], av[BC][m + ty]);                                            \
+            __builtin_amdgcn_sched_barrier(0);                                                               \
+          }
+          V5P_STEP(0) V5P_STEP(1) V5P_STEP(2) V5P_STEP(3) V5P_STEP(4) V5P_STEP(5) V5P_STEP(6) V5P_STEP(7)
+#undef V5P_STEP
+        } else {
         const unsigned char* hb = smem + (gch % 3) * C::HALO_B + hlane;
-        u32x4 av[2][6];
         if (!V5_DIAG(2)) v4_read_step<0>(av[0], hb);
 #define V5_STEP(K)                                                                                           \
         {                                                                                                    \
@@ -233,6 +303,7 @@
         V5_STEP(6) V5_STEP(7) V5_STEP(8) V5_STEP(9) V5_STEP(10) V5_STEP(11)
         V5_STEP(12) V5_STEP(13) V5_STEP(14) V5_STEP(15) V5_STEP(16) V5_STEP(17)
 #undef V5_STEP
+        }
         V5_STAMP(2 + gch, tid == 0 && gch < 16);
         __builtin_amdgcn_s_barrier();
         V5_STAMP(18 + gch, tid == 0 && gch < 16);
@@ -264,8 +335,12 @@
       __builtin_amdgcn_s_barrier();
       cur = nxt;
     }
-    asm volatile("s_waitcnt vmcnt(0)" : "+v"(wr[0][0]), "+v"(wr[0][1]), "+v"(wr[0][2]), "+v"(wr[1][0]), "+v"(wr[1][1]),
-                 "+v"(wr[1][2])::"memory");
+    if constexpr (PH) {
+      asm volatile("s_waitcnt vmcnt(0)" : "+v"(wr[0][0]), "+v"(wr[0][1]), "+v"(wr[1][0]), "+v"(wr[1][1])::"memory");
+    } else {
+      asm volatile("s_waitcnt vmcnt(0)" : "+v"(wr[0][0]), "+v"(wr[0][1]), "+v"(wr[0][2]), "+v"(wr[1][0]),
+                   "+v"(wr[1][1]), "+v"(wr[1][2])::"memory");
+    }
 #ifdef CWDM_CONV_STAMPS
     if (p.stamps && tid == 0) p.stamps[(long long)blockIdx.x * 64 + 51] = __builtin_amdgcn_s_memrealtime();
 #endif
@@ -280,7 +355,7 @@
   int pc = pt.c0;
   auto issue_next = [&](int buf) -> bool {
     if (pit >= ntile) return false;
-    if (!V5_DIAG(1)) v4_issue_halo<T, MODE>(p, pt, V5_PHYS(pt, pc), smem + buf * C::HALO_B, h, lane);
+    if (!V5_DIAG(1)) v4_issue_halo<T, HM>(p, pt, V5_PHYS(pt, pc), smem + buf * C::HALO_B, h, lane);
     if constexpr (GN) {
       if (lane < 32)
         __builtin_amdgcn_global_load_lds(
@@ -335,8 +410,9 @@
       (void)x0; (void)y0; (void)z0; (void)buf;
     }
   };
-  const long long HW = (long long)p.H * p.W, VV = (long long)p.D * HW;
-  const unsigned rowb = (unsigned)p.W * (unsigned)p.cout * 2u, planeb = (unsigned)HW * (unsigned)p.cout * 2u;
+  const long long HW = (long long)p.H * p.W, VV = (long long)p.D * HW * (PH ? 8 : 1);
+  const unsigned rowb = (unsigned)p.W * (unsigned)p.cout * (PH ? 8u : 2u);
+  const unsigned planeb = (unsigned)HW * (unsigned)p.cout * (PH ? 16u : 2u);
   float s1[8], s2[8];
   bool wg_final = false;
   u32x4 dq[8];
@@ -377,8 +453,11 @@
 #pragma unroll
       for (int e = 0; e < 8; ++e) { s1[e] = 0.f; s2[e] = 0.f; }
     }
-    const unsigned obase =
-        ((unsigned)((tt.z0 * p.H + tt.y0) * p.W) + (unsigned)ox) * (unsigned)p.cout * 2u + (unsigned)(tt.ct * 64 + 8 * q) * 2u;
+    const unsigned ovox =
+        PH ? (unsigned)(((2 * tt.z0 + (tt.ph >> 2)) * (2 * p.H) + 2 * tt.y0 + ((tt.ph >> 1) & 1)) * (2 * p.W)) +
+                 (unsigned)(2 * ox + (tt.ph & 1))
+           : (unsigned)((tt.z0 * p.H + tt.y0) * p.W) + (unsigned)ox;
+    const unsigned obase = ovox * (unsigned)p.cout * 2u + (unsigned)(tt.ct * 64 + 8 * q) * 2u;
 #pragma unroll
     for (int k = 0; k < 8; ++k) {
       if (k < k0 || k >= k1) continue;
@@ -437,7 +516,13 @@
                   run[ct * 64 + lane];
           }
         } else {
-          const long long pidx = ((long long)tt.b * tiles + tt.sl) * p.cout + tt.ct * 64 + lane;
+          long long row = (long long)tt.b * tiles + tt.sl;
+          if constexpr (PH) {
+            const int sx = tt.sl % p.tx, sy = (tt.sl / p.tx) % p.ty, sz = tt.sl / (p.tx * p.ty);
+            row = (long long)tt.b * tiles * 8 +
+                  ((2 * sz + (tt.ph >> 2)) * (2 * p.ty) + 2 * sy + ((tt.ph >> 1) & 1)) * (2 * p.tx) + 2 * sx + (tt.ph & 1);
+          }
+          const long long pidx = row * p.cout + tt.ct * 64 + lane;
           *reinterpret_cast<float2*>(p.stats + pidx * 2) = make_float2(su, sq);
         }
       }
@@ -469,7 +554,7 @@
     int pc = pt.c0;
     bool chk = false;
     auto issue_aa = [&](int buf) {
-      v4_issue_halo<T, MODE, C::HVP * 16, true>(p, pt, pc, smem + buf * C::HALO_B, h, lane);
+      v4_issue_halo<T, HM, C::HVP * 16, true>(p, pt, pc, smem + buf * C::HALO_B, h, lane);
       if (pc + 1 < pt.c1) {
         ++pc;
       } else if (pit + 1 < ntile) {
@@ -997,6 +1082,8 @@
 std::atomic<int> g_v5_grid{0};
 std::atomic<int> g_v5_aa{env_int("CWDM_V5_AA", 1)};
 std::atomic<int> g_v5_aa_launches{0};
+std::atomic<int> g_up_phase{env_not0("CWDM_UP_PHASE") ? 1 : 0};
+std::atomic<int> g_up_phase_launches{0};
 std::atomic<int> g_v5_aa_extra{0};
 std::atomic<int> g_v5_aa_spin{0};
 thread_local int g_stats_wg = 0;
@@ -1054,14 +1141,31 @@
   if (d->D * d->H * d->W * d->cout * 2 >= 0xFFFFE000LL) return false;
   if (d->a_c0 + d->a_c1 < 32) return false;
   if (gbwd_grid_ok(d)) return false;
-  static const int ncu = [] {
-    int dev = 0, n = 0;
-    if (hipGetDevice(&dev) != hipSuccess || hipDeviceGetAttribute(&n, hipDeviceAttributeMultiprocessorCount, dev) != hipSuccess)
-      return 256;
-    return n > 0 ? n : 256;
-  }();
+  const int ncu = v5_ncu();
   static const double min_tpc = env_double("CWDM_V5_MIN_TPC", 1.0);
   return path == 2 || (double)v4_items(d) >= min_tpc * ncu;
+}
+
+namespace {
+unsigned v5_grid(long long nblk) {
+  const int cap = g_v5_grid.load(std::memory_order_relaxed);
+  return (unsigned)std::min<long long>(nblk, cap > 0 ? cap : v5_ncu());
+}
+}
+
+bool v5_phase_ok(const cwdm_conv3d_desc* d, int rmode) {
+  if (!d->a_w_phase || !g_up_phase.load(std::memory_order_relaxed)) return false;
+  if (!dtype_half(d->dtype) || d->a_mode != 1 || d->b_w || rmode != -1 || d->res_mode != -1) return false;
+  if (!v5_eligible(d, false)) return false;
+  const int64_t SD = d->D / 2, SH = d->H / 2, SW = d->W / 2;
+  if (SW < kWideMinW || SH % 4 || SD % 4) return false;
+  if (d->stats) {
+    const int64_t stx = (SW + 31) / 32, otx = (d->W + 31) / 32, otiles = otx * (d->H / 4) * (d->D / 4);
+    const long long nblk = (long long)d->B * stx * (SH / 4) * (SD / 4) * (d->cout / 64) * 8;
+    const bool wg = g_stats_wg && d->B == 1 && d->cout / 64 <= 2 && (long long)v5_grid(nblk) <= otiles;
+    if (!wg && otx != 2 * stx) return false;
+  }
+  return true;
 }
 
 int v5_aa_units(const cwdm_conv3d_desc* d, int* lead) {
@@ -1098,23 +1202,26 @@
 }
 
 int v5_launch(const cwdm_conv3d_desc* d, const void* a0, int c0, const void* a1, int c1, int a0_cm,
-              const float* agn, const void* res, int rmode, hipStream_t s, const V5Aa* aa) {
+              const float* agn, const void* res, int rmode, hipStream_t s, const V5Aa* aa, bool phase) {
   const int esz = dtype_size(d->dtype);
   const int ck = 32 / esz;
   const int64_t SV = d->a_mode == 1 ? d->D * d->H * d->W / 8 : d->D * d->H * d->W;
   CWDM_REQUIRE(!agn || !a0_cm, CWDM_E_INVALID, "conv3d_v5: GroupNorm applies to raw channels-last sources only");
+  CWDM_REQUIRE(!phase || (d->a_w_phase && d->a_mode == 1 && !agn && !aa && rmode < 0 && dtype_half(d->dtype)),
+               CWDM_E_INVALID, "conv3d_v5: phase arguments");
   V4Params p{};
   p.B = (int)d->B; p.D = (int)d->D; p.H = (int)d->H; p.W = (int)d->W;
+  if (phase) { p.D /= 2; p.H /= 2; p.W /= 2; }
   p.tx = (p.W + 31) / 32; p.ty = p.H / 4; p.tz = p.D / 4;
   p.cout = d->cout; p.nct = d->cout / 64;
   p.nch0 = c0 / ck; p.nch = (c0 + c1) / ck;
   p.a0 = a0; p.ac0 = c0; p.a1 = a1; p.ac1 = c1;
   p.a0_bstride = SV * c0 * esz; p.a1_bstride = SV * c1 * esz;
   p.a0_bytes = (unsigned)(SV * c0 * esz); p.a1_bytes = (unsigned)(SV * c1 * esz);
-  p.amode = d->a_mode;
+  p.amode = phase ? 0 : d->a_mode;
   p.a0_cm = a0_cm;
   p.a0_cvox = (int)SV;
-  p.aw = reinterpret_cast<const unsigned char*>(d->a_w);
+  p.aw = reinterpret_cast<const unsigned char*>(phase ? d->a_w_phase : d->a_w);
   p.bias = d->bias; p.bias_bs = d->bias_bstride;
   p.res = res; p.rmode = rmode;
   p.out = d->out;
@@ -1140,27 +1247,22 @@
   p.diag = diag;
 #endif
   p.stamps = g_stamps.load(std::memory_order_relaxed);
-  const long long nblk = (long long)p.B * p.tx * p.ty * p.tz * p.nct;
+  const long long nblk = (long long)p.B * p.tx * p.ty * p.tz * p.nct * (phase ? 8 : 1);
+  CWDM_REQUIRE(nblk < (1LL << 31), CWDM_E_UNSUPPORTED, "conv3d_v5: too many work items");
   p.nblk = (int)nblk;
-  static const int ncu = [] {
-    int dev = 0, n = 0;
-    if (hipGetDevice(&dev) != hipSuccess || hipDeviceGetAttribute(&n, hipDeviceAttributeMultiprocessorCount, dev) != hipSuccess)
-      return 256;
-    return n > 0 ? n : 256;
-  }();
-  const int cap = g_v5_grid.load(std::memory_order_relaxed);
-  const dim3 grid(aa ? (unsigned)v5_aa_grid(nblk) : (unsigned)std::min<long long>(nblk, cap > 0 ? cap : ncu));
-  if (g_stats_wg && d->stats && p.B == 1 && p.nct <= 2 &&
-      (long long)grid.x <= (long long)p.tx * p.ty * p.tz) {
+  const dim3 grid(aa ? (unsigned)v5_aa_grid(nblk) : v5_grid(nblk));
+  const long long otiles = phase ? ((d->W + 31) / 32) * (d->H / 4) * (d->D / 4) : (long long)p.tx * p.ty * p.tz;
+  if (g_stats_wg && d->stats && p.B == 1 && p.nct <= 2 && (long long)grid.x <= otiles) {
     p.stats_wg = 1;
     g_stats_rows = grid.x;
   }
+  CWDM_REQUIRE(!(agn && p.amode == 1 && dtype_half(d->dtype)), CWDM_E_UNSUPPORTED,
+               "conv3d_v5: GroupNorm in LDS on an upsampling conv");
   prof_begin(s);
   auto go = [&](auto tag) {
     using T = decltype(tag);
     if (agn) {
-      if (p.amode == 1) hipLaunchKernelGGL((conv3d_v5_kernel<T, 1, true>), grid, dim3(512), 0, s, p);
-      else hipLaunchKernelGGL((conv3d_v5_kernel<T, 0, true>), grid, dim3(512), 0, s, p);
+      hipLaunchKernelGGL((conv3d_v5_kernel<T, 0, true>), grid, dim3(512), 0, s, p);
     } else {
       if (p.amode == 1) hipLaunchKernelGGL((conv3d_v5_kernel<T, 1, false>), grid, dim3(512), 0, s, p);
       else hipLaunchKernelGGL((conv3d_v5_kernel<T, 0, false>), grid, dim3(512), 0, s, p);
@@ -1175,6 +1277,10 @@
       if (p.amode == 1) hipLaunchKernelGGL((conv3d_v5s_kernel<1, false>), grid, dim3(512), 0, s, p);
       else hipLaunchKernelGGL((conv3d_v5s_kernel<0, false>), grid, dim3(512), 0, s, p);
     }
+  } else if (phase) {
+    g_up_phase_launches.fetch_add(1, std::memory_order_relaxed);
+    if (d->dtype == CWDM_BF16) hipLaunchKernelGGL((conv3d_v5_kernel<bf16_t, 2, false>), grid, dim3(512), 0, s, p);
+    else hipLaunchKernelGGL((conv3d_v5_kernel<f16_t, 2, false>), grid, dim3(512), 0, s, p);
   } else if (aa) {
     g_v5_aa_launches.fetch_add(1, std::memory_order_relaxed);
     auto go_aa = [&](auto tag) {
@@ -1189,17 +1295,18 @@
   } else {
     go(f16_t{});
   }
-  prof_end(s, 2.0 * p.B * p.D * p.H * p.W * (double)p.cout * 27.0 * (c0 + c1));
+  prof_end(s, phase ? 2.0 * d->B * d->D * d->H * d->W * (double)p.cout * 8.0 * (c0 + c1)
+                    : 2.0 * p.B * p.D * p.H * p.W * (double)p.cout * 27.0 * (c0 + c1));
   CWDM_LAUNCHED();
   return CWDM_OK;
 }
 
+template __global__ void conv3d_v5_kernel<bf16_t, 2, false>(V4Params);
+template __global__ void conv3d_v5_kernel<f16_t, 2, false>(V4Params);
 template __global__ void conv3d_v5_kernel<bf16_t, 0, true>(V4Params);
-template __global__ void conv3d_v5_kernel<bf16_t, 1, true>(V4Params);
 template __global__ void conv3d_v5_kernel<bf16_t, 0, false>(V4Params);
 template __global__ void conv3d_v5_kernel<bf16_t, 1, false>(V4Params);
 template __global__ void conv3d_v5_kernel<f16_t, 0, true>(V4Params);
-template __global__ void conv3d_v5_kernel<f16_t, 1, true>(V4Params);
 template __global__ void conv3d_v5_kernel<f16_t, 0, false>(V4Params);
 template __global__ void conv3d_v5_kernel<f16_t, 1, false>(V4Params);
 template __global__ void conv3d_v5_kernel<bf16_t, 0, false, 4>(V4Params);
@@ -1218,6 +1325,19 @@
   return cwdm::g_v5_aa.exchange(on > 2 ? 2 : on);
 }
 
+extern "C" int cwdm_debug_up_phase(int on) {
+  if (on < 0) return cwdm::g_up_phase_launches.load(std::memory_order_relaxed);
+  return cwdm::g_up_phase.exchange(on ? 1 : 0);
+}
+
+extern "C" int64_t cwdm_debug_stats_wg(int on) {
+  if (on < 0) return cwdm::g_stats_rows;
+  const int prev = cwdm::g_stats_wg;
+  cwdm::g_stats_wg = on ? 1 : 0;
+  cwdm::g_stats_rows = 0;
+  return prev;
+}
+
 extern "C" int cwdm_debug_v5_aa_timeout(int extra, int spin) {
   CWDM_REQUIRE(extra >= 0 && spin >= 0, CWDM_E_INVALID, "cwdm_debug_v5_aa_timeout: extra, spin >= 0");
   cwdm::g_v5_aa_extra.store(extra);
diff --git a/fast-cwdm_amd/csrc/internal.hpp b/fast-cwdm_amd/csrc/internal.hpp
--- a/fast-cwdm_amd/csrc/internal.hpp
+++ b/fast-cwdm_amd/csrc/internal.hpp
@@ -51,6 +51,7 @@
 
 bool v5_eligible(const cwdm_conv3d_desc* d, bool gn);
 int v5_aa_units(const cwdm_conv3d_desc* d, int* lead);
+bool v5_phase_ok(const cwdm_conv3d_desc* d, int rmode);
 extern thread_local int g_stats_wg;
 extern thread_local int64_t g_stats_rows;
 
diff --git a/fast-cwdm_amd/csrc/unet_plan.cpp b/fast-cwdm_amd/csrc/unet_plan.cpp
--- a/fast-cwdm_amd/csrc/unet_plan.cpp
+++ b/fast-cwdm_amd/csrc/unet_plan.cpp
@@ -52,6 +52,7 @@
   int skip_conv = -1;
   int64_t wsplit_off = -1;
   int64_t hsplit_off = -1;
+  int64_t wphase_off = -1;
   int64_t xsplit_off = -1;
   int64_t xsplit_sk_off = -1;
   int s2 = 0;
@@ -504,6 +505,9 @@
     cs.w_off = take(cwdm_conv3d_packed_bytes(cs.cout, cs.cin_a, 3, c.dtype));
     if (c.mfma_split && c.dtype == CWDM_F32 && !cs.s2 && cs.cout % 64 == 0 && cs.cin_a % 16 == 0)
       cs.wsplit_off = take(cwdm_conv3d_packed_split_bytes(cs.cout, cs.cin_a));
+    if (dtype_half(c.dtype) && cs.amode == 1 && !cs.s2 && cs.ws_p < 0 && cs.rmode == -1 && cs.cout % 64 == 0 &&
+        cs.cin_a % 16 == 0 && cs.cin_a >= 32)
+      cs.wphase_off = take(cwdm_conv3d_packed_phase_bytes(cs.cout, cs.cin_a, c.dtype));
     if (c.mfma_split && c.dtype == CWDM_F32 && &cs == &u->convs[u->head_c] && cs.a1 < 0 && cs.amode == 0 &&
         cs.gn >= 0 && cs.cout <= 16 && cs.cin_a % 32 == 0 && 3 * cs.cin_a <= 256) {
       cs.hsplit_off = take(cwdm_conv3d_packed_bytes(cs.cout, 3 * cs.cin_a, 3, CWDM_BF16));
@@ -864,6 +868,9 @@
       } else if ((rc = cwdm_conv3d_pack(P[cs.w_p], cs.cout, cs.cin_a, 3, u->cfg.dtype, base + cs.w_off, stream))) {
         return rc;
       }
+      if (cs.wphase_off >= 0 &&
+          (rc = cwdm_conv3d_pack_phase(P[cs.w_p], cs.cout, cs.cin_a, u->cfg.dtype, base + cs.wphase_off, stream)))
+        return rc;
       if (cs.wsplit_off >= 0 &&
           (rc = cwdm_conv3d_pack_split(P[cs.w_p], cs.cout, cs.cin_a, base + cs.wsplit_off, stream)))
         return rc;
@@ -1044,6 +1051,7 @@
     d.a_gn = cs.gn >= 0 ? reinterpret_cast<const float*>(wb + L.ss_off[cs.gn]) : nullptr;
     d.a_w = pk + cs.w_off;
     d.a_w_split = cs.wsplit_off >= 0 ? pk + cs.wsplit_off : nullptr;
+    d.a_w_phase = cs.wphase_off >= 0 ? pk + cs.wphase_off : nullptr;
     if (cs.ws_p >= 0) {
       d.b0 = tptr(cs.sb0); d.b_c0 = u->tensors[cs.sb0].channels;
       d.b1 = tptr(cs.sb1); d.b_c1 = cs.sb1 >= 0 ? u->tensors[cs.sb1].channels : 0;
diff --git a/fast-cwdm_amd/cwdm_hip/_lib.py b/fast-cwdm_amd/cwdm_hip/_lib.py
--- a/fast-cwdm_amd/cwdm_hip/_lib.py
+++ b/fast-cwdm_amd/cwdm_hip/_lib.py
@@ -59,6 +59,7 @@
         ("out1", vp), ("out_c0", ctypes.c_int),
         ("accumulate", ctypes.c_int),
         ("a_w_split", vp),
+        ("a_w_phase", vp),
     ]
 
 
@@ -130,6 +131,8 @@
     "cwdm_conv3d_pack": (ctypes.c_int, [vp, ctypes.c_int, ctypes.c_int, ctypes.c_int, ctypes.c_int, vp, vp]),
     "cwdm_conv3d_packed_split_bytes": (i64, [ctypes.c_int, ctypes.c_int]),
     "cwdm_conv3d_pack_split": (ctypes.c_int, [vp, ctypes.c_int, ctypes.c_int, vp, vp]),
+    "cwdm_conv3d_packed_phase_bytes": (i64, [ctypes.c_int, ctypes.c_int, ctypes.c_int]),
+    "cwdm_conv3d_pack_phase": (ctypes.c_int, [vp, ctypes.c_int, ctypes.c_int, ctypes.c_int, vp, vp]),
     "cwdm_conv3d_pack_dgrad": (ctypes.c_int, [vp, ctypes.c_int, ctypes.c_int, ctypes.c_int, ctypes.c_int, vp, vp]),
     "cwdm_conv3d_parts": (i64, [ctypes.c_int, i64, i64, i64, ctypes.c_int]),
     "cwdm_space_to_depth": (ctypes.c_int, [vp, ctypes.c_int, i64, i64, i64, i64, ctypes.c_int, vp, ctypes.c_int,
@@ -145,6 +148,8 @@
     "cwdm_conv3d_set_path": (ctypes.c_int, [ctypes.c_int]),
     "cwdm_debug_v5_grid": (ctypes.c_int, [ctypes.c_int]),
     "cwdm_debug_v5_aa": (ctypes.c_int, [ctypes.c_int]),
+    "cwdm_debug_up_phase": (ctypes.c_int, [ctypes.c_int]),
+    "cwdm_debug_stats_wg": (i64, [ctypes.c_int]),
     "cwdm_debug_v5_aa_timeout": (ctypes.c_int, [ctypes.c_int, ctypes.c_int]),
     "cwdm_device_status": (ctypes.c_int, [ctypes.c_int]),
     "cwdm_debug_gn_fin_apply": (ctypes.c_int, [vp, i64, ctypes.c_int, vp, i64, ctypes.c_int, vp, vp, ctypes.c_int,
diff --git a/include/cwdm.h b/include/cwdm.h
--- a/include/cwdm.h
+++ b/include/cwdm.h
@@ -128,12 +128,16 @@
   void* out1; int out_c0;
   int accumulate;
   const void* a_w_split;
+  const void* a_w_phase;
 } cwdm_conv3d_desc;
 int64_t cwdm_conv3d_packed_bytes(int cout, int cin, int ksize, int dtype);
 int64_t cwdm_conv3d_packed_split_bytes(int cout, int cin);
 int cwdm_conv3d_pack_split(const float* w_oidhw, int cout, int cin, void* packed, cwdm_stream_t stream);
 int cwdm_conv3d_pack(const float* w_oidhw, int cout, int cin, int ksize, int dtype,
                      void* packed, cwdm_stream_t stream);
+int64_t cwdm_conv3d_packed_phase_bytes(int cout, int cin, int dtype);
+int cwdm_conv3d_pack_phase(const float* w_oidhw, int cout, int cin, int dtype, void* packed,
+                           cwdm_stream_t stream);
 int cwdm_conv3d_pack_dgrad(const float* w_oidhw, int cout, int cin, int ksize, int dtype,
                            void* packed, cwdm_stream_t stream);
 int cwdm_space_to_depth(const void* x, int C, int64_t B, int64_t d, int64_t h, int64_t w, int dtype, void* out,
@@ -160,6 +164,10 @@
 int cwdm_debug_v5_grid(int n);
 
 int cwdm_debug_v5_aa(int on);
+
+int cwdm_debug_up_phase(int on);
+
+int64_t cwdm_debug_stats_wg(int on);
 
 int cwdm_debug_v5_aa_timeout(int extra, int spin);
 
```

After: 68.91 denoising-steps/s (median of 6 runs). +4.8%, better.
